# beast-dev/beast-mcmc

Hardware: AMD Instinct MI355X
Metric: full-tree lnL evals/sec (GTR+G4, 1e5 patterns) (higher is better)
Workload: dtype f64

## Files before the change

### beast-mcmc_amd/beagle.py

```python
import ctypes as C
import os

import numpy as np

_HERE = os.path.dirname(os.path.abspath(__file__))
ENGINE_LIB = os.path.join(_HERE, "lib", "libhmsbeagle-jni.so")
if os.environ.get("BEAGLE_MI355_ENGINE_LIB"):
    ENGINE_LIB = os.environ["BEAGLE_MI355_ENGINE_LIB"]
HOST_LIB = os.path.join(_HERE, "lib", "libbeast_host.so")

NONE = -1
FLAG_EIGEN_REAL, FLAG_EIGEN_COMPLEX, FLAG_PROCESSOR_GPU, FLAG_FRAMEWORK_CPU = 1 << 4, 1 << 5, 1 << 16, 1 << 27
OPERATION_TUPLE_SIZE = 7

ERROR_NAMES = {0: "NO_ERROR", -1: "GENERAL_ERROR", -2: "OUT_OF_MEMORY_ERROR", -3: "UNIDENTIFIED_EXCEPTION_ERROR",
               -4: "UNINITIALIZED_INSTANCE_ERROR", -5: "OUT_OF_RANGE_ERROR", -6: "NO_RESOURCE_ERROR",
               -7: "NO_IMPLEMENTATION_ERROR", -8: "FLOATING_POINT_ERROR"}


class BeagleException(RuntimeError):

    def __init__(self, function_name, code):
        super().__init__("%s returned %d (%s)" % (function_name, code, ERROR_NAMES.get(code, "?")))
        self.function_name = function_name
# ... 56 lines not shown
    "ConvolveTransitionMatrices": ([C.c_int, _IP, _IP, _IP, C.c_int], C.c_int),
    "UpdateTransitionMatrices": ([C.c_int, C.c_int, _IP, _IP, _IP, _DP, C.c_int], C.c_int),
    "UpdateTransitionMatricesWithMultipleModels": ([C.c_int, _IP, _IP, _IP, _IP, _IP, _DP, C.c_int], C.c_int),
    "UpdatePartials": ([C.c_int, _IP, C.c_int, C.c_int], C.c_int),
    "UpdatePartialsByPartition": ([C.c_int, _IP, C.c_int], C.c_int),
    "WaitForPartials": ([C.c_int, _IP, C.c_int], C.c_int),
    "AccumulateScaleFactors": ([C.c_int, _IP, C.c_int, C.c_int], C.c_int),
    "AccumulateScaleFactorsByPartition": ([C.c_int, _IP, C.c_int, C.c_int, C.c_int], C.c_int),
    "RemoveScaleFactors": ([C.c_int, _IP, C.c_int, C.c_int], C.c_int),
    "RemoveScaleFactorsByPartition": ([C.c_int, _IP, C.c_int, C.c_int, C.c_int], C.c_int),
    "ResetScaleFactors": ([C.c_int, C.c_int], C.c_int),
    "ResetScaleFactorsByPartition": ([C.c_int, C.c_int, C.c_int], C.c_int),
    "CopyScaleFactors": ([C.c_int, C.c_int, C.c_int], C.c_int),
    "CalculateRootLogLikelihoods": ([C.c_int, _IP, _IP, _IP, _IP, C.c_int, _DP], C.c_int),
    "CalculateRootLogLikelihoodsByPartition": ([C.c_int, _IP, _IP, _IP, _IP, _IP, C.c_int, C.c_int, _DP, _DP], C.c_int),
    "GetSiteLogLikelihoods": ([C.c_int, _DP], C.c_int),
    "SetRootPrePartials": ([C.c_int, _IP, _IP, C.c_int], C.c_int),
    "SetDifferentialMatrix": ([C.c_int, C.c_int, _DP], C.c_int),
    "AddTransitionMatrices": ([C.c_int, _IP, _IP, _IP, C.c_int], C.c_int),
    "TransposeTransitionMatrices": ([C.c_int, _IP, _IP, C.c_int], C.c_int),
    "UpdatePrePartials": ([C.c_int, _IP, C.c_int, C.c_int], C.c_int),
    "UpdatePrePartialsByPartition": ([C.c_int, _IP, C.c_int], C.c_int),
    "CalculateEdgeDifferentials": ([C.c_int, _IP, _IP, _IP, _IP, C.c_int, _DP, _DP, _DP], C.c_int),
    "CalculateCrossProductDifferentials": ([C.c_int, _IP, _IP, _IP, _IP, _DP, C.c_int, _DP, _DP], C.c_int),
}

ABI_SYMBOLS = ["beagleGetVersion", "beagleGetCitation", "beagleGetResourceList", "beagleGetBenchmarkedResourceList", "beagleGetApiTable",
               "beagleGetPartitionApiTable"] + \
              ["beagle" + k for k in _PROTOS] + \
              ["beagleMi355SetStream", "beagleMi355CalculateRootLogLikelihoodsDevice", "beagleMi355Synchronize",
               "beagleMi355KernelTimer", "beagleMi355DeviceBytes", "beagleMi355WalkStats", "beagleMi355GradientStats", "beagleMi355GetPartialsBatch", "beagleMi355SampleAncestralStates", "beagleMi355SampleMarkovJumps", "beagleMi355SampleMarkovJumpsUniformized",
               "beagleMi355SimulateSequences", "beagleMi355SimulateCompleteHistories", "beagleMi355RobustCounts", "beagleMi355SimulateUnconditionedCounts", "beagleMi355NodeHeightDerivatives", "beagleMi355UpdateDifferentialMatrices", "beagleMi355SetReversibleModels", "beagleMi355GetEigenDecomposition", "beagleMi355EigenStats", "beagleMi355UpdateTransitionMatricesFromGenerators", "beagleMi355GeneratorStats", "beagleMi355UpdateTransitionMatricesWithEpochs", "beagleMi355EpochStats", "beagleMi355NodePatternLikelihoods", "beagleMi355NodePatternStats", "beagleMi355NodePosteriors", "beagleMi355NodePosteriorStats", "beagleMi355PlacementScores", "beagleMi355PlacementStats", "beagleMi355SetTipEmission", "beagleMi355TipEmissionStats",
               "beagleMi355GetPartialsPinned", "beagleMi355GetSiteLogLikelihoodsPinned",
               "beagleMi355KernelTimerCalls", "beagleMi355WalkHealth", "beagleMi355RepeatStats", "beagleMi355RepeatSubRunStats", "beagleMi355TableOperandStats", "beagleMi355WalkLaunchInfo", "beagleMi355RootFusedCount", "beagleMi355SitePrefetchCount", "beagleMi355KernelTimerRestart", "beagleMi355GetDimensions", "beagleMi355GetCommUniqueId", "beagleMi355CommInit", "beagleMi355CommInfo", "beagleMi355CalculateRootLogLikelihoodsAllReduce"] + \
              ["beagleBasta" + k for k in ("AllocateCoalescentBuffers", "UpdatePartials", "AccumulatePartials", "GetBuffer", "GetBufferLength", "Stats", "SampleStates", "StatesStats",
                                           "Gradient", "GradientStats", "UpdatePartialsGrad", "UpdateTransitionMatricesGrad", "AccumulatePartialsGrad")]
BASTA_OPERATION_SIZE = 8


class EngineLibrary:

    def __init__(self, path=ENGINE_LIB, prefix=""):
        if not os.path.exists(path):
            raise OSError("engine library %s is missing: run `python -c 'import __graft_entry__ as g; g.build()'` "
                          "(there is no CPU fallback)" % path)
        self.path = path
        self.prefix = prefix
        self.lib = C.CDLL(path, mode=C.RTLD_LOCAL)
        self.fn = {}
        for name, (argtypes, restype) in _PROTOS.items():
            f = getattr(self.lib, prefix + "beagle" + name, None)
            if f is None:
                continue
            f.argtypes = argtypes
            f.restype = restype
            self.fn[name] = f
        gv = getattr(self.lib, prefix + "beagleGetVersion")
        gv.restype = C.c_char_p
        self.version = gv().decode()
        tab = getattr(self.lib, prefix + "beagleGetApiTable")
        tab.restype = C.c_void_p
        self.api_table = tab()
        ptab = getattr(self.lib, prefix + "beagleGetPartitionApiTable", None)
        self.partition_api_table = None
        if ptab is not None:
            ptab.restype = C.c_void_p
            self.partition_api_table = ptab()
# ... 858 lines not shown

    def bastaGradientStats(self):
        out = (C.c_long * 4)()
        self._check("bastaGradientStats", self._ext("beagleBastaGradientStats", [C.c_int, C.POINTER(C.c_long)])(self.instance, out))
        return tuple(out)

    def walkStats(self):
        out = (C.c_long * 8)()
        self._check("walkStats", self._ext("beagleMi355WalkStats", [C.c_int, C.POINTER(C.c_long)])(self.instance, out))
        keys = ("micro_ops", "stored", "mem_reads", "tip_reads", "scale_reads", "walks", "scale_writes", "fast_walks")
        stats = {k: int(out[i]) for i, k in enumerate(keys)}
        rep = self.repeatStats()
        stats.update({k: rep[k] for k in ("table_rows", "table_reads", "repeat_clades")})
        return stats

    def repeatStats(self):
        out = (C.c_long * 10)()
        self._check("repeatStats", self._ext("beagleMi355RepeatStats", [C.c_int, C.POINTER(C.c_long)])(self.instance, out))
        keys = ("table_rows", "table_reads", "repeat_clades", "table_bytes", "clades_indexed", "index_host_us", "two_table_nodes",
                "tables_under_definitions", "index_host_bytes", "index_resets")
        return {k: int(out[i]) for i, k in enumerate(keys)}

    def repeatSubRunStats(self):
        out = (C.c_long * 2)()
        self._check("repeatSubRunStats", self._ext("beagleMi355RepeatSubRunStats", [C.c_int, C.POINTER(C.c_long)])(self.instance, out))
        return {"sub_runs": int(out[0]), "sub_run_micro_ops": int(out[1])}

    def tableOperandStats(self):
        out = (C.c_long * 4)()
        self._check("tableOperandStats", self._ext("beagleMi355TableOperandStats", [C.c_int, C.POINTER(C.c_long)])(self.instance, out))
        return {"table_first_children": int(out[0]), "behind_memory_first_child": int(out[1]), "behind_fused_cherry": int(out[2]),
                "max_classes": int(out[3])}

    def walkHealth(self):
        out = (C.c_long * 4)()
        self._check("walkHealth", self._ext("beagleMi355WalkHealth", [C.c_int, C.POINTER(C.c_long)])(self.instance, out))
        return {"self_served": int(out[0]), "spin_limit_us": int(out[1]), "folded_vectors": int(out[2]), "fold_builds": int(out[3])}

    def walkLaunchInfo(self):
        out = (C.c_long * 8)()
        self._check("walkLaunchInfo", self._ext("beagleMi355WalkLaunchInfo", [C.c_int, C.POINTER(C.c_long)])(self.instance, out))
        return {"ticket_walks": int(out[0]), "flag_walks": int(out[1]), "rows": int(out[2]), "slices": int(out[3]),
                "fused_cherries": int(out[4]), "micro_ops": int(out[5]), "slice_accumulations": int(out[6]), "partition_roots_in_walk": int(out[7])}

    def gradientStats(self):
        out = (C.c_long * 4)()
        self._check("gradientStats", self._ext("beagleMi355GradientStats", [C.c_int, C.POINTER(C.c_long)])(self.instance, out))
        return {"fused": int(out[0]), "by_operation": int(out[1]), "walked": int(out[2]), "late": int(out[3])}

    def deviceBytes(self):
        return self._ext("beagleMi355DeviceBytes", [C.c_int], C.c_long)(self.instance)
```

### beast-mcmc_amd/csrc/engine_abi.cpp

```cpp
#include "engine_internal.h"

using mi355::OpDesc;
using mi355::shardedStates;
using mi355::shardedCategories;
using namespace mi355::eng;

namespace {

int accumulate(Instance* in, const int* idx, int count, int cum, double sign, int part) {
    if (badIndex(cum, in->scaleCount) || (part >= 0 && badIndex(part, in->partitionCount))) return BEAGLE_ERROR_OUT_OF_RANGE;
    const int pStart = part < 0 ? 0 : in->partStart[part], pEnd = part < 0 ? in->P : in->partEnd[part];
    int rc = materializeScaleUsers(in, cum); if (rc) return rc;
    rc = ensureScale(in, cum); if (rc) return rc;
    if (in->scaleIsRaw[cum]) return BEAGLE_ERROR_OUT_OF_RANGE;
    if (in->walk && in->sliceSums && in->partitionCount == 1 && in->lastSums.valid && in->lastSums.epoch == in->scaleWriteEpoch &&
        count > 0 && count == in->lastSums.nWritten) {
        const long stamp = ++in->seenCounter;
        bool same = true;
        for (int k = 0; k < count && same; k++) {
            if (badIndex(idx[k], in->scaleCount)) return BEAGLE_ERROR_OUT_OF_RANGE;
            same = in->scaleGen[(size_t)idx[k]] == in->lastSums.gen && in->scaleSeen[(size_t)idx[k]] != stamp;
            in->scaleSeen[(size_t)idx[k]] = stamp;
        }
        if (same) {
// ... 11 lines not shown
    for (int k = 0; k < count; k++) {
        if (badIndex(idx[k], in->scaleCount)) return BEAGLE_ERROR_OUT_OF_RANGE;
        rc = ensureScale(in, idx[k]); if (rc) return rc;
        srcs[k] = in->scale[idx[k]]; raw[k] = in->scaleIsRaw[idx[k]];
    }
    const int chunk = 4096;
    for (int b = 0; b < count; b += chunk) {
        const int n = std::min(chunk, count - b);
        void *dSrc = nullptr, *dRaw = nullptr;
        rc = uploadTransient(in, &srcs[b], (size_t)n * sizeof(double*), &dSrc); if (rc) return rc;
        rc = uploadTransient(in, &raw[b], (size_t)n * sizeof(int), &dRaw); if (rc) return rc;
        mi355::launchAccumulateScale(live(in), in->scale[cum], (const double* const*)dSrc, (const int*)dRaw, n, sign, pStart, pEnd);
    }
    HIP_TRY(hipGetLastError());
    return 0;
}

int runTriples(Instance* in, const int* first, const int* second, const int* result, int count, decltype(&mi355::launchConvolveMatrices) launch) {
    int b = 0;
    while (b < count) {
        int e = b + 1;
        for (; e < count; e++) {
            bool dep = false;
            for (int k = b; k < e && !dep; k++)
                dep = result[k] == first[e] || result[k] == second[e] || result[k] == result[e] ||
                      first[k] == result[e] || second[k] == result[e];
            if (dep) break;
        }
        const int n = e - b;
        void *dF, *dS, *dR;
        int rc = uploadTransient(in, first + b, n * sizeof(int), &dF); if (rc) return rc;
        rc = uploadTransient(in, second + b, n * sizeof(int), &dS); if (rc) return rc;
        rc = uploadTransient(in, result + b, n * sizeof(int), &dR); if (rc) return rc;
        launch(live(in), in->matrices, (const int*)dF, (const int*)dS, (const int*)dR, n, in->S, in->C);
        b = e;
    }
    HIP_TRY(hipGetLastError());
    return BEAGLE_SUCCESS;
}

void toTiled(const Instance* in, const double* api, double* tiled, int categories) {
    const size_t S = in->S, P = in->P, nt = in->ntile;
    std::fill(tiled, tiled + (size_t)categories * nt * S * 32, 0.0);
    for (int c = 0; c < categories; c++)
        for (size_t p = 0; p < P; p++) {
            const double* src = api + ((size_t)c * P + p) * S;
            double* dst = tiled + ((size_t)c * nt + p / 32) * S * 32 + p % 32;
            for (size_t j = 0; j < S; j++) dst[j * 32] = src[j];
        }
}

}

extern "C" {

const char* beagleGetVersion(void) { return "4.0.0-mi355"; }

const char* beagleGetCitation(void) {
    return "MI355X-native tree-likelihood engine behind the beagle.Beagle surface (gfx950 HIP kernels).\n"
           "API after: Ayres et al. (2019) BEAGLE 3, Systematic Biology 68:1052-1061.";
}

BeagleResourceList* beagleGetResourceList(void) { return &resources()->rl; }

int beagleFinalizeInstance(int instance) {
    if (mi355::isShardedHandle(instance)) { return mi355::shardedFinalize(instance); }
    Instance* in = nullptr;
// ... 16 lines not shown
int beagleSetPatternWeights(int instance, const double* w) {
    if (mi355::isShardedHandle(instance)) {
        return mi355::shardedSetPerPatternDoubles(instance, w, 1, 1, [&](int h, const double* v) { return beagleSetPatternWeights(h, v); });
    }
    GET_INSTANCE(instance);
    return upload(in, in->patternWeights, w, (size_t)in->P * sizeof(double));
}

int beagleSetPatternPartitions(int instance, int partitionCount, const int* partitions) {
    if (mi355::isShardedHandle(instance)) {
        return mi355::shardedSetPerPatternInts(instance, partitions,
                                               [&](int h, const int* v) { return beagleSetPatternPartitions(h, partitionCount, v); });
    }
    GET_INSTANCE(instance);
    if (partitionCount < 1) return BEAGLE_ERROR_OUT_OF_RANGE;
    for (int x = 0; x < in->partialsCount; x++) { int rcv = materializeVirtual(in, x); if (rcv) return rcv; }
    std::vector<int> s(partitionCount, -1), e(partitionCount, -1);
    for (int p = 0; p < in->P; p++) {
        const int k = partitions[p];
        if (badIndex(k, partitionCount)) return BEAGLE_ERROR_OUT_OF_RANGE;
        if (s[k] < 0) s[k] = p;
        else if (e[k] != p) return BEAGLE_ERROR_NO_IMPLEMENTATION;
        e[k] = p + 1;
    }
    for (int k = 0; k < partitionCount; k++) if (s[k] < 0) { s[k] = 0; e[k] = 0; }
    in->partitionCount = partitionCount; in->partStart = s; in->partEnd = e; in->resolveEpoch++;
    if (in->walk || in->walkT || in->virt) in->planner.setPartitionCount(partitionCount);
    if (in->virt) {
        const size_t per = (size_t)in->C * in->S * in->S, slots = matrixSlotLayout(in);
        double* grown = nullptr;
        int rcm = devAlloc(in, (void**)&grown, slots * per * sizeof(double)); if (rcm) return rcm;
        HIP_TRY(hipMemsetAsync(grown, 0, slots * per * sizeof(double), live(in)));
        HIP_TRY(hipMemcpyAsync(grown, in->matrices, (size_t)std::max(1, in->matrixCount) * per * sizeof(double), hipMemcpyDeviceToDevice, live(in)));
        in->matrices = grown;
        if (in->tiled) { int rci = uploadIdentityMatrix(in); if (rci) return rci; }
    }
    if (in->walk) {
        forgetFolds(in);
        setPairLayout(in);
        in->sliceRows = 0; in->lastSums.valid = false;
        if (!in->dPairPos) { int rc = devAlloc(in, (void**)&in->dPairPos, (size_t)in->P * sizeof(unsigned)); if (rc) return rc; }
        HIP_TRY(hipStreamSynchronize(live(in)));
        HIP_TRY(hipMemcpy(in->dPairPos, in->pairPos.data(), (size_t)in->P * sizeof(unsigned), hipMemcpyHostToDevice));
        in->stateSlabLeft = 0; in->scaleSlabLeft = 0;
        std::vector<mi355::RelayoutJob> jobs;
        for (int t = 0; t < in->partialsCount; t++) {
            uint8_t* old = in->tipStates[t];
            if (!old) continue;
            in->tipStates[t] = nullptr;
            int rc = ensureStates(in, t); if (rc) return rc;
            jobs.push_back({old, in->tipStates[t], in->tipStates[t] + in->statePairOff});
        }
        for (size_t b = 0; b < jobs.size(); b += 16384) {
            const size_t e = std::min(jobs.size(), b + 16384);
            void* dJobs = nullptr;
            int rc = uploadTransient(in, jobs.data() + b, (e - b) * sizeof(mi355::RelayoutJob), &dJobs); if (rc) return rc;
            mi355::launchRelayoutStatesBatch(live(in), (const mi355::RelayoutJob*)dJobs, (int)(e - b), in->dPairPos, in->P, (int)in->pairLen, in->S);
        }
        for (int k = 0; k < (int)in->scale.size(); k++) {
            double* old = in->scale[k];
            if (!old) continue;
            const char raw = in->scaleIsRaw[k];
            in->scale[k] = nullptr;
            int rc = ensureScale(in, k); if (rc) return rc;
            in->scaleIsRaw[k] = raw;
            HIP_TRY(hipMemcpyAsync(in->scale[k], old, (size_t)in->P * sizeof(double), hipMemcpyDeviceToDevice, live(in)));
            if (raw) mi355::launchRecipFromFactors(live(in), in->scale[k], in->scale[k] + in->scaleStride, in->dPairPos, in->P);
// ... 200 lines not shown

int beagleConvolveTransitionMatrices(int instance, const int* first, const int* second, const int* result, int count) {
    if (mi355::isShardedHandle(instance)) {
        return mi355::shardedBroadcast(instance, [&](int h) { return beagleConvolveTransitionMatrices(h, first, second, result, count); });
    }
    GET_INSTANCE(instance);
    if (count <= 0) return BEAGLE_SUCCESS;
    for (int k = 0; k < count; k++) {
        if (badIndex(first[k], in->matrixCount) || badIndex(second[k], in->matrixCount) || badIndex(result[k], in->matrixCount) ||
            result[k] == first[k] || result[k] == second[k]) return BEAGLE_ERROR_OUT_OF_RANGE;
    }
    return runTriples(in, first, second, result, count, mi355::launchConvolveMatrices);
}

static void noteScaleOfOp(Instance* in, const int* op, int tuple) {
    if (badIndex(op[0], in->partialsCount)) return;
    const int sIdx = op[1] != BEAGLE_OP_NONE ? op[1] : op[2];
    if (op[1] != BEAGLE_OP_NONE && !badIndex(op[1], in->scaleCount)) in->scaleVersion[op[1]]++;
    const bool unknown = tuple == BEAGLE_PARTITION_OP_COUNT && in->partitionCount > 1;
    in->scaleOfPartial[op[0]] = unknown ? -2 : (sIdx != BEAGLE_OP_NONE && !badIndex(sIdx, in->scaleCount)) ? sIdx : -1;
    in->scaleVersionAtWrite[op[0]] = in->scaleOfPartial[op[0]] >= 0 ? in->scaleVersion[sIdx] : 0u;
}

static int transitionMatrices(Instance* in, const int* eigenIdx, int eigenScalar, const int* rateIdx,
                              const int* probIdx, const double* lens, int count) {
    if (count <= 0) return BEAGLE_SUCCESS;
    auto outOfRange = [count](const int* v, int limit) {
        int lo = v[0], hi = v[0];
        for (int k = 1; k < count; k++) { lo = v[k] < lo ? v[k] : lo; hi = v[k] > hi ? v[k] : hi; }
        return lo < 0 || hi >= limit;
    };
    if (outOfRange(probIdx, in->matrixCount) || (eigenIdx ? outOfRange(eigenIdx, in->eigenCount) : badIndex(eigenScalar, in->eigenCount)) ||
        (rateIdx && outOfRange(rateIdx, in->eigenCount))) return BEAGLE_ERROR_OUT_OF_RANGE;
    bool fusable = in->S == 4 && in->kernelUploads && in->fuseLaunches && !eigenIdx && !rateIdx && (size_t)count * 12 <= RING_BYTES / 4 &&
                   (int)in->pendingCopies.size() <= mi355::HOST_COPY_MAX;
    if (fusable) {
        const char* m0 = (const char*)in->matrices;
        const char* m1 = m0 + (size_t)std::max(1, in->matrixCount) * in->C * in->S * in->S * sizeof(double);
        const std::vector<Instance::PendingCopy>& pc = in->pendingCopies;
        for (size_t a = 0; a < pc.size() && fusable; a++) {
            const char* d0 = (const char*)pc[a].dst; const char* d1 = d0 + pc[a].bytes;
            if (d0 < m1 && m0 < d1) fusable = false;
            for (size_t b = a + 1; b < pc.size() && fusable; b++) {
                const char* e0 = (const char*)pc[b].dst; const char* e1 = e0 + pc[b].bytes;
                if (d0 < e1 && e0 < d1 && !(e0 <= d0 && d1 <= e1)) fusable = false;
            }
        }
    }
    if (fusable) {
        const size_t lenBytes = (size_t)count * sizeof(double), idxBytes = (size_t)count * sizeof(int);
        const long off = stage(in, lens, lenBytes, lenBytes + idxBytes);
        if (off < 0) return BEAGLE_ERROR_GENERAL;
        memcpy(in->hRing + off + lenBytes, probIdx, idxBytes);
        const size_t eigStride = in->eigenComplex ? 40 : 36;
        const double* const eigDst = in->eigen + eigStride * eigenScalar;
        const double* eigSrc = eigDst;
        const double* ratesSrc = in->rates;
        mi355::HostCopyList L;
        L.n = 0;
        unsigned blocks = 0;
        for (const Instance::PendingCopy& pc : in->pendingCopies) {
            mi355::HostCopyList::Entry& e = L.e[L.n++];
            e.dst = pc.dst; e.src = in->hRingDev + pc.ringOff; e.bytes = (unsigned)pc.bytes; e.firstBlock = blocks;
            blocks += (unsigned)((pc.bytes + 4095) / 4096);
            if (pc.dst == (void*)eigDst && pc.bytes == eigStride * sizeof(double)) eigSrc = (const double*)(in->hRingDev + pc.ringOff);
            if (pc.dst == (void*)in->rates && pc.bytes >= (size_t)in->C * sizeof(double)) ratesSrc = (const double*)(in->hRingDev + pc.ringOff);
        }
        for (int a = 0; a < L.n; a++)
            for (int b = a + 1; b < L.n; b++)
                if ((const char*)L.e[b].dst <= (const char*)L.e[a].dst &&
                    (const char*)L.e[a].dst + L.e[a].bytes <= (const char*)L.e[b].dst + L.e[b].bytes) L.e[a].bytes = 0;
        in->pendingCopies.clear();
        mi355::launchTransitionMatrices4Fused(in->stream, in->matrices, eigSrc, ratesSrc, (const int*)(in->hRingDev + off + lenBytes),
                                              (const double*)(in->hRingDev + off), count, in->C, in->eigenComplex, L, (int)blocks);
        HIP_TRY(hipGetLastError());
        return BEAGLE_SUCCESS;
    }
    if (in->S == 4 && in->kernelUploads && in->fuseLaunches && (size_t)count * 20 <= RING_BYTES / 4) {
        const size_t lenBytes = (size_t)count * sizeof(double), idxBytes = (size_t)count * sizeof(int);
        const long off = stage(in, lens, lenBytes, lenBytes + 3 * idxBytes);
        if (off < 0) return BEAGLE_ERROR_GENERAL;
        memcpy(in->hRing + off + lenBytes, probIdx, idxBytes);
        int* rEig = (int*)(in->hRing + off + lenBytes + idxBytes);
        int* rRate = rEig + count;
        if (eigenIdx) memcpy(rEig, eigenIdx, idxBytes); else std::fill(rEig, rEig + count, eigenScalar);
        if (rateIdx) memcpy(rRate, rateIdx, idxBytes); else std::fill(rRate, rRate + count, 0);
        const int* rIdx = (const int*)(in->hRingDev + off + lenBytes);
        mi355::launchTransitionMatrices(live(in), in->matrices, in->eigen, in->rates, rIdx, (const double*)(in->hRingDev + off),
                                        rIdx + count, rIdx + 2 * (size_t)count, count, in->S, in->C, in->eigenComplex);
        HIP_TRY(hipGetLastError());
        return BEAGLE_SUCCESS;
    }
    std::vector<char> pack((size_t)count * (sizeof(double) + 3 * sizeof(int)));
    double* pLen = (double*)pack.data();
    int* pIdx = (int*)(pack.data() + (size_t)count * sizeof(double));
    memcpy(pLen, lens, (size_t)count * sizeof(double));
    memcpy(pIdx, probIdx, (size_t)count * sizeof(int));
    if (eigenIdx) memcpy(pIdx + count, eigenIdx, (size_t)count * sizeof(int)); else std::fill(pIdx + count, pIdx + 2 * (size_t)count, eigenScalar);
    if (rateIdx) memcpy(pIdx + 2 * (size_t)count, rateIdx, (size_t)count * sizeof(int)); else std::fill(pIdx + 2 * (size_t)count, pIdx + 3 * (size_t)count, 0);
    void* dPack;
    int rc = uploadTransient(in, pack.data(), pack.size(), &dPack); if (rc) return rc;
    const double* dLen = (const double*)dPack;
    const int* dIdx = (const int*)((const char*)dPack + (size_t)count * sizeof(double));
    mi355::launchTransitionMatrices(live(in), in->matrices, in->eigen, in->rates, dIdx, dLen,
                                    dIdx + count, dIdx + 2 * (size_t)count, count, in->S, in->C, in->eigenComplex);
    HIP_TRY(hipGetLastError());
    return BEAGLE_SUCCESS;
}

int beagleUpdateTransitionMatrices(int instance, int eigenIndex, const int* probabilityIndices,
                                   const int* firstDerivativeIndices, const int* secondDerivativeIndices,
                                   const double* edgeLengths, int count) {
    if (mi355::isShardedHandle(instance)) {
        if (firstDerivativeIndices || secondDerivativeIndices) return BEAGLE_ERROR_NO_IMPLEMENTATION;
        if (count <= 0) return BEAGLE_SUCCESS;
        std::vector<int> p(probabilityIndices, probabilityIndices + count); std::vector<double> t(edgeLengths, edgeLengths + count);
        return mi355::shardedPost(instance, [=](int h) { return beagleUpdateTransitionMatrices(h, eigenIndex, p.data(), nullptr, nullptr, t.data(), count); });
    }
    GET_INSTANCE_KEEP_PENDING(instance);
    if (firstDerivativeIndices || secondDerivativeIndices) return BEAGLE_ERROR_NO_IMPLEMENTATION;
    if (in->heldPre.held && probabilityIndices)
        for (int k = 0; k < count; k++) if (heldReadsMatrix(in, probabilityIndices[k])) { int rcp = executeHeldPre(in); if (rcp) return rcp; break; }
    return transitionMatrices(in, nullptr, eigenIndex, nullptr, probabilityIndices, edgeLengths, count);
}

int beagleUpdateTransitionMatricesWithMultipleModels(int instance, const int* eigenIndices, const int* categoryRateIndices,
                                   const int* probabilityIndices, const int* firstDerivativeIndices,
                                   const int* secondDerivativeIndices, const double* edgeLengths, int count) {
    if (mi355::isShardedHandle(instance)) {
        if (firstDerivativeIndices || secondDerivativeIndices) return BEAGLE_ERROR_NO_IMPLEMENTATION;
        if (!eigenIndices || !categoryRateIndices) return BEAGLE_ERROR_OUT_OF_RANGE;
        if (count <= 0) return BEAGLE_SUCCESS;
        std::vector<int> e(eigenIndices, eigenIndices + count), r(categoryRateIndices, categoryRateIndices + count), p(probabilityIndices, probabilityIndices + count);
        std::vector<double> t(edgeLengths, edgeLengths + count);
        return mi355::shardedPost(instance, [=](int h) { return beagleUpdateTransitionMatricesWithMultipleModels(h, e.data(), r.data(), p.data(), nullptr, nullptr, t.data(), count); });
    }
    GET_INSTANCE(instance);
    if (firstDerivativeIndices || secondDerivativeIndices) return BEAGLE_ERROR_NO_IMPLEMENTATION;
// ... 131 lines not shown
}

int beagleSetDifferentialMatrix(int instance, int matrixIndex, const double* inMatrix) {
    return beagleSetTransitionMatrix(instance, matrixIndex, inMatrix, 0.0);
}

int beagleAddTransitionMatrices(int instance, const int* first, const int* second, const int* result, int count) {
    if (mi355::isShardedHandle(instance)) {
        return mi355::shardedBroadcast(instance, [&](int h) { return beagleAddTransitionMatrices(h, first, second, result, count); });
    }
    GET_INSTANCE(instance);
    if (count <= 0) return BEAGLE_SUCCESS;
    if (!first || !second || !result) return BEAGLE_ERROR_OUT_OF_RANGE;
    for (int k = 0; k < count; k++)
        if (badIndex(first[k], in->matrixCount) || badIndex(second[k], in->matrixCount) || badIndex(result[k], in->matrixCount)) return BEAGLE_ERROR_OUT_OF_RANGE;
    return runTriples(in, first, second, result, count, mi355::launchAddMatrices);
}

int beagleTransposeTransitionMatrices(int instance, const int* inputIndices, const int* resultIndices, int matrixCount) {
    if (mi355::isShardedHandle(instance)) {
        return mi355::shardedBroadcast(instance,
                                       [&](int h) { return beagleTransposeTransitionMatrices(h, inputIndices, resultIndices, matrixCount); });
    }
    GET_INSTANCE(instance);
    if (matrixCount <= 0) return BEAGLE_SUCCESS;
    std::vector<int> pairs((size_t)matrixCount * 2);
    for (int k = 0; k < matrixCount; k++) {
        if (badIndex(inputIndices[k], in->matrixCount) || badIndex(resultIndices[k], in->matrixCount) || inputIndices[k] == resultIndices[k])
            return BEAGLE_ERROR_OUT_OF_RANGE;
        pairs[2 * k] = inputIndices[k]; pairs[2 * k + 1] = resultIndices[k];
    }
    void* dPairs = nullptr;
    int rc = uploadTransient(in, pairs.data(), pairs.size() * sizeof(int), &dPairs); if (rc) return rc;
    mi355::launchTransposeMatrices(live(in), in->matrices, (const int*)dPairs, matrixCount, in->S, in->C);
    HIP_TRY(hipGetLastError());
    return BEAGLE_SUCCESS;
}

int beagleUpdatePrePartials(int instance, const int* operations, int operationCount, int cumulativeScaleIndex) {
    if (mi355::isShardedHandle(instance)) {
        return mi355::shardedBroadcast(instance, [&](int h) { return beagleUpdatePrePartials(h, operations, operationCount, cumulativeScaleIndex); });
    }
    GET_INSTANCE_KEEP_PENDING(instance);
    DEMOTE_FOLDED_TIPS(in);
    return runPreOperations(in, operations, operationCount, cumulativeScaleIndex, true);
}

int beagleCalculateCrossProductDifferentials(int instance, const int* postBufferIndices, const int* preBufferIndices,
                                             const int* categoryRateIndices, const int* categoryWeightsIndices,
                                             const double* edgeLengths, int count,
                                             double* outSumDerivatives, double* outSumSquaredDerivatives) {
    if (mi355::isShardedHandle(instance)) {
        if (!outSumDerivatives) return BEAGLE_ERROR_OUT_OF_RANGE;
        const int len = shardedStates(instance) * shardedStates(instance);
        std::vector<double> tot(len, 0.0);
        const int rc = mi355::shardedSumDoubles(instance, len, [&](int h, double* out) { return beagleCalculateCrossProductDifferentials(h, postBufferIndices,
                              preBufferIndices, categoryRateIndices, categoryWeightsIndices, edgeLengths, count, out, outSumSquaredDerivatives); }, tot.data());
        for (int k = 0; k < len && !rc; k++) outSumDerivatives[k] += tot[k];
        return rc;
    }
    GET_INSTANCE(instance);
    DEMOTE_FOLDED_TIPS(in);
    if (outSumSquaredDerivatives) return BEAGLE_ERROR_NO_IMPLEMENTATION;
    if (!postBufferIndices || !preBufferIndices || !categoryRateIndices || !categoryWeightsIndices || !edgeLengths || !outSumDerivatives)
        return BEAGLE_ERROR_OUT_OF_RANGE;
    if (badIndex(categoryRateIndices[0], in->eigenCount) || badIndex(categoryWeightsIndices[0], in->eigenCount)) return BEAGLE_ERROR_OUT_OF_RANGE;
    return crossProducts(in, postBufferIndices, preBufferIndices, categoryRateIndices[0], categoryWeightsIndices[0], edgeLengths, count,
// ... 84 lines not shown
```

### beast-mcmc_amd/csrc/engine_create.cpp

```cpp
#include "engine_internal.h"

using mi355::labEnv;
using namespace mi355::eng;

static bool switchOn(const char* name) {
    const char* v = getenv(name);
    return v && atoi(v) != 0;
}

namespace mi355 {
namespace eng {

size_t matrixSlotLayout(Instance* in) {
    size_t slots = std::max<size_t>(std::max<size_t>(1, in->matrixCount), (size_t)in->planner.matrixSlots());
    if (in->tiled) { in->preIdentity = (int)slots; in->preTransposed = (int)slots + 1; slots += 1 + PRE_SCRATCH; }
    if (in->emis) { in->emis->shadowBase = (int)slots; slots += (size_t)std::max(1, in->matrixCount); }
    return slots;
}
int uploadIdentityMatrix(Instance* in) {
    const size_t S = in->S, C = in->C;
    std::vector<double> eye(C * S * S, 0.0);
    for (size_t c = 0; c < C; c++) for (size_t i = 0; i < S; i++) eye[c * S * S + i * S + i] = 1.0;
    return upload(in, in->matrices + (size_t)in->preIdentity * C * S * S, eye.data(), eye.size() * sizeof(double));
}
// ... 147 lines not shown
                     !switchOn("BEAGLE_MI355_NO_T32_WRITE_WALK");
    in->planner.init(partialsBufferCount, tipCount, matrixBufferCount, scaleBufferCount, maxVirtSteps, virtualOn, in->holdSlots);
    {
        int memSteps = maxVirtSteps == 24 ? MEM_DEF_STEPS : 0, seenSteps = maxVirtSteps == 24 ? MEM_DEF_SEEN_STEPS : 0;
        if (getenv("BEAGLE_MI355_MEM_DEF_STEPS")) { memSteps = std::max(0, std::min(maxVirtSteps, atoi(getenv("BEAGLE_MI355_MEM_DEF_STEPS")))); seenSteps = 0; }
        if (getenv("BEAGLE_MI355_MEM_DEF_SEEN_STEPS")) seenSteps = std::max(0, std::min(maxVirtSteps, atoi(getenv("BEAGLE_MI355_MEM_DEF_SEEN_STEPS"))));
        if (switchOn("BEAGLE_MI355_NO_MEM_DEFS") || !in->walk || in->walkT || !virtualOn || in->holdSlots < 2) memSteps = seenSteps = 0;
        in->planner.memStepCap = memSteps;
        in->planner.memStepCapSeen = seenSteps;
        if (getenv("BEAGLE_MI355_MEM_DEF_INLINE_STEPS")) in->memDefInlineSteps = std::max(0, atoi(getenv("BEAGLE_MI355_MEM_DEF_INLINE_STEPS")));
    }
    {
        double frac = 1.0 / 8.0;
        if (const char* f = getenv("BEAGLE_MI355_REPEAT_MAX_FRAC")) {
            const char* slash = strchr(f, '/');
            const double num = atof(f), den = slash ? atof(slash + 1) : 1.0;
            if (num > 0.0 && den > 0.0) frac = num > 1.0 && !slash ? 1.0 / num : num / den;
        }
        frac = std::min(frac, 0.5);
        in->repeatsOn = in->walk && !in->walkT && virtualOn && stateCount == 4 && in->holdSlots >= 2 && !switchOn("BEAGLE_MI355_NO_REPEATS") &&
                        (bufferBytes >= ((size_t)2 << 20) || switchOn("BEAGLE_MI355_REPEATS_ANY_SIZE"));
        in->repeatMaxClasses = std::max(1, (int)((double)patternCount * frac));
        if (in->repeatsOn) { in->repeatIndex.init(tipCount, patternCount, in->repeatMaxClasses); in->hostTips.assign((size_t)tipCount, std::vector<uint8_t>()); }
        if (in->repeatsOn && getenv("BEAGLE_MI355_REPEAT_CAPACITY")) in->repeatIndex.setCapacity((size_t)std::max(1, atoi(getenv("BEAGLE_MI355_REPEAT_CAPACITY"))));
    }
    in->planner.memDefTables = !switchOn("BEAGLE_MI355_NO_MEMDEF_TABLES");
    in->planner.cacheEnabled = !switchOn("BEAGLE_MI355_NO_PLAN_CACHE");
    in->fastWalk = !switchOn("BEAGLE_MI355_NO_FAST_WALK");
    in->strictWaits = !(getenv("BEAGLE_MI355_STRICT_WAITS") && atoi(getenv("BEAGLE_MI355_STRICT_WAITS")) == 0);
    in->fuseGradient = !switchOn("BEAGLE_MI355_NO_FUSED_GRADIENT");
    in->preWalk = !switchOn("BEAGLE_MI355_NO_PRE_WALK");
    in->fuseLaunches = !switchOn("BEAGLE_MI355_NO_LAUNCH_FUSION");
    in->deferWalk = !switchOn("BEAGLE_MI355_NO_ROOT_FUSION");
    in->foldScales = !switchOn("BEAGLE_MI355_NO_SCALE_FOLD");
    {
        const int gv = getenv("BEAGLE_MI355_GRADIENT_VIRTUAL") ? atoi(getenv("BEAGLE_MI355_GRADIENT_VIRTUAL")) : GRADIENT_VIRT_DEFAULT;
        in->gradientVirtual = in->walk && virtualOn && in->preWalk && in->fuseGradient && gv > 0;
        in->gradientVirtualSteps = std::max(1, std::min(GRADIENT_VIRT_STEPS, gv));
    }
    const size_t matrixSlots = matrixSlotLayout(in);
    const size_t patternSlots = in->tiled ? (size_t)in->ntile * 32 : (size_t)patternCount;
    in->partialsBytes = (((size_t)categoryCount * patternSlots * stateCount * sizeof(double)) + 255 + (in->walk ? 256 : 0)) & ~(size_t)255;
    in->partials.assign(partialsBufferCount, nullptr);
    in->scaleOfPartial.assign(partialsBufferCount, -2); in->scaleVersionAtWrite.assign(partialsBufferCount, 0u);
    in->scaleVersion.assign(std::max(1, scaleBufferCount), 0u);
    in->tipStates.assign(partialsBufferCount, nullptr);
    in->scale.assign(std::max(1, scaleBufferCount), nullptr);
    in->scaleIsRaw.assign(std::max(1, scaleBufferCount), 0);
    in->partStart.assign(1, 0); in->partEnd.assign(1, patternCount);
    setPairLayout(in);
    in->wStamp.assign(partialsBufferCount, 0); in->wLevel.assign(partialsBufferCount, 0); in->wOp.assign(partialsBufferCount, 0);
    in->rStamp.assign(partialsBufferCount, 0); in->rLevel.assign(partialsBufferCount, 0);
    in->resourceName = res->names[device + 1];

    bool ok = hipStreamCreateWithFlags(&in->ownStream, hipStreamNonBlocking) == hipSuccess;
    in->stream = in->ownStream;
    ok = ok && hipHostMalloc((void**)&in->hRing, RING_BYTES, hipHostMallocMapped | hipHostMallocCoherent) == hipSuccess;
    ok = ok && hipHostGetDevicePointer((void**)&in->hRingDev, in->hRing, 0) == hipSuccess;
    in->kernelUploads = !switchOn("BEAGLE_MI355_COPY_ENGINE_UPLOADS");
    in->sitePrefetch = !switchOn("BEAGLE_MI355_NO_SITE_PREFETCH");
    in->fuseWaves = !switchOn("BEAGLE_MI355_NO_WALK_FUSION");
    in->useTickets = !switchOn("BEAGLE_MI355_NO_WALK_TICKETS");
    in->xcdAware = !switchOn("BEAGLE_MI355_NO_XCD_MAP");
    in->fuseCherries = !switchOn("BEAGLE_MI355_NO_CHERRY_FUSION");
    in->skipTipLoads = !switchOn("BEAGLE_MI355_NO_LOAD_SKIP");
    in->sliceSums = !switchOn("BEAGLE_MI355_NO_SLICE_SUMS");
// ... 62 lines not shown
```

### beast-mcmc_amd/csrc/engine_differential.cpp

```cpp
#include "engine_internal.h"

using namespace mi355::eng;

static int differentialMatrices(Instance* in, const int* eigenIdx, const int* rateIdx, const double* inDifferentials, int differentialCount,
                                const int* diffIdx, const int* slots, const double* lens, int count, int mode) {
    if (in->S > 64 || in->basta) return BEAGLE_ERROR_NO_IMPLEMENTATION;
    if (count <= 0) return BEAGLE_SUCCESS;
    if (mode != BEAGLE_MI355_DIFFERENTIAL_EXACT && mode != BEAGLE_MI355_DIFFERENTIAL_FIRST_ORDER) return BEAGLE_ERROR_OUT_OF_RANGE;
    if (!inDifferentials || !slots || !lens || differentialCount < 1) return BEAGLE_ERROR_OUT_OF_RANGE;
    std::vector<char> named((size_t)in->matrixCount, 0);
    for (int k = 0; k < count; k++) {
        if (badIndex(slots[k], in->matrixCount) || named[(size_t)slots[k]]) return BEAGLE_ERROR_OUT_OF_RANGE;
        named[(size_t)slots[k]] = 1;
        if ((eigenIdx && badIndex(eigenIdx[k], in->eigenCount)) || (rateIdx && badIndex(rateIdx[k], in->eigenCount)) ||
            (diffIdx && badIndex(diffIdx[k], differentialCount))) return BEAGLE_ERROR_OUT_OF_RANGE;
    }
    if (in->eigenCount < 1) return BEAGLE_ERROR_OUT_OF_RANGE;
    const bool exact = mode == BEAGLE_MI355_DIFFERENTIAL_EXACT;
    std::vector<int> pairs, pairOf((size_t)count);
    if (exact) {
        std::unordered_map<long long, int> seen;
        for (int k = 0; k < count; k++) {
            const int e = eigenIdx ? eigenIdx[k] : 0, d = diffIdx ? diffIdx[k] : 0;
            const auto at = seen.emplace((long long)e * differentialCount + d, (int)(pairs.size() / 2));
            if (at.second) { pairs.push_back(e); pairs.push_back(d); }
            pairOf[(size_t)k] = at.first->second;
        }
    } else for (int k = 0; k < count; k++) pairOf[(size_t)k] = diffIdx ? diffIdx[k] : 0;
    const size_t per = (size_t)in->S * in->S, nPairs = pairs.size() / 2;
    const size_t qBytes = (size_t)differentialCount * per * sizeof(double), lenBytes = (size_t)count * sizeof(double),
                 idxBytes = (size_t)count * sizeof(int), bytes = qBytes + lenBytes + 4 * idxBytes + pairs.size() * sizeof(int);
    if (bytes > RING_BYTES / 2) return BEAGLE_ERROR_OUT_OF_RANGE;
    for (int k = 0; k < count; k++)
        if (heldReadsMatrix(in, slots[k])) { const int rcp = executeHeldPre(in); if (rcp) return rcp; break; }
    std::vector<char> pack(bytes);
    memcpy(pack.data(), inDifferentials, qBytes);
    memcpy(pack.data() + qBytes, lens, lenBytes);
    int* pIdx = (int*)(pack.data() + qBytes + lenBytes);
    memcpy(pIdx, slots, idxBytes);
    if (eigenIdx) memcpy(pIdx + count, eigenIdx, idxBytes); else std::fill(pIdx + count, pIdx + 2 * (size_t)count, 0);
    if (rateIdx) memcpy(pIdx + 2 * (size_t)count, rateIdx, idxBytes); else std::fill(pIdx + 2 * (size_t)count, pIdx + 3 * (size_t)count, 0);
    memcpy(pIdx + 3 * (size_t)count, pairOf.data(), idxBytes);
    if (!pairs.empty()) memcpy(pIdx + 4 * (size_t)count, pairs.data(), pairs.size() * sizeof(int));
    if (exact) {
        const size_t need = nPairs * per * sizeof(double);
        const int rcg = growDevice(in, in->differentialDev, need, (need + 4095) & ~(size_t)4095, Grow::SyncIfHeld); if (rcg) return rcg;
    }
    void* dPack = nullptr;
    const int rc = uploadTransient(in, pack.data(), bytes, &dPack); if (rc) return rc;
    const double* dQ = (const double*)dPack;
    const double* dLen = (const double*)((const char*)dPack + qBytes);
    const int* dIdx = (const int*)((const char*)dPack + qBytes + lenBytes);
    const int *dEig = dIdx + count, *dRate = dIdx + 2 * (size_t)count, *dPair = dIdx + 3 * (size_t)count, *dPairs = dIdx + 4 * (size_t)count;
    if (exact) {
        double* V = in->differentialDev.as<double>();
        mi355::launchDifferentialRotate(live(in), V, in->eigen, dQ, dPairs, (int)nPairs, in->S, in->eigenComplex);
        mi355::launchDifferentialExact(live(in), in->matrices, in->eigen, in->rates, V, dIdx, dLen, dEig, dRate, dPair, count, in->S, in->C,
                                       in->eigenComplex);
    } else {
        mi355::launchDifferentialFirstOrder(live(in), in->matrices, in->rates, dQ, dIdx, dLen, dRate, dPair, count, in->S, in->C);
    }
    HIP_TRY(hipGetLastError());
    return BEAGLE_SUCCESS;
}

extern "C" {

int beagleMi355UpdateDifferentialMatrices(int instance, const int* eigenIndices, const int* categoryRatesIndices,
                                          const double* inDifferentials, int differentialCount, const int* differentialIndices,
                                          const int* matrixIndices, const double* edgeLengths, int count, int mode) {
    if (mi355::isShardedHandle(instance)) {
        return mi355::shardedBroadcast(instance, [&](int h) {
            return beagleMi355UpdateDifferentialMatrices(h, eigenIndices, categoryRatesIndices, inDifferentials, differentialCount,
                                                         differentialIndices, matrixIndices, edgeLengths, count, mode); });
    }
    GET_INSTANCE_KEEP_PENDING(instance);
    return differentialMatrices(in, eigenIndices, categoryRatesIndices, inDifferentials, differentialCount, differentialIndices,
                                matrixIndices, edgeLengths, count, mode);
}

}
```

### beast-mcmc_amd/csrc/engine_epoch.cpp

```cpp
#include "engine_internal.h"

using namespace mi355::eng;

constexpr size_t EPOCH_LAUNCH_BYTES = RING_BYTES / 4;

static size_t epochChunk() {
    if (const char* e = getenv("BEAGLE_MI355_EPOCH_CHUNK")) { const long v = atol(e); if (v > 0) return (size_t)v; }
    return SIZE_MAX;
}

static int checkEpochList(int S, const int* off, const int* segEig, const double* segLen, const int* slots, int count, int flags) {
    if (S > 64) return BEAGLE_ERROR_NO_IMPLEMENTATION;
    if (count < 0 || flags != 0) return BEAGLE_ERROR_OUT_OF_RANGE;
    if (count == 0) return BEAGLE_SUCCESS;
    if (!off || !segEig || !segLen || !slots) return BEAGLE_ERROR_OUT_OF_RANGE;
    if (off[0] != 0) return BEAGLE_ERROR_OUT_OF_RANGE;
    for (int k = 0; k < count; k++) if (off[k + 1] <= off[k]) return BEAGLE_ERROR_OUT_OF_RANGE;
    for (int j = 0; j < off[count]; j++) if (!(std::isfinite(segLen[j]) && segLen[j] >= 0.0)) return BEAGLE_ERROR_OUT_OF_RANGE;
    return BEAGLE_SUCCESS;
}

static int epochMatrices(Instance* in, const int* off, const int* segEig, const double* segLen, const int* rateIdx, const int* slots,
                         int count, int flags) {
    const int rcc = checkEpochList(in->S, off, segEig, segLen, slots, count, flags); if (rcc) return rcc;
// ... 9 lines not shown
    for (int j = 0; j < off[count]; j++) if (badIndex(segEig[j], in->eigenCount)) return BEAGLE_ERROR_OUT_OF_RANGE;
    if (in->eigenCount < 1) return BEAGLE_ERROR_OUT_OF_RANGE;
    for (int k = 0; k < count; k++)
        if (heldReadsMatrix(in, slots[k])) { const int rcp = executeHeldPre(in); if (rcp) return rcp; break; }
    const size_t chunk = epochChunk();
    std::vector<char> pack;
    for (int first = 0; first < count;) {
        const size_t perEntry = 3 * sizeof(int), perSeg = sizeof(double) + sizeof(int);
        int last = first + 1;
        size_t bytes = sizeof(int) + perEntry + (size_t)(off[last] - off[first]) * perSeg;
        while (last < count && (size_t)(last - first) < chunk) {
            const size_t more = perEntry + (size_t)(off[last + 1] - off[last]) * perSeg;
            if (bytes + more > EPOCH_LAUNCH_BYTES) break;
            bytes += more; last++;
        }
        const size_t m = (size_t)(last - first), s0 = (size_t)off[first], nSeg = (size_t)off[last] - s0;
        pack.resize(nSeg * sizeof(double) + (m + 1 + nSeg + 2 * m) * sizeof(int));
        double* pLen = (double*)pack.data();
        int* pOff = (int*)(pack.data() + nSeg * sizeof(double));
        int* pEig = pOff + m + 1;
        int* pSlot = pEig + nSeg;
        int* pRate = pSlot + m;
        memcpy(pLen, segLen + s0, nSeg * sizeof(double));
        memcpy(pEig, segEig + s0, nSeg * sizeof(int));
        for (size_t k = 0; k <= m; k++) pOff[k] = off[(size_t)first + k] - (int)s0;
        for (size_t k = 0; k < m; k++) { pSlot[k] = slots[(size_t)first + k]; pRate[k] = rateIdx ? rateIdx[(size_t)first + k] : 0; }
        void* dPack = nullptr;
        const int rc = uploadTransient(in, pack.data(), pack.size(), &dPack); if (rc) return rc;
        const double* dLen = (const double*)dPack;
        const int* dOff = (const int*)((const char*)dPack + nSeg * sizeof(double));
        const int* dEig = dOff + m + 1;
        const int* dSlot = dEig + nSeg;
        const int* dRate = dSlot + m;
        if (!mi355::launchEpochMatrices(live(in), in->matrices, in->eigen, in->rates, dSlot, dRate, dOff, dEig, dLen, (int)m, in->S, in->C,
                                        in->eigenComplex)) return BEAGLE_ERROR_GENERAL;
        HIP_TRY(hipGetLastError());
        first = last;
    }
    in->statEpochCalls++; in->statEpochMatrices += (long)count * in->C; in->statEpochSegments += off[count]; in->statEpochLongest = longest;
    return BEAGLE_SUCCESS;
}

extern "C" {

int beagleMi355UpdateTransitionMatricesWithEpochs(int instance, const int* segmentOffsets, const int* segmentEigenIndices,
                                                  const double* segmentLengths, const int* categoryRateIndices,
                                                  const int* probabilityIndices, int count, int flags) {
    if (mi355::isShardedHandle(instance)) {
        const int rcc = checkEpochList(mi355::shardedStates(instance), segmentOffsets, segmentEigenIndices, segmentLengths,
                                       probabilityIndices, count, flags); if (rcc) return rcc;
        if (count == 0) return BEAGLE_SUCCESS;
        const int nSeg = segmentOffsets[count];
        std::vector<int> o(segmentOffsets, segmentOffsets + count + 1), e(segmentEigenIndices, segmentEigenIndices + nSeg),
                         p(probabilityIndices, probabilityIndices + count), r;
        std::vector<double> t(segmentLengths, segmentLengths + nSeg);
        if (categoryRateIndices) r.assign(categoryRateIndices, categoryRateIndices + count);
        const bool hasR = categoryRateIndices != nullptr;
        return mi355::shardedPost(instance, [=](int h) {
            return beagleMi355UpdateTransitionMatricesWithEpochs(h, o.data(), e.data(), t.data(), hasR ? r.data() : nullptr, p.data(), count, 0); });
    }
    GET_INSTANCE_KEEP_PENDING(instance);
    return epochMatrices(in, segmentOffsets, segmentEigenIndices, segmentLengths, categoryRateIndices, probabilityIndices, count, flags);
}

int beagleMi355EpochStats(int instance, long* out4) {
    if (mi355::isShardedHandle(instance)) { return mi355::shardedFirst(instance, [&](int h) { return beagleMi355EpochStats(h, out4); }); }
    GET_INSTANCE_KEEP_PENDING(instance);
// ... 7 lines not shown
```

### beast-mcmc_amd/csrc/engine_generator.cpp

```cpp
#include "engine_internal.h"
#include <cfloat>

using namespace mi355::eng;

constexpr size_t GENERATOR_TABLE_BUDGET = (size_t)128 << 20;

static size_t generatorChunk(size_t n) {
    n = std::max<size_t>(1, n);
    if (const char* e = getenv("BEAGLE_MI355_GENERATOR_CHUNK")) { const long v = atol(e); if (v > 0) n = std::min(n, (size_t)v); }
    return n;
}

static int checkGenerators(int S, const double* Q, int G, const double* lens, int count, std::vector<double>& mu) {
    if (S > 64) return BEAGLE_ERROR_NO_IMPLEMENTATION;
    if (count < 0 || G < 1 || !Q) return BEAGLE_ERROR_OUT_OF_RANGE;
    if (count > 0 && !lens) return BEAGLE_ERROR_OUT_OF_RANGE;
    mu.resize((size_t)G);
    for (int g = 0; g < G; g++) {
        const double* q = Q + (size_t)g * S * S;
        for (int i = 0; i < S; i++)
            for (int j = 0; j < S; j++) {
                const double x = q[(size_t)i * S + j];
                if (!std::isfinite(x) || (i == j ? x > 0.0 : x < 0.0)) return BEAGLE_ERROR_OUT_OF_RANGE;
            }
// ... 37 lines not shown
        if (heldReadsMatrix(in, slots[k])) { const int rcp = executeHeldPre(in); if (rcp) return rcp; break; }
    int rc = growScratch(in, in->generatorDev, std::min((size_t)G, genChunk) * tableBytes); if (rc) return rc;
    bool fresh = false;
    rc = growDevice(in, in->generatorStatsDev, 2 * sizeof(unsigned), 256, Grow::SyncIfHeld, &fresh); if (rc) return rc;
    if (fresh) HIP_TRY(hipMemsetAsync(in->generatorStatsDev.p, 0, 256, live(in)));
    std::vector<char> pack;
    for (size_t p = 0; p < nParts; p++) {
        const size_t g0 = p * genChunk, nGen = std::min(genChunk, (size_t)G - g0);
        bool tablesDone = false;
        for (size_t first = (size_t)partStart[p]; first < (size_t)partStart[p + 1]; first += entChunk) {
            const size_t m = std::min(entChunk, (size_t)partStart[p + 1] - first);
            const size_t qBytes = tablesDone ? 0 : nGen * SS * sizeof(double), muBytes = nGen * sizeof(double),
                         lenBytes = m * sizeof(double), idxBytes = m * sizeof(int), bytes = qBytes + muBytes + lenBytes + 3 * idxBytes;
            pack.resize(bytes);
            if (qBytes) memcpy(pack.data(), Q + g0 * SS, qBytes);
            memcpy(pack.data() + qBytes, mu.data() + g0, muBytes);
            double* pLen = (double*)(pack.data() + qBytes + muBytes);
            int* pIdx = (int*)(pack.data() + qBytes + muBytes + lenBytes);
            for (size_t k = 0; k < m; k++) {
                const int e = order[first + k];
                pLen[k] = lens[e];
                pIdx[k] = slots[e];
                pIdx[m + k] = (genIdx ? genIdx[e] : 0) - (int)g0;
                pIdx[2 * m + k] = rateIdx ? rateIdx[e] : 0;
            }
            void* dPack = nullptr;
            rc = uploadTransient(in, pack.data(), bytes, &dPack); if (rc) return rc;
            const double* dMu = (const double*)((const char*)dPack + qBytes);
            const double* dLen = (const double*)((const char*)dPack + qBytes + muBytes);
            const int* dIdx = (const int*)((const char*)dPack + qBytes + muBytes + lenBytes);
            double* tables = in->generatorDev.as<double>();
            if (!tablesDone && !mi355::launchGeneratorPowers(live(in), tables, (const double*)dPack, dMu, (int)nGen, in->S)) return BEAGLE_ERROR_GENERAL;
            tablesDone = true;
            if (!mi355::launchGeneratorMatrices(live(in), in->matrices, in->rates, tables, dMu, dIdx, dLen, dIdx + m, dIdx + 2 * m,
                                                in->generatorStatsDev.as<unsigned>(), (int)m, in->S, in->C)) return BEAGLE_ERROR_GENERAL;
            HIP_TRY(hipGetLastError());
        }
    }
    in->statGeneratorCalls++; in->statGeneratorMatrices += (long)count * in->C;
    return BEAGLE_SUCCESS;
}

extern "C" {

int beagleMi355UpdateTransitionMatricesFromGenerators(int instance, const double* generators, int generatorCount,
                                                      const int* generatorIndices, const int* categoryRateIndices,
                                                      const int* probabilityIndices, const double* edgeLengths, int count) {
    if (mi355::isShardedHandle(instance)) {
        const int S = mi355::shardedStates(instance);
        std::vector<double> mu;
        const int rcc = checkGenerators(S, generators, generatorCount, edgeLengths, count, mu); if (rcc) return rcc;
        if (count == 0) return BEAGLE_SUCCESS;
        if (!probabilityIndices) return BEAGLE_ERROR_OUT_OF_RANGE;
        std::vector<double> q(generators, generators + (size_t)generatorCount * S * S), t(edgeLengths, edgeLengths + count);
        std::vector<int> p(probabilityIndices, probabilityIndices + count), g, r;
        if (generatorIndices) g.assign(generatorIndices, generatorIndices + count);
        if (categoryRateIndices) r.assign(categoryRateIndices, categoryRateIndices + count);
        const bool hasG = generatorIndices != nullptr, hasR = categoryRateIndices != nullptr;
        return mi355::shardedPost(instance, [=](int h) {
            return beagleMi355UpdateTransitionMatricesFromGenerators(h, q.data(), generatorCount, hasG ? g.data() : nullptr,
                                                                     hasR ? r.data() : nullptr, p.data(), t.data(), count); });
    }
    GET_INSTANCE_KEEP_PENDING(instance);
    return generatorMatrices(in, generators, generatorCount, generatorIndices, categoryRateIndices, probabilityIndices, edgeLengths, count);
}

int beagleMi355GeneratorStats(int instance, long* out4) {
// ... 14 lines not shown
```

### beast-mcmc_amd/csrc/engine_instance.cpp

```cpp
#include "engine_internal.h"

using mi355::OpDesc;

namespace mi355 {
namespace eng {

std::mutex g_mutex;
std::vector<Instance*> g_instances;

Instance* lookup(int h) {
    std::lock_guard<std::mutex> lock(g_mutex);
    if (h < 0 || h >= (int)g_instances.size()) return nullptr;
    return g_instances[h];
}

int devAlloc(Instance* in, void** p, size_t bytes, bool counted) {
    HIP_TRY(hipMalloc(p, bytes));
    in->allocations.push_back({*p, bytes, counted});
    if (counted) in->deviceBytes += bytes;
    return 0;
}

void devFree(Instance* in, void* p) {
    if (!p) return;
// ... 5 lines not shown

int growDevice(Instance* in, DevBuf& b, size_t need, size_t want, Grow how, bool* grew) {
    if (grew) *grew = false;
    if (b.bytes >= need) return 0;
    if (how == Grow::SyncAndFree || (how == Grow::SyncIfHeld && b.p)) HIP_TRY(hipStreamSynchronize(live(in)));
    if (how != Grow::KeepOld) devFree(in, b.p);
    b.p = nullptr; b.bytes = 0;
    int rc = devAlloc(in, (void**)&b.p, want, b.counted); if (rc) { b.p = nullptr; return rc; }
    b.bytes = want;
    if (grew) *grew = true;
    return 0;
}

int ScopedDevice::alloc(size_t bytes) {
    reset();
    if (hipMalloc(&p, bytes) != hipSuccess) { p = nullptr; return BEAGLE_ERROR_OUT_OF_MEMORY; }
    return 0;
}
void ScopedDevice::reset() { if (p) { hipStreamSynchronize(live(in)); hipFree(p); p = nullptr; } }

long stage(Instance* in, const void* src, size_t bytes, size_t reserve) {
    const size_t need = (std::max(bytes, reserve) + 255) & ~(size_t)255;
    if (need > RING_BYTES) return -1;
    if (in->ringHead + need > RING_BYTES) {
        if (hipStreamSynchronize(live(in)) != hipSuccess) return -1;
        in->ringHead = 0;
    }
    const size_t off = in->ringHead;
    memcpy(in->hRing + off, src, bytes);
    in->ringHead += need;
    return (long)off;
}

int upload(Instance* in, void* dst, const void* src, size_t bytes) {
    if (bytes == 0) return 0;
    if (bytes <= RING_BYTES / 4) {
        long off = stage(in, src, bytes);
        if (off < 0) return BEAGLE_ERROR_GENERAL;
        return queueCopy(in, dst, (size_t)off, bytes);
    }
    HIP_TRY(hipMemcpyAsync(dst, src, bytes, hipMemcpyHostToDevice, live(in)));
    HIP_TRY(hipStreamSynchronize(live(in)));
    return 0;
}

int uploadTransient(Instance* in, const void* src, size_t bytes, void** dptr) {
    long off = stage(in, src, bytes);
    if (off < 0) return BEAGLE_ERROR_GENERAL;
    *dptr = in->dRing + off;
    return queueCopy(in, in->dRing + off, (size_t)off, bytes);
}

int queueCopy(Instance* in, void* dst, size_t off, size_t bytes) {
    if (bytes == 0) return 0;
    if (in->pendingWalk.valid && !in->copyKeepsWalk) { const int rcw = flushWalk(in); if (rcw) return rcw; }
    if (!in->kernelUploads) {
        HIP_TRY(hipMemcpyAsync(dst, in->hRing + off, bytes, hipMemcpyHostToDevice, in->stream));
        return 0;
    }
    Instance::PendingCopy pc; pc.dst = dst; pc.ringOff = off; pc.bytes = bytes;
    in->pendingCopies.push_back(pc);
    return 0;
}

int flushUploads(Instance* in) {
    std::vector<Instance::PendingCopy>& pc = in->pendingCopies;
    int rc = 0;
    for (size_t i = 0; i < pc.size();) {
        mi355::HostCopyList L;
        L.n = 0;
        unsigned blocks = 0;
        for (; i < pc.size() && L.n < mi355::HOST_COPY_MAX; i++) {
            const char* d0 = (const char*)pc[i].dst; const char* d1 = d0 + pc[i].bytes;
            bool partial = false;
            for (int a = 0; a < L.n; a++) {
                const char* e0 = (const char*)L.e[a].dst; const char* e1 = e0 + L.e[a].bytes;
                if (L.e[a].bytes == 0 || !(d0 < e1 && e0 < d1)) continue;
                if (d0 <= e0 && e1 <= d1) L.e[a].bytes = 0; else partial = true;
            }
            if (partial) break;
            mi355::HostCopyList::Entry& e = L.e[L.n++];
            e.dst = pc[i].dst; e.src = in->hRingDev + pc[i].ringOff; e.bytes = (unsigned)pc[i].bytes; e.firstBlock = blocks;
            blocks += (unsigned)((pc[i].bytes + 4095) / 4096);
        }
        mi355::launchHostCopies(in->stream, L, (int)blocks);
    }
    pc.clear();
    if (hipGetLastError() != hipSuccess) rc = BEAGLE_ERROR_GENERAL;
// ... 170 lines not shown
```

### beast-mcmc_amd/csrc/engine_internal.h

```cpp
#pragma once
#include <hip/hip_runtime.h>
#include <rccl/rccl.h>
#include <algorithm>
#include <climits>
#include <cmath>
#include <cstdio>
#include <cstdlib>
#include <cstring>
#include <mutex>
#include <string>
#include <thread>
#include <vector>
#include <chrono>
#include <atomic>
#include <unordered_map>
#include "../../include/beagle_mi355.h"
#include "kernels.h"
#include "planner.h"
#include "scratch_layout.h"
#include "sharded.h"

namespace mi355 {
namespace eng {


#define HIP_TRY(expr)                                                                         \
    do {                                                                                      \
        hipError_t e__ = (expr);                                                              \
        if (e__ != hipSuccess) {                                                              \
            if (getenv("BEAGLE_MI355_DEBUG"))                                                 \
                fprintf(stderr, "[beagle-mi355] %s failed: %s (%s:%d)\n", #expr, hipGetErrorString(e__), __FILE__, __LINE__); \
            return e__ == hipErrorOutOfMemory ? BEAGLE_ERROR_OUT_OF_MEMORY : BEAGLE_ERROR_GENERAL; \
        }                                                                                     \
    } while (0)

constexpr size_t RING_BYTES = 16u << 20;
constexpr int SLAB_BUFFERS = 32;
constexpr int PRE_SCRATCH = 32;
constexpr int GRADIENT_VIRT_STEPS = 2;
constexpr int MEM_DEF_STEPS = 8;
constexpr int MEM_DEF_SEEN_STEPS = 24;
constexpr int MEM_DEF_INLINE_STEPS = 8;
constexpr int GRADIENT_VIRT_DEFAULT = 1;

struct Basta;
struct TipEmissions;

struct DevBuf {
    char* p = nullptr; size_t bytes = 0;
    bool counted = true;
    template <class T> T* as() const { return reinterpret_cast<T*>(p); }
};
// ... 10 lines not shown
    mi355::WalkPlanner planner;
    mi355::Plan plan;
    size_t scaleStride = 0;
    size_t statePairOff = 0;
    std::vector<unsigned> pairPos; size_t pairLen = 0; std::vector<int> padStart; unsigned* dPairPos = nullptr;
    DevBufUncounted matStream;
    uint8_t* dummyTips = nullptr; double* onesScale = nullptr;
    long statFastWalks = 0;
    struct WalkTraffic {
        long memReads = 0, tipReads = 0, scaleReads = 0, scaleWrites = 0, stored = 0, fused = 0;
        long microOps = 0;
        long tableRows = 0, tableReads = 0, repeatClades = 0, twoTables = 0, unstoredConsumers = 0;
        long subRuns = 0, subRunOps = 0;
        long tabFirst = 0, tabFirstBehindMem = 0, tabFirstBehindCherry = 0, tabMaxClasses = 0;
    };
    struct Resolved {
        bool kept = false;
        long tag = 0, epoch = -1;
        std::vector<mi355::WalkOp> w; std::vector<mi355::WalkSeg> segs; std::vector<int> deps;
        bool oneLaunch = false;
        std::vector<int> order;
        int leaves = 0;
        int maxRange = 0, sinks = 0;
        std::vector<int> finalStore, finalPart, sinkRows;
        std::vector<int> sumRows, wroteScale;
        std::vector<const double*> cm;
        WalkTraffic traffic;
        DevBufUncounted dProg; bool dProgValid = false;
        std::vector<int> folds;
        long foldEpoch = -1;
        long noFoldTag = 0;
        bool compressed = false; mi355::RepeatPlan repeats; int lowerRange = 0;
        bool repeatsMissing = false;
    } resolved[8], scratch;
    struct FoldVec { std::vector<int> members; double* recip = nullptr; long builtEpoch = -1; bool bad = false; };
    std::vector<FoldVec> folds;
    std::vector<std::pair<size_t, int>> foldIndex;
    std::vector<double*> foldFree;
    long scaleWriteEpoch = 0;
    bool foldScales = true;
    DevBuf foldWorst;
    long resolveEpoch = 0;
    bool repeatsOn = false; int repeatMaxClasses = 0;
    bool repeatSlicing = false, repeatSlicingOff = false;
    int memDefInlineSteps = MEM_DEF_INLINE_STEPS;
    int closedListRun = 0;
    mi355::RepeatIndex repeatIndex;
    std::vector<std::vector<uint8_t>> hostTips;
    long tipDataEpoch = 0, repeatEpoch = -1, repeatCompactEpoch = -1;
    struct RepeatTable { int D = 0, arena = 0, row = 0; char* dev = nullptr; size_t bytes = 0, tipStride = 0; std::vector<int> tips; };
    std::unordered_map<int, RepeatTable> repeatTables;
    struct RepeatBlock { char* dev = nullptr; size_t size = 0, used = 0; };
    std::vector<RepeatBlock> repeatPool;
    char* repeatStage = nullptr; size_t repeatStageSize = 0, repeatStageUsed = 0;
    double* repeatArena = nullptr; int repeatArenas = 0; mi355::RepeatRows repeatRows;
    std::vector<int> repeatQueue;
    long statTableRows = 0, statTableReads = 0, statRepeatClades = 0, statTwoTables = 0, statUnstoredConsumers = 0;
    long statSubRuns = 0, statSubRunOps = 0;
    long statTabFirst = 0, statTabFirstBehindMem = 0, statTabFirstBehindCherry = 0, statTabMaxClasses = 0;
    size_t repeatTableCap = 0;
    bool lastPlanCached = false;
    long statRepeatResets = 0;
    long statRepeatBuildUs = 0;
    bool lowerLaunched = false;
    bool fastWalk = true;
    struct HeldPreNode { int par, preA, preB, postA, postB, matA, matB, level, jobA, jobB, size; };
    struct HeldPreList {
// ... 2 lines not shown
        std::vector<HeldPreNode> nodes;
        std::vector<int> order;
        std::vector<unsigned> walkFlags;
        std::vector<int> segStart, segRoot;
        int maxLevel = 0, holdSlots = 0, rootBuf = -1;
        std::vector<char> readsMatrix, readsBuf, writesBuf;
    } heldPre;
    double* preRootCopy = nullptr;
    uint8_t* preDummyStates = nullptr;
    DevBuf dPreProg;
    std::vector<int> scaleOfPartial; std::vector<unsigned> scaleVersionAtWrite, scaleVersion;
    bool trackScales = false;
    long statFusedGradients = 0, statPreLists = 0, statWalkedGradients = 0, statLateLists = 0;
    int storeAllEvaluations = 0;
    bool gradientVirtual = false; int gradientVirtualSteps = GRADIENT_VIRT_STEPS;
    DevBuf edgeScratch;
    bool preWalk = true;
    bool fuseGradient = true;
    bool walkT = false;
    bool walkTWrite = false;
    bool fuseRootParts = true;
    long statRootPartsFused = 0;
    static constexpr int ROOT_PARTS_TABLES = 4;
    mi355::RootFusedParts* rootPartsDev = nullptr;
    std::vector<char> rootPartsShadow[ROOT_PARTS_TABLES];
    int rootPartsNext = 0;
    bool fuseLaunches = true;
    struct PendingWalk {
        bool valid = false;
        const mi355::WalkOp* prog = nullptr; const mi355::WalkSeg* segs = nullptr; const int* deps = nullptr;
        int nSegs = 0, range = 0, flagStride = 0; unsigned epoch = 0;
        int leaves = 0;
        unsigned cherryOff = 0;
        std::vector<int> finalStore;
        std::vector<int> finalPart;
        std::vector<int> sinkRows;
    } pendingWalk;
    std::vector<int> snapSourceOf;
    bool deferWalk = true;
    bool copyKeepsWalk = false;
    long statRootFused = 0;
    long statFoldedVectors = 0, statFoldBuilds = 0;
    unsigned* rootCounter = nullptr;
    DevBuf cherryTables;
    int holdSlots = 3;
    bool eigenComplex = false;
    bool strictWaits = true;
    bool virt = false;
    bool cherry = false;
    long statCherries = 0;
    double hostPlanUs = 0, hostRunUs = 0, hostPrepUs = 0, hostPlanHitUs = 0, hostRunHitUs = 0; long hostCalls = 0, hostHits = 0; bool hostTrace = false, lastResolveMiss = false;
    DevBufUncounted bigStage;
    DevBufUncounted exportDev[2]; double* exportHost[2] = {nullptr, nullptr}; size_t exportBytes = 0;
    hipEvent_t exportEvent[2] = {nullptr, nullptr};
    DevBuf ancestralDev;
    DevBuf jumpDev;
    DevBuf uniformDev;
    DevBuf eventDev;
    DevBuf simulateDev;
    DevBuf robustDev;
    DevBuf historyDev;
    DevBuf differentialDev;
    DevBuf eigenSweepsDev;
    long statEigenCalls = 0, statEigenModels = 0; int eigenLastCount = 0;
    Basta* basta = nullptr;
    TipEmissions* emis = nullptr;
// ... 69 lines not shown
int devAlloc(Instance* in, void** p, size_t bytes, bool counted = true);
void devFree(Instance* in, void* p);
int growDevice(Instance* in, DevBuf& b, size_t need, size_t want, Grow how, bool* grew = nullptr);
void releaseDevice(Instance* in, DevBuf& b);
inline int growScratch(Instance* in, DevBuf& b, size_t need) { return growDevice(in, b, need, need, Grow::SyncIfHeld); }
static_assert(mi355::scratch::FLAG_SLOTS == mi355::MAX_JUMP_REGISTERS, "scratch_layout.h keeps one flag word per possible register");
long stage(Instance* in, const void* src, size_t bytes, size_t reserve = 0);
int upload(Instance* in, void* dst, const void* src, size_t bytes);
int uploadTransient(Instance* in, const void* src, size_t bytes, void** dptr);
int download(Instance* in, void* dst, const void* src, size_t bytes);
int ensurePartials(Instance* in, int idx);
int ensureScale(Instance* in, int idx);
int ensureStates(Instance* in, int idx);
void destroy(Instance* in);
struct Resources {
    std::vector<std::string> names, descs;
    std::vector<BeagleResource> list;
    BeagleResourceList rl;
    int gpuCount = 0;
};
extern const long GPU_FLAGS;
Resources* resources();
void setPairLayout(Instance* in);
int holdPreList(Instance* in, const int* ops, int count);
bool supersedesHeld(Instance* in, const int* ops, int count);
int ensureWalkDummies(Instance* in);
int flushUploads(Instance* in);
int flushWalk(Instance* in, const mi355::RootFused* root = nullptr);
inline hipStream_t live(Instance* in) {
    if (!in->pendingCopies.empty()) flushUploads(in);
    if (in->pendingWalk.valid) flushWalk(in);
    return in->stream;
}
int queueCopy(Instance* in, void* dst, size_t off, size_t bytes);
inline void ringIdle(Instance* in) { if (in->pendingCopies.empty() && !in->pendingWalk.valid) in->ringHead = 0; }
struct KeepWalkHeld {
    Instance* in;
    explicit KeepWalkHeld(Instance* i) : in(i) { in->copyKeepsWalk = true; }
    ~KeepWalkHeld() { in->copyKeepsWalk = false; }
};

#define GET_INSTANCE_KEEP_PENDING(h)                             \
    Instance* in = lookup(h);                                    \
    if (!in) return BEAGLE_ERROR_UNINITIALIZED_INSTANCE;         \
    if (hipSetDevice(in->device) != hipSuccess) return BEAGLE_ERROR_GENERAL;
#define GET_INSTANCE(h)                                          \
    GET_INSTANCE_KEEP_PENDING(h)                                 \
    if (in->heldPre.held) { const int rcPending__ = executeHeldPre(in); if (rcPending__) return rcPending__; }

struct ScopedDevice {
    Instance* in; void* p = nullptr;
    explicit ScopedDevice(Instance* i) : in(i) {}
    ScopedDevice(const ScopedDevice&) = delete; ScopedDevice& operator=(const ScopedDevice&) = delete;
    int alloc(size_t bytes);
    template <class T> T* as() const { return static_cast<T*>(p); }
    void reset();
    ~ScopedDevice() { reset(); }
};

inline bool badIndex(int i, int n) { return i < 0 || i >= n; }

struct TipEmission {
    int K = 0;
    bool folded = false;
    std::vector<uint8_t> codes;
    std::vector<double> table;
// ... 189 lines not shown
```

### beast-mcmc_amd/csrc/engine_preorder.cpp

```cpp
#include "engine_internal.h"

using mi355::OpDesc;

namespace mi355 {
namespace eng {

int ensurePreScratch(Instance* in) {
    if (!in->preScratch.empty()) return 0;
    void* slab = nullptr;
    int rc = devAlloc(in, &slab, in->partialsBytes * PRE_SCRATCH); if (rc) return rc;
    void* miss = nullptr;
    rc = devAlloc(in, &miss, ((size_t)in->P + 255) & ~(size_t)255); if (rc) return rc;
    in->preMissing = (uint8_t*)miss;
    HIP_TRY(hipMemsetAsync(in->preMissing, in->S, (size_t)in->P, live(in)));
    in->preScratch.assign(PRE_SCRATCH, nullptr);
    for (int j = 0; j < PRE_SCRATCH; j++) in->preScratch[j] = (double*)((char*)slab + in->partialsBytes * j);
    return 0;
}

int ensureEdgeScratch(Instance* in, size_t bytes) {
    return growDevice(in, in->edgeScratch, bytes, (bytes * 5 / 4 + 4095) & ~(size_t)4095, Grow::SyncAndFree);
}

int preLevelTwoPass(Instance* in, const OpDesc* ops, int nOps) {
    { int rc0 = ensurePreScratch(in); if (rc0) return rc0; }
    std::vector<OpDesc> pass(2 * PRE_SCRATCH);
    std::vector<int> pairs(2 * PRE_SCRATCH);
    for (int b = 0; b < nOps; b += PRE_SCRATCH) {
        const int n = std::min(PRE_SCRATCH, nOps - b);
        bool anyWrite = false;
        for (int j = 0; j < n; j++) {
            const OpDesc& o = ops[b + j];
            pairs[2 * j] = o.mat1; pairs[2 * j + 1] = in->preTransposed + j;
            OpDesc& a = pass[j];
            memset(&a, 0, sizeof(a));
            a.dest = in->preScratch[j];
            a.child1 = o.child1; a.mat1 = in->preIdentity;
            a.child2 = o.child2; a.mat2 = o.mat2; a.kind = o.kind & mi355::KIND_STATES2;
            a.pStart = 0; a.pEnd = in->P;
            OpDesc& c = pass[n + j];
            memset(&c, 0, sizeof(c));
            c.dest = o.dest;
            c.child1 = in->preScratch[j]; c.mat1 = in->preTransposed + j;
            c.child2 = in->preMissing; c.mat2 = in->preIdentity; c.kind = mi355::KIND_STATES2;
            c.scaleWrite = o.scaleWrite; c.scaleRead = o.scaleRead;
            c.pStart = 0; c.pEnd = in->P;
            anyWrite = anyWrite || o.scaleWrite != nullptr;
        }
        void *dPairs = nullptr, *dPass = nullptr;
        int rc = uploadTransient(in, pairs.data(), (size_t)2 * n * sizeof(int), &dPairs); if (rc) return rc;
        rc = uploadTransient(in, pass.data(), (size_t)2 * n * sizeof(OpDesc), &dPass); if (rc) return rc;
        mi355::launchTransposeMatrices(live(in), in->matrices, (const int*)dPairs, n, in->S, in->C);
        mi355::launchPruneLevelTiled(live(in), (const OpDesc*)dPass, n, in->matrices, in->P, in->S, in->C, false);
        mi355::launchPruneLevelTiled(live(in), (const OpDesc*)dPass + n, n, in->matrices, in->P, in->S, in->C, anyWrite);
    }
    return 0;
}

static bool walkableDefinition(const Instance* in, int buf) {
    if (!in->gradientVirtual || in->partitionCount != 1 || !isVirt(in, buf)) return false;
    const mi355::VirtDef& d = in->planner.definition(in->planner.key(buf, 0));
    if (!d.on || d.nSteps < 1 || d.nSteps > 2) return false;
    const mi355::VirtStep& s0 = d.steps[0];
    if (s0.type != mi355::VT_CHERRY || s0.memA || s0.memB || !in->tipStates[s0.tipA] || !in->tipStates[s0.tipB]) return false;
    if (d.nSteps == 2) {
        const mi355::VirtStep& s1 = d.steps[1];
        if (s1.type != mi355::VT_EXTEND || s1.subA != 0 || s1.memB || !in->tipStates[s1.tipB]) return false;
    }
    return true;
}
static int materializeHeldOperands(Instance* in) {
    ReadSet reads(in);
    for (const Instance::HeldPreNode& nd : in->heldPre.nodes) { reads.note(nd.postA); reads.note(nd.postB); }
    return reads.materialize();
}

int runPreOperations(Instance* in, const int* ops, int count, int globalCum, bool mayHold, int tuple) {
    if (count <= 0) return 0;
    if (in->partitionCount != 1 || tuple != BEAGLE_OP_COUNT) mayHold = false;
    const int n = in->partialsCount;
    {
        std::vector<char> written(n, 0), scaleWritten(std::max(1, in->scaleCount), 0);
        for (int k = 0; k < count; k++) {
            const int* op = ops + (size_t)k * tuple;
            const int dest = op[0], wS = op[1], rS = op[2], par = op[3], mc = op[4], sib = op[5], ms = op[6];
// ... 664 lines not shown
```

### beast-mcmc_amd/csrc/engine_stats.cpp

```cpp
#include "engine_internal.h"

using mi355::shardedStates;
using mi355::shardedCategories;
using namespace mi355::eng;

static void resetWalkCounters(Instance* in) {
    in->statMicroOps = in->statStored = in->statMemReads = in->statTipReads = in->statScaleReads = in->statWalks = in->statScaleWrites = 0;
    in->statFastWalks = in->statFused = 0;
    in->statTableRows = in->statTableReads = in->statRepeatClades = in->statTwoTables = in->statUnstoredConsumers = 0;
    in->statSubRuns = in->statSubRunOps = 0;
    in->statTabFirst = in->statTabFirstBehindMem = in->statTabFirstBehindCherry = in->statTabMaxClasses = 0;
}

extern "C" {

int beagleMi355SetStream(int instance, void* hipStream) {
    if (mi355::isShardedHandle(instance)) { return BEAGLE_ERROR_NO_IMPLEMENTATION; }
    GET_INSTANCE(instance);
    HIP_TRY(hipStreamSynchronize(live(in)));
    ringIdle(in);
    in->stream = hipStream ? (hipStream_t)hipStream : in->ownStream;
    return BEAGLE_SUCCESS;
}

// ... 121 lines not shown
        return mi355::shardedFirst(instance, [&](int h) { return beagleMi355RepeatStats(h, out10); });
    }
    Instance* in = lookup(instance);
    if (!in || !out6) return BEAGLE_ERROR_UNINITIALIZED_INSTANCE;
    out10[6] = in->statTwoTables; out10[7] = in->statUnstoredConsumers;
    out10[8] = (long)in->repeatIndex.bytes(); out10[9] = in->statRepeatResets;
    size_t bytes = in->repeatArena ? (size_t)in->repeatArenas * in->C * in->P * 32 : 0;
    for (const auto& b : in->repeatPool) bytes += b.size;
    out6[0] = in->statTableRows; out6[1] = in->statTableReads; out6[2] = in->statRepeatClades;
    out6[3] = (long)bytes; out6[4] = in->repeatIndex.builds; out6[5] = in->statRepeatBuildUs;
    return BEAGLE_SUCCESS;
}

int beagleMi355RepeatSubRunStats(int instance, long* out2) {
    if (mi355::isShardedHandle(instance)) {
        return mi355::shardedFirst(instance, [&](int h) { return beagleMi355RepeatSubRunStats(h, out2); });
    }
    Instance* in = lookup(instance);
    if (!in || !out2) return BEAGLE_ERROR_UNINITIALIZED_INSTANCE;
    out2[0] = in->statSubRuns; out2[1] = in->statSubRunOps;
    return BEAGLE_SUCCESS;
}

int beagleMi355TableOperandStats(int instance, long* out4) {
    if (mi355::isShardedHandle(instance)) {
        return mi355::shardedFirst(instance, [&](int h) { return beagleMi355TableOperandStats(h, out4); });
    }
    Instance* in = lookup(instance);
    if (!in || !out4) return BEAGLE_ERROR_UNINITIALIZED_INSTANCE;
    out4[0] = in->statTabFirst; out4[1] = in->statTabFirstBehindMem; out4[2] = in->statTabFirstBehindCherry; out4[3] = in->statTabMaxClasses;
    return BEAGLE_SUCCESS;
}

int beagleMi355WalkLaunchInfo(int instance, long* out8) {
    if (mi355::isShardedHandle(instance)) {
        return mi355::shardedFirst(instance, [&](int h) { return beagleMi355WalkLaunchInfo(h, out8); });
    }
    Instance* in = lookup(instance);
    if (!in || !out8) return BEAGLE_ERROR_UNINITIALIZED_INSTANCE;
    out8[0] = in->statTicketWalks; out8[1] = in->statFlagWalks; out8[2] = in->lastLaunchRows; out8[3] = in->lastLaunchSlices;
    out8[4] = in->statFused; out8[5] = in->statMicroOps; out8[6] = in->statSliceAccum; out8[7] = in->statRootPartsFused;
    return BEAGLE_SUCCESS;
}

int beagleMi355GradientStats(int instance, long* out4) {
    if (mi355::isShardedHandle(instance)) {
        return mi355::shardedFirst(instance, [&](int h) { return beagleMi355GradientStats(h, out4); });
    }
    Instance* in = lookup(instance);
    if (!in || !out4) return BEAGLE_ERROR_UNINITIALIZED_INSTANCE;
    out4[0] = in->statFusedGradients; out4[1] = in->statPreLists; out4[2] = in->statWalkedGradients; out4[3] = in->statLateLists;
    return BEAGLE_SUCCESS;
}

long beagleMi355DeviceBytes(int instance) {
    if (mi355::isShardedHandle(instance)) {
        std::mutex mu; long total = 0;
        mi355::shardedBroadcast(instance, [&](int h) { const long b = beagleMi355DeviceBytes(h); std::lock_guard<std::mutex> l(mu); total += b; return 0; });
        return total;
    }
    Instance* in = lookup(instance);
    return in ? (long)in->deviceBytes : -1;
}

}
```

### beast-mcmc_amd/csrc/engine_tipemission.cpp

```cpp
#include "engine_internal.h"

using namespace mi355::eng;

namespace mi355 {
namespace eng {

static int enableEmissions(Instance* in) {
    const size_t per = (size_t)in->C * in->S * in->S, oldSlots = matrixSlotLayout(in);
    in->emis = new TipEmissions();
    in->emis->tips.resize((size_t)in->tipCount);
    in->emis->useOf.assign((size_t)std::max(1, in->matrixCount), -1);
    in->emis->useStamp.assign((size_t)std::max(1, in->matrixCount), 0);
    const size_t slots = matrixSlotLayout(in);
    double* grown = nullptr;
    int rc = devAlloc(in, (void**)&grown, slots * per * sizeof(double));
    if (rc) { delete in->emis; in->emis = nullptr; matrixSlotLayout(in); return rc; }
    HIP_TRY(hipMemsetAsync(grown + oldSlots * per, 0, (slots - oldSlots) * per * sizeof(double), live(in)));
    HIP_TRY(hipMemcpyAsync(grown, in->matrices, oldSlots * per * sizeof(double), hipMemcpyDeviceToDevice, live(in)));
    in->matrices = grown;
    in->resolveEpoch++;
    return 0;
}

void freeTipEmissions(Instance* in) { delete in->emis; in->emis = nullptr; }

void dropTipEmission(Instance* in, int tip) {
    if (!in->emis || badIndex(tip, in->tipCount)) return;
    TipEmission& t = in->emis->tips[(size_t)tip];
    if (t.K == 0) return;
    if (t.folded) in->emis->foldedCount--; else in->emis->expandedCount--;
    t.K = 0; t.folded = false;
    t.codes.clear(); t.codes.shrink_to_fit(); t.table.clear();
}

static int uploadTable(Instance* in, TipEmission& t) {
    const size_t n = (size_t)t.K * in->S;
    int rc = growDevice(in, t.dTable, n * sizeof(double), n * sizeof(double), Grow::KeepOld); if (rc) return rc;
    return upload(in, t.dTable.p, t.table.data(), n * sizeof(double));
}

static int expandTip(Instance* in, int tip) {
    TipEmission& t = in->emis->tips[(size_t)tip];
    in->scaleOfPartial[tip] = -1;
    int rc = materializeTipUsers(in, tip); if (rc) return rc;
    clearVirtual(in, tip);
    rc = ensurePartials(in, tip); if (rc) return rc;
    if (!t.dCodes) { rc = devAlloc(in, (void**)&t.dCodes, ((size_t)in->P + 255) & ~(size_t)255); if (rc) return rc; }
    if (!t.codesOnDevice) { rc = upload(in, t.dCodes, t.codes.data(), (size_t)in->P); if (rc) return rc; t.codesOnDevice = true; }
    mi355::launchExpandTipEmission(live(in), in->partials[tip], t.dCodes, t.dTable.as<double>(), t.K, in->P, in->S, in->C, in->tiled);
    HIP_TRY(hipGetLastError());
    in->tipStates[tip] = nullptr;
    setCompact(in, tip, false);
// ... 34 lines not shown
            for (int w = 0; w < 2; w++) {
                const int c = op[3 + 2 * w], m = op[4 + 2 * w];
                if (badIndex(m, in->matrixCount)) continue;
                const int user = foldedTip(in, c) ? c : OTHER;
                any = any || user != OTHER;
                if (E.useStamp[(size_t)m] != stamp) {
                    E.useStamp[(size_t)m] = stamp; E.useOf[(size_t)m] = user;
                    if (user != OTHER) {
                        const TipEmission& t = E.tips[(size_t)c];
                        E.jobs.push_back(mi355::TipFoldJob{m, E.shadowBase + m, t.K, 0, t.dTable.as<double>()});
                    }
                } else if (E.useOf[(size_t)m] != user) { E.useOf[(size_t)m] = -3; conflict = true; }
            }
        }
        if (!any) return 0;
        if (!conflict) break;
        for (int k = 0; k < count; k++) {
            const int* op = ops + (size_t)k * tuple;
            for (int w = 0; w < 2; w++) {
                const int c = op[3 + 2 * w], m = op[4 + 2 * w];
                if (badIndex(m, in->matrixCount) || E.useOf[(size_t)m] != -3 || !foldedTip(in, c)) continue;
                const int rc = demoteFoldedTip(in, c); if (rc) return rc;
            }
        }
    }
    E.ops.assign(ops, ops + (size_t)count * tuple);
    for (int k = 0; k < count; k++) {
        int* op = E.ops.data() + (size_t)k * tuple;
        if (foldedTip(in, op[3]) && !badIndex(op[4], in->matrixCount)) op[4] += E.shadowBase;
        if (foldedTip(in, op[5]) && !badIndex(op[6], in->matrixCount)) op[6] += E.shadowBase;
    }
    void* dJobs = nullptr;
    int rc = uploadTransient(in, E.jobs.data(), E.jobs.size() * sizeof(mi355::TipFoldJob), &dJobs); if (rc) return rc;
    mi355::launchFoldTipEmission(live(in), in->matrices, (const mi355::TipFoldJob*)dJobs, (int)E.jobs.size(), in->S, in->C);
    HIP_TRY(hipGetLastError());
    E.foldLaunches++;
    *opsInOut = E.ops.data();
    return 0;
}

}
}

extern "C" {

int beagleMi355SetTipEmission(int instance, int tipIndex, const int* codes, int codeCount, const double* emission) {
    if (mi355::isShardedHandle(instance)) {
        if (codeCount < 1 || codeCount > 255 || !emission) return BEAGLE_ERROR_OUT_OF_RANGE;
        if (codes) return mi355::shardedSetPerPatternInts(instance, codes, [&](int h, const int* v) { return beagleMi355SetTipEmission(h, tipIndex, v, codeCount, emission); });
        return mi355::shardedBroadcast(instance, [&](int h) { return beagleMi355SetTipEmission(h, tipIndex, nullptr, codeCount, emission); });
    }
    GET_INSTANCE(instance);
    if (in->basta) return BEAGLE_ERROR_NO_IMPLEMENTATION;
    if (codeCount < 1 || codeCount > 255 || !emission || badIndex(tipIndex, in->tipCount) || badIndex(tipIndex, in->partialsCount) ||
        tipIndex >= in->compactCount) return BEAGLE_ERROR_OUT_OF_RANGE;
    if (!codes && (!in->emis || in->emis->tips[(size_t)tipIndex].K == 0)) return BEAGLE_ERROR_OUT_OF_RANGE;
    if (!in->emis) { const int rce = enableEmissions(in); if (rce) return rce; }
    TipEmissions& E = *in->emis;
    TipEmission& t = E.tips[(size_t)tipIndex];
    const int S = in->S;
    if (!codes) {
        if (codeCount != t.K) return BEAGLE_ERROR_OUT_OF_RANGE;
        t.table.assign(emission, emission + (size_t)codeCount * S);
        int rc = uploadTable(in, t); if (rc) return rc;
        return t.folded ? 0 : expandTip(in, tipIndex);
    }
    std::vector<uint8_t> c8((size_t)in->P);
// ... 25 lines not shown
```

### beast-mcmc_amd/csrc/engine_walk.cpp

```cpp
#include "engine_internal.h"
#include <atomic>
#include <unordered_map>

using mi355::OpDesc;

namespace mi355 {
namespace eng {

constexpr int FOLD_MAX_MEMBERS = 32;
constexpr double FOLD_SAFE_MAX = 1e100;

static inline void invalidate(Instance::Resolved& r) { r.tag = 0; r.dProgValid = false; r.folds.clear(); r.foldEpoch = -1; }

static void dropFolds(Instance* in, bool keepVectors) {
    for (Instance::FoldVec& f : in->folds) if (keepVectors && f.recip) in->foldFree.push_back(f.recip);
    if (!keepVectors) in->foldFree.clear();
    in->folds.clear(); in->foldIndex.clear();
    for (Instance::Resolved& r : in->resolved) invalidate(r);
}
void forgetFolds(Instance* in) { dropFolds(in, false); scalesWritten(in); }

static int foldFor(Instance* in, const std::vector<int>& members) {
    size_t h = 1469598103934665603ull;
    for (int m : members) { h ^= (size_t)(unsigned)m; h *= 1099511628211ull; }
// ... 453 lines not shown
    if (s.low) { sg.pStart = s.tab->row; sg.pEnd = s.tab->row + s.tab->D; sg.tStart = 0; sg.next = -1; return; }
    const mi355::PlanSeg& ps = *s.ps;
    sg.pStart = in->partStart[ps.partition]; sg.pEnd = in->partEnd[ps.partition]; sg.tStart = in->padStart[ps.partition];
    r.maxRange = std::max(r.maxRange, sg.pEnd - sg.pStart);
    if (r.oneLaunch) {
        if (ps.progCount > 0) r.finalStore[s.si] = use->prog[(size_t)ps.progStart + ps.progCount - 1].storeBuf;
        r.finalPart[s.si] = ps.partition;
    }
}

void ProgramResolver::finish() {
    for (size_t oi = 0; oi < nUp; oi++) {
        const mi355::PlanSeg& ps = use->segs[r.oneLaunch ? (size_t)r.order[oi] : oi];
        r.segs[oi].next = ticket && ps.next >= 0 ? posOf[(size_t)ps.next] : -1;
    }
    r.sinks = 0; r.sinkRows.clear();
    if (r.oneLaunch) {
        std::vector<char> feeds(r.segs.size(), 0);
        for (int d : r.deps) feeds[(size_t)d] = 1;
        for (size_t i = 0; i < nUp; i++) if (!feeds[i] && r.segs[i].progCount > 0) r.sinkRows.push_back((int)i);
        r.sinks = (int)r.sinkRows.size();
    }
    r.cm.clear();
    if (!fusedAt.empty()) {
        r.cm.assign(2 * r.w.size(), nullptr);
        for (const FusedAt& f : fusedAt) { r.cm[2 * f.at] = in->matrices + (size_t)f.matA * matStride; r.cm[2 * f.at + 1] = in->matrices + (size_t)f.matB * matStride; }
    }
    r.traffic.fused = (long)fusedAt.size();
    for (const mi355::PlanSeg& sg : use->segs) r.traffic.microOps += sg.progCount;
    if (r.kept) r.tag = planTag;
    r.epoch = in->resolveEpoch;
}

static int resolveProgram(Instance* in, const mi355::Plan& plan, long planTag, Instance::Resolved& r) {
    ProgramResolver pr{in, plan, r, planTag};
    return pr.run();
}

static void accountTraffic(Instance* in, const Instance::Resolved& r) {
    const Instance::WalkTraffic& t = r.traffic;
    in->statMemReads += t.memReads; in->statTipReads += t.tipReads; in->statScaleReads += t.scaleReads;
    in->statScaleWrites += t.scaleWrites; in->statStored += t.stored; in->statFused += t.fused; in->statMicroOps += t.microOps;
    in->statTableRows += t.tableRows; in->statTableReads += t.tableReads; in->statRepeatClades += t.repeatClades;
    in->statTwoTables += t.twoTables; in->statUnstoredConsumers += t.unstoredConsumers;
    in->statSubRuns += t.subRuns; in->statSubRunOps += t.subRunOps;
    in->statTabFirst += t.tabFirst; in->statTabFirstBehindMem += t.tabFirstBehindMem; in->statTabFirstBehindCherry += t.tabFirstBehindCherry;
    in->statTabMaxClasses = std::max(in->statTabMaxClasses, t.tabMaxClasses);
}

static void recordSliceSums(Instance* in, const Instance::Resolved& r) {
    if (r.sumRows.empty()) return;
    if (in->scaleGen.size() < (size_t)in->scaleCount) { in->scaleGen.assign((size_t)in->scaleCount, 0); in->scaleSeen.assign((size_t)in->scaleCount, 0); }
    const long gen = ++in->sliceGen;
    for (int idx : r.wroteScale) in->scaleGen[(size_t)idx] = gen;
    in->lastSums.valid = true; in->lastSums.epoch = in->scaleWriteEpoch; in->lastSums.gen = gen; in->lastSums.rows = r.sumRows; in->lastSums.nWritten = (int)r.wroteScale.size();
}

static int refreshProgramFolds(Instance* in, Instance::Resolved& r, bool* bad) {
    *bad = false;
    if (r.folds.empty()) return 0;
    if (r.foldEpoch != in->scaleWriteEpoch) {
        int rc = refreshFolds(in, r.folds, bad); if (rc) return rc;
        r.foldEpoch = in->scaleWriteEpoch;
        if (*bad) return 0;
    }
    in->statFoldedVectors = (long)r.folds.size();
    return 0;
// ... 22 lines not shown
};
static inline unsigned cherryRegionOff(const Instance* in, const Instance::Resolved& r) {
    return r.cm.empty() ? 0u : (unsigned)(r.w.size() * (size_t)in->C * 40 * sizeof(double));
}
static inline size_t matStreamBytes(const Instance* in, const Instance::Resolved& r) {
    if (in->walkT) return mi355::walkT32StreamBytes((int)r.w.size(), in->C, in->S) + 8192;
    return r.w.size() * (size_t)in->C * 40 * sizeof(double) * (r.cm.empty() ? 1 : 2) + 1024;
}

static int stageProgram(Instance* in, Instance::Resolved& r, PackedProgram& pp) {
    if (r.kept && r.dProgValid) { pp.dev = r.dProg.p; return 0; }
    if (pp.total > RING_BYTES / 4) {
        HIP_TRY(hipStreamSynchronize(live(in)));
        { int rc = growDevice(in, in->bigStage, pp.total, pp.total, Grow::SyncIfHeld); if (rc) return rc; }
        for (const PackedProgram::Part& q : pp.part) if (q.bytes) HIP_TRY(hipMemcpy(in->bigStage.p + q.off, q.src, q.bytes, hipMemcpyHostToDevice));
        pp.dev = in->bigStage.p;
        return 0;
    }
    const long off = stage(in, pp.part[0].src, pp.part[0].bytes, pp.total);
    if (off < 0) return BEAGLE_ERROR_GENERAL;
    for (int k = 1; k < 5; k++) if (pp.part[k].bytes) memcpy(in->hRing + off + pp.part[k].off, pp.part[k].src, pp.part[k].bytes);
    { int rc = queueCopy(in, in->dRing + off, (size_t)off, pp.total); if (rc) return rc; }
    pp.dev = in->dRing + off;
    if (in->kernelUploads) pp.staged = (const char*)in->hRingDev + off;
    if (r.kept) {
        { int rc = growDevice(in, r.dProg, pp.total, pp.total + pp.total / 4, Grow::SyncIfHeld); if (rc) return rc; }
        if (in->kernelUploads) { int rc = queueCopy(in, r.dProg.p, (size_t)off, pp.total); if (rc) return rc; }
        else HIP_TRY(hipMemcpyAsync(r.dProg.p, in->dRing + off, pp.total, hipMemcpyDeviceToDevice, live(in)));
        r.dProgValid = true;
    }
    return 0;
}

static bool uploadsCanRide(const Instance* in, const PackedProgram& pp) {
    if (in->walkT || !in->fuseLaunches || !pp.staged || in->pendingCopies.empty() || (int)in->pendingCopies.size() > mi355::HOST_COPY_MAX) return false;
    const char* m0 = (const char*)in->matrices;
    const char* m1 = m0 + (size_t)std::max(1, in->planner.matrixSlots()) * in->C * in->S * in->S * sizeof(double);
    const char* t0 = in->matStream.p; const char* t1 = t0 + in->matStream.bytes;
    const std::vector<Instance::PendingCopy>& pc = in->pendingCopies;
    for (size_t a = 0; a < pc.size(); a++) {
        const char* d0 = (const char*)pc[a].dst; const char* d1 = d0 + pc[a].bytes;
        if ((d0 < m1 && m0 < d1) || (d0 < t1 && t0 < d1)) return false;
        for (size_t b = a + 1; b < pc.size(); b++) {
            const char* e0 = (const char*)pc[b].dst; const char* e1 = e0 + pc[b].bytes;
            if (d0 < e1 && e0 < d1 && !(e0 <= d0 && d1 <= e1)) return false;
        }
    }
    return true;
}
static unsigned takeQueuedCopies(Instance* in, mi355::HostCopyList& L) {
    L.n = 0;
    unsigned blocks = 0;
    for (const Instance::PendingCopy& pc : in->pendingCopies) {
        mi355::HostCopyList::Entry& e = L.e[L.n++];
        e.dst = pc.dst; e.src = in->hRingDev + pc.ringOff; e.bytes = (unsigned)pc.bytes; e.firstBlock = blocks;
        blocks += (unsigned)((pc.bytes + 4095) / 4096);
    }
    for (int a = 0; a < L.n; a++)
        for (int b = a + 1; b < L.n; b++)
            if ((const char*)L.e[b].dst <= (const char*)L.e[a].dst && (const char*)L.e[a].dst + L.e[a].bytes <= (const char*)L.e[b].dst + L.e[b].bytes) L.e[a].bytes = 0;
    in->pendingCopies.clear();
    return blocks;
}

static int gatherMatrices(Instance* in, const Instance::Resolved& r, const PackedProgram& pp, bool* rode) {
    const int elems = in->C * in->S * in->S;
    const bool fusedSnapshot = pp.nPairs && !in->walkT && in->fuseLaunches;
    if (pp.nPairs && !fusedSnapshot) mi355::launchSnapshotMatrices(live(in), in->matrices, pp.pairs(pp.dev), pp.nPairs, elems);
    const size_t streamBytes = matStreamBytes(in, r);
    { int rc = growDevice(in, in->matStream, streamBytes, std::max(streamBytes + streamBytes / 4, (size_t)1 << 20), Grow::SyncAndFree); if (rc) return rc; }
    *rode = uploadsCanRide(in, pp);
    if (*rode) {
        if (in->pendingWalk.valid) { int rc = flushWalk(in); if (rc) return rc; }
        mi355::HostCopyList L;
        const unsigned blocks = takeQueuedCopies(in, L);
        mi355::launchGatherAndSnapshot(in->stream, pp.ops(pp.staged), pp.nOps, in->C, in->matStream.p, in->matrices, pp.pairs(pp.staged), pp.nPairs, elems,
                                       &L, (int)blocks, pp.cherryMats(pp.staged));
    }
    else if (in->walkT) mi355::launchGatherFragments(live(in), pp.ops(pp.dev), pp.nOps, in->C, in->S, in->matStream.p);
    else if (fusedSnapshot) mi355::launchGatherAndSnapshot(live(in), pp.ops(pp.dev), pp.nOps, in->C, in->matStream.p, in->matrices, pp.pairs(pp.dev), pp.nPairs, elems,
                                                           nullptr, 0, pp.cherryMats(pp.dev));
    else mi355::launchGatherMatrices(live(in), pp.ops(pp.dev), pp.nOps, in->C, in->matStream.p, pp.cherryMats(pp.dev));
    return 0;
}

static void dumpPlan(const Instance::Resolved& r, const mi355::Plan& plan) {
    if (!labEnv("BEAGLE_MI355_DUMP_PLAN")) return;
    const mi355::Plan& UP = planInUse(r, plan);
    const size_t lowN = lowerSlices(r), upN = r.segs.size() - lowN;
    fprintf(stderr, "[mi355] plan: %zu micro-ops in %zu slices (+ %zu class-table programs):", plan.prog.size(), upN, lowN);
    for (size_t i = 0; i < upN; i++) {
        const mi355::PlanSeg& ps = UP.segs[r.oneLaunch ? (size_t)r.order[i] : i];
        fprintf(stderr, " w%d:%d", ps.wave, r.segs[i].progCount);
        if (r.oneLaunch) fprintf(stderr, "(t%d d%d)", ps.tail, ps.depCount);
    }
    fprintf(stderr, "\n");
    if (atoi(labEnv("BEAGLE_MI355_DUMP_PLAN")) > 1)
        for (size_t i = 0; i < r.w.size(); i++)
            fprintf(stderr, "[mi355]   %3zu: k1 %u k2 %u hold %u scale %u store %d\n", i, (r.w[i].flags >> 5) & 7, (r.w[i].flags >> 8) & 7, (r.w[i].flags >> 11) & 3,
                    (r.w[i].flags >> 13) & 3, (r.w[i].flags & mi355::WF_STORE) ? 1 : 0);
}

static void launchClassTables(Instance* in, const Instance::Resolved& r, const PackedProgram& pp) {
    const size_t lowN = lowerSlices(r);
    in->lowerLaunched = lowN > 0;
    if (!lowN) return;
    const mi355::WalkSeg* dLow = pp.segs(pp.dev) + (r.segs.size() - lowN);
    if (in->fastWalk)
        mi355::launchWalk4Fast(live(in), pp.ops(pp.dev), dLow, (int)lowN, r.lowerRange, in->matStream.p, in->P, in->C, (long)in->scaleStride,
                               nullptr, nullptr, 0, 0, nullptr, 0, nullptr, nullptr, 0, false, cherryRegionOff(in, r));
    else
        mi355::launchWalk4(live(in), pp.ops(pp.dev), dLow, (int)lowN, r.lowerRange, in->matStream.p, in->P, in->C, (long)in->scaleStride);
}

static int launchWalk(Instance* in, const Instance::Resolved& r, const PackedProgram& pp, bool timed) {
    const size_t upN = r.segs.size() - lowerSlices(r);
    const int flagStride = (in->P + 127) / 128 + 1;
    const size_t flagBytes = r.segs.size() * (size_t)flagStride * sizeof(unsigned);
    const size_t want = (std::max(flagBytes + flagBytes / 2, (size_t)1 << 16) + 255) & ~(size_t)255;
    bool grew = false;
    in->walkTickets = nullptr;
    { int rc = growDevice(in, in->walkFlags, 2 * flagBytes, 2 * want, Grow::SyncAndFree, &grew); if (rc) return rc; }
    if (grew) HIP_TRY(hipMemsetAsync(in->walkFlags.p, 0, in->walkFlags.bytes, live(in)));
    in->walkTickets = (unsigned*)(in->walkFlags.p + in->walkFlags.bytes / 2);
    if (++in->walkEpoch == 0u) in->walkEpoch = 1u;
    Instance::PendingWalk& pw = in->pendingWalk;
    if (pw.valid) { int rc = flushWalk(in); if (rc) return rc; }
    pw.prog = pp.ops(pp.dev); pw.segs = pp.segs(pp.dev); pw.deps = pp.deps(pp.dev);
    pw.nSegs = (int)upN; pw.range = r.maxRange; pw.flagStride = flagStride; pw.epoch = in->walkEpoch;
    pw.leaves = r.leaves;
    pw.cherryOff = cherryRegionOff(in, r);
    in->statFastWalks++; in->statWalks++;
    const bool holdParts = in->partitionCount > 1 && r.sinks >= 1 && r.sinks <= mi355::ROOT_MAX_PARTS && in->fuseRootParts;
    const bool hold = in->deferWalk && in->fuseLaunches && !timed && ((in->partitionCount == 1 && pw.range == in->P && r.sinks == 1) || holdParts);
    if (hold) {
        pw.finalStore = r.finalStore; pw.finalPart = r.finalPart; pw.sinkRows = r.sinkRows;
        (void)live(in);
        pw.valid = true;
        return 0;
    }
    pw.valid = true;
    return flushWalk(in);
}

static int launchWaves(Instance* in, const Instance::Resolved& r, const mi355::Plan& UP, const PackedProgram& pp) {
    const size_t lowN = lowerSlices(r), upN = r.segs.size() - lowN;
    for (size_t b = 0; b < upN;) {
        size_t e = b + 1;
        while (e < upN && UP.segs[e].wave == UP.segs[b].wave) e++;
        int range = 0;
        for (size_t i = b; i < e; i++) range = std::max(range, r.segs[i].pEnd - r.segs[i].pStart);
        if (in->walkT) {
            if (!mi355::launchWalkT32(live(in), pp.ops(pp.dev), pp.segs(pp.dev) + b, (int)(e - b), range,
                                      in->matStream.p, in->P, in->S, in->C, in->holdSlots, r.traffic.scaleWrites > 0)) return BEAGLE_ERROR_GENERAL;
        } else if (in->fastWalk) {
            mi355::launchWalk4Fast(live(in), pp.ops(pp.dev), pp.segs(pp.dev) + b, (int)(e - b), range,
                                   in->matStream.p, in->P, in->C, (long)in->scaleStride, nullptr, nullptr, 0, 0, nullptr, 0, nullptr, nullptr, 0, false,
                                   cherryRegionOff(in, r));
            in->statFastWalks++;
        } else
            mi355::launchWalk4(live(in), pp.ops(pp.dev), pp.segs(pp.dev) + b, (int)(e - b), range,
                               in->matStream.p, in->P, in->C, (long)in->scaleStride, lowN > 0);
        in->statWalks++;
        b = e;
    }
    HIP_TRY(hipGetLastError());
    return 0;
}

static int snapshotsOnly(Instance* in, const mi355::Plan& plan) {
    if (plan.snapPairs.empty()) return 0;
    void* dPairs = nullptr;
    int rc = uploadTransient(in, plan.snapPairs.data(), plan.snapPairs.size() * sizeof(int), &dPairs); if (rc) return rc;
    mi355::launchSnapshotMatrices(live(in), in->matrices, (const int*)dPairs, (int)(plan.snapPairs.size() / 2), in->C * in->S * in->S);
    HIP_TRY(hipGetLastError());
    return 0;
}

int runPlan(Instance* in, const mi355::Plan& plan, long planTag, hipEvent_t recordBeforeWalk) {
    typedef std::chrono::steady_clock PhaseClock;
    const PhaseClock::time_point ph0 = PhaseClock::now();
    if (plan.prog.empty()) return snapshotsOnly(in, plan);
    Instance::Resolved& r = planTag && !ablateMode() ? in->resolved[planTag & 7] : in->scratch;
    r.kept = &r != &in->scratch;
    bool reuse = r.kept && r.tag == planTag && r.epoch == in->resolveEpoch;
    in->lastResolveMiss = !reuse;
    in->lastPlanCached = planTag != 0;
    if (!reuse) { int rc = resolveProgram(in, plan, planTag, r); if (rc) return rc; }
    if (r.traffic.scaleWrites > 0) scalesWritten(in);
    bool badFolds = false;
    { int rc = refreshProgramFolds(in, r, &badFolds); if (rc) return rc; }
    if (badFolds) {
        r.noFoldTag = planTag; reuse = false; in->lastResolveMiss = true;
        int rc = resolveProgram(in, plan, planTag, r); if (rc) return rc;
    }
    accountTraffic(in, r);
    recordSliceSums(in, r);
    const PhaseClock::time_point ph1 = PhaseClock::now();
    PackedProgram pp(r, plan);
    { int rc = stageProgram(in, r, pp); if (rc) return rc; }
    const PhaseClock::time_point ph2 = PhaseClock::now();
    bool rode = false;
    { int rc = gatherMatrices(in, r, pp, &rode); if (rc) return rc; }
    dumpPlan(r, plan);
    const PhaseClock::time_point ph3 = PhaseClock::now();
    if (in->hostTrace) {
        static std::atomic<int> left{6};
        if (left.fetch_sub(1) > 0)
            fprintf(stderr, "[mi355] gather launch: %zu micro-operations x %d categories%s, %zu matrix snapshots, program %s (%zu bytes), %zu queued uploads ride along\n",
                    r.w.size(), in->C, r.cm.empty() ? "" : " + cherry region", (size_t)pp.nPairs, pp.staged ? "staged by this call" : "on the device",
                    pp.total, rode ? (size_t)1 : (size_t)0);
    }
    if (in->hostTrace && !reuse && plan.prog.size() >= 64) {
        auto us = [](PhaseClock::time_point a, PhaseClock::time_point b) { return std::chrono::duration<double, std::micro>(b - a).count(); };
        fprintf(stderr, "[mi355] program of %zu micro-operations resolved: descriptors and waits %.1f us, upload %.1f us, stream + gather launch %.1f us\n", plan.prog.size(), us(ph0, ph1), us(ph1, ph2), us(ph2, ph3));
    }
    if (recordBeforeWalk) HIP_TRY(hipEventRecord(recordBeforeWalk, live(in)));
    launchClassTables(in, r, pp);
    if (r.oneLaunch) return launchWalk(in, r, pp, recordBeforeWalk != nullptr);
    return launchWaves(in, r, planInUse(r, plan), pp);
}

int flushWalk(Instance* in, const mi355::RootFused* root) {
    Instance::PendingWalk& pw = in->pendingWalk;
    if (!pw.valid) return 0;
    pw.valid = false;
    if (!in->pendingCopies.empty()) { int rc = flushUploads(in); if (rc) return rc; }
#ifdef BEAGLE_MI355_LAB
    static const int traceAt = labEnv("BEAGLE_MI355_WALK_TRACE") ? atoi(labEnv("BEAGLE_MI355_WALK_TRACE")) : 0;
    static int traceSeen = 0;
    unsigned long long* dTrace = nullptr;
    const int groupsX = (pw.range + 127) / 128;
    if (traceAt > 0 && pw.nSegs > 1 && ++traceSeen == traceAt) {
        HIP_TRY(hipMalloc((void**)&dTrace, (size_t)pw.nSegs * groupsX * 3 * sizeof(unsigned long long)));
        HIP_TRY(hipMemsetAsync(dTrace, 0, (size_t)pw.nSegs * groupsX * 3 * sizeof(unsigned long long), in->stream));
        mi355::setWalkTrace(dTrace);
    }
#endif
    mi355::launchWalk4Fast(in->stream, pw.prog, pw.segs, pw.nSegs, pw.range, in->matStream.p, in->P, in->C, (long)in->scaleStride,
                           pw.deps, in->walkFlags.as<unsigned>(), pw.epoch, pw.flagStride, root, in->walkSpinLimit, in->walkSelfServed,
                           pw.leaves > 0 ? in->walkTickets : nullptr, pw.leaves, in->xcdAware, pw.cherryOff);
#ifdef BEAGLE_MI355_LAB
    if (dTrace) {
        HIP_TRY(hipStreamSynchronize(in->stream));
        std::vector<unsigned long long> t((size_t)pw.nSegs * groupsX * 3);
        HIP_TRY(hipMemcpy(t.data(), dTrace, t.size() * sizeof(unsigned long long), hipMemcpyDeviceToHost));
        mi355::setWalkTrace(nullptr);
        hipFree(dTrace);
        unsigned long long t0 = ~0ull;
        for (size_t i = 0; i < t.size(); i += 3) if (t[i] && t[i] < t0) t0 = t[i];
        fprintf(stderr, "[mi355] walk trace, %d slices x %d groups (us from the first workgroup's entry: entry min..max | wait over min..max | end min..max):\n", pw.nSegs, groupsX);
        for (int s = 0; s < pw.nSegs; s++) {
            double lo[3] = {1e30, 1e30, 1e30}, hi[3] = {0, 0, 0};
            for (int g = 0; g < groupsX; g++)
                for (int k = 0; k < 3; k++) {
                    const unsigned long long v = t[((size_t)s * groupsX + g) * 3 + k];
                    if (!v) continue;
                    const double us = (double)(v - t0) / 100.0;
                    lo[k] = std::min(lo[k], us); hi[k] = std::max(hi[k], us);
                }
            fprintf(stderr, "[mi355]   slice %2d: %6.1f..%6.1f | %6.1f..%6.1f | %6.1f..%6.1f\n", s, lo[0], hi[0], lo[1], hi[1], lo[2], hi[2]);
        }
    }
#endif
    if (root) in->statRootFused++;
    if (pw.leaves > 0) in->statTicketWalks++; else in->statFlagWalks++;
    in->lastLaunchRows = pw.leaves > 0 ? pw.leaves : pw.nSegs; in->lastLaunchSlices = pw.nSegs;
    HIP_TRY(hipGetLastError());
    return 0;
}

int materializeList(Instance* in, const std::vector<int>& xs) {
    if (!in->virt || xs.empty()) return 0;
    if (!in->walk && !in->walkT) return materializeCherries(in, xs);
    mi355::Plan mp;
    in->planner.planMaterialize(xs, mp);
    return runPlan(in, mp);
}
int materializeVirtual(Instance* in, int X) {
    ReadSet reads(in);
    return reads.note(X) ? reads.materialize() : 0;
}
int materializeScaleUsers(Instance* in, int scaleIdx) {
    if (!in->virt || in->planner.scaleUsers(scaleIdx).empty()) return 0;
    return materializeList(in, std::vector<int>(in->planner.scaleUsers(scaleIdx)));
}
int materializeTipUsers(Instance* in, int tip) {
    if (!in->virt || in->planner.tipUsers(tip).empty()) return 0;
    return materializeList(in, std::vector<int>(in->planner.tipUsers(tip)));
}


int walkChunkOps(const Instance* in, int opCount) {
    static const int forced = labEnv("BEAGLE_MI355_CHUNK") ? atoi(labEnv("BEAGLE_MI355_CHUNK")) : -1;
    if (forced >= 0) return forced;
    if (opCount < (in->fuseWaves && in->fastWalk && !in->walkT && in->useTickets ? 32 : 64)) return 0;
    const long groups = (in->P + 127) / 128;
// ... 103 lines not shown
```

### beast-mcmc_amd/csrc/kernels.h

```cpp
#pragma once
#include <hip/hip_runtime.h>
#include <stdint.h>
#include <stdlib.h>

namespace mi355 {

#ifdef BEAGLE_MI355_LAB
inline const char* labEnv(const char* name) { return getenv(name); }
#else
inline const char* labEnv(const char*) { return nullptr; }
#endif

#if defined(__HIPCC__)
#define MI355_GLOBAL __attribute__((address_space(1)))
template <class T> __device__ __forceinline__ T MI355_GLOBAL* gptr(T* p) { return (T MI355_GLOBAL*)p; }
#endif

struct OpDesc {
    double*        dest;
    const void*    child1;
    const void*    child2;
    double*        scaleWrite;
    const double*  scaleRead;
    int            mat1, mat2;
// ... 89 lines not shown
        }
        w[i].flags |= walkWaitCode(nWait);
    }
}
struct WalkSeg { int progStart, progCount, pStart, pEnd, tStart, depStart, depCount, next; };
void launchWalk4(hipStream_t stream, const WalkOp* dProg, const WalkSeg* dSegs, int nSegs, int maxRange, const void* dStream,
                 int P, int C, long recipOff, bool tables = false);
void launchGatherMatrices(hipStream_t stream, const WalkOp* dProg, int nOps, int C, void* dStream, const double* const* cherryMats = nullptr);
struct HostCopyList;
void launchGatherAndSnapshot(hipStream_t stream, const WalkOp* dProg, int nOps, int C, void* dStream, double* matrices, const int* dSrcDst, int nPairs, int elems,
                             const HostCopyList* copies = nullptr, int copyBlocks = 0, const double* const* cherryMats = nullptr);
struct RootFusedParts;
struct RootFused {
    const double* catWeights; const double* freqs; const double* cum; const double* patternWeights;
    double* siteLogL; double* blockSums; unsigned* counter; double* out; unsigned long long* flag; unsigned long long seq;
    int cumIsRaw; int rootSeg; int groups; int pad;
    const RootFusedParts* parts;
};
struct RootFusedPart { const double* catWeights; const double* freqs; const double* cum; int cumIsRaw, rootSeg, blockOff, groups; };
struct RootFusedParts { RootFusedPart p[8]; int n, totalGroups; };
void launchWalk4Fast(hipStream_t stream, const WalkOp* dProg, const WalkSeg* dSegs, int nSegs, int maxRange, const void* dStream, int P, int C,
                     long recipOff, const int* dDeps = nullptr, unsigned* flags = nullptr, unsigned epoch = 0, int flagStride = 0,
                     const RootFused* root = nullptr, unsigned long long spinLimit = 0, unsigned* selfServed = nullptr,
                     unsigned* tickets = nullptr, int nLeaves = 0, bool xcdAware = false, unsigned cherryOff = 0);
#ifdef BEAGLE_MI355_LAB
void setWalkTrace(unsigned long long* devicePointer);
#endif
void launchRootLogLikelihood4W(hipStream_t stream, const double* root, const double* catWeights, const double* freqs,
                               const double* cum, int cumIsRaw, const double* patternWeights, double* siteLogL,
                               double* blockSums, double* out, int P, int C, int pStart, int pEnd,
                               unsigned long long* flag, unsigned long long seq, unsigned* counter);

void launchSnapshotMatrices(hipStream_t stream, double* matrices, const int* dSrcDst, int n, int elems);


constexpr int HOST_COPY_MAX = 12;
struct HostCopyList { struct Entry { void* dst; const void* src; unsigned bytes, firstBlock; } e[HOST_COPY_MAX]; int n; };
void launchHostCopies(hipStream_t stream, const HostCopyList& list, int blocks);
#ifdef __HIPCC__
__device__ __forceinline__ void hostCopyBlock(const HostCopyList& L, unsigned block) {
    int k = 0;
    while (k + 1 < L.n && block >= L.e[k + 1].firstBlock) k++;
    const size_t base = (size_t)(block - L.e[k].firstBlock) * 4096;
    if (base >= L.e[k].bytes) return;
    const char* s = (const char*)L.e[k].src + base;
    char* d = (char*)L.e[k].dst + base;
    const unsigned left = L.e[k].bytes - (unsigned)base, n = left < 4096u ? left : 4096u;
    const unsigned t = threadIdx.x;
    if ((((size_t)s | (size_t)d) & 15) == 0) {
        if (t * 16 + 16 <= n) *reinterpret_cast<uint4*>(d + t * 16) = *reinterpret_cast<const uint4*>(s + t * 16);
        for (unsigned i = (n & ~15u) + t; i < n; i += 256) d[i] = s[i];
    } else if ((((size_t)s | (size_t)d) & 3) == 0) {
        for (unsigned i = t * 4; i + 4 <= n; i += 1024) *reinterpret_cast<unsigned*>(d + i) = *reinterpret_cast<const unsigned*>(s + i);
        for (unsigned i = (n & ~3u) + t; i < n; i += 256) d[i] = s[i];
    } else
        for (unsigned i = t; i < n; i += 256) d[i] = s[i];
}
#endif
void launchPublish(hipStream_t stream, const double* src, int n, double* dst, unsigned long long* flag, unsigned long long seq);

void launchTransitionMatrices(hipStream_t stream, double* matrices, const double* eigen, const double* rates,
                              const int* dIdx, const double* dLen, const int* dEig, const int* dRate,
                              int count, int S, int C, bool complexEigen = false);

void launchTransitionMatrices4Fused(hipStream_t stream, double* matrices, const double* eigSrc, const double* ratesSrc, const int* idx,
                                    const double* len, int count, int C, bool complexEigen, const HostCopyList& pending, int copyBlocks);

void launchConvolveMatrices(hipStream_t stream, double* matrices, const int* dFirst, const int* dSecond,
                            const int* dResult, int count, int S, int C);
void launchAddMatrices(hipStream_t stream, double* matrices, const int* dFirst, const int* dSecond, const int* dResult, int count, int S, int C);

void launchDifferentialRotate(hipStream_t stream, double* V, const double* eigen, const double* dQ, const int* dPairs, int pairCount,
                              int S, bool complexEigen);
void launchDifferentialExact(hipStream_t stream, double* matrices, const double* eigen, const double* rates, const double* V,
                             const int* dIdx, const double* dLen, const int* dEig, const int* dRate, const int* dPair,
                             int count, int S, int C, bool complexEigen);
void launchDifferentialFirstOrder(hipStream_t stream, double* matrices, const double* rates, const double* dQ, const int* dIdx,
                                  const double* dLen, const int* dRate, const int* dDiff, int count, int S, int C);

constexpr int EIGEN_SWEEP_CAP = 30;
bool launchEigenReversible(hipStream_t stream, double* eigen, const double* models, const int* slots, int* sweeps, int count, int S,
                           bool complexEigen);

constexpr int GENERATOR_TERMS = 21;
constexpr int GENERATOR_MAX_SQUARINGS = 40;
bool launchGeneratorPowers(hipStream_t stream, double* tables, const double* Q, const double* mu, int count, int S);
bool launchGeneratorMatrices(hipStream_t stream, double* matrices, const double* rates, const double* tables, const double* mu,
                             const int* dIdx, const double* dLen, const int* dGen, const int* dRate, unsigned* stats, int count, int S, int C);

bool launchEpochMatrices(hipStream_t stream, double* matrices, const double* eigen, const double* rates, const int* dSlot, const int* dRate,
                         const int* dOff, const int* dSegEig, const double* dSegLen, int count, int S, int C, bool complexEigen);

void launchPruneLevel(hipStream_t stream, const OpDesc* dOps, int nOps, const double* matrices,
                      int P, int S, int C, int maxRange);

constexpr int ROOT_MAX_PARTS = 8;
struct RootPart { const double* root; const double* catWeights; const double* freqs; const double* cum; int cumIsRaw, pStart, pEnd, blockOff; };
struct RootParts { RootPart p[ROOT_MAX_PARTS]; int n; };
void launchRootLogLikelihoodParts(hipStream_t stream, const RootParts& parts, const double* patternWeights, double* siteLogL, double* blockSums,
// ... 371 lines not shown
```

### beast-mcmc_amd/csrc/kernels.hip

```cpp
#include "kernels.h"
#include "root_site4.h"
#include "transition_body.h"
#include <stdlib.h>
#include <algorithm>
#include <map>
#include <mutex>
#include <utility>

namespace mi355 {

bool grantDynamicLds(const void* kernel, size_t bytes) {
    static std::mutex mu;
    static std::map<std::pair<const void*, int>, size_t> granted;
    int dev = 0;
    if (hipGetDevice(&dev) != hipSuccess) return false;
    std::lock_guard<std::mutex> lock(mu);
    size_t& g = granted[std::make_pair(kernel, dev)];
    if (bytes <= g) return true;
    if (hipFuncSetAttribute(kernel, hipFuncAttributeMaxDynamicSharedMemorySize, (int)bytes) != hipSuccess) return false;
    g = bytes;
    return true;
}

__global__ __launch_bounds__(256) void k_hostCopies(const HostCopyList L) { hostCopyBlock(L, blockIdx.x); }
// ... 33 lines not shown
    extern __shared__ double sh[];
    double* ec = sh; double* es = sh + S; double* role = sh + 2 * S;
    const int u = blockIdx.x, c = blockIdx.y;
    const size_t eigStride = (size_t)2 * S * S + (complexEigen ? 2 : 1) * S;
    const double* U = eigen + eigStride * dEig[u];
    const double* Ui = U + (size_t)S * S;
    const double* lam = Ui + (size_t)S * S;
    const double dist = dLen[u] * rates[(size_t)dRate[u] * C + c];
    for (int k = threadIdx.x; k < S; k += blockDim.x) {
        const double im = complexEigen ? lam[S + k] : 0.0;
        if (im == 0.0) { ec[k] = exp(dist * lam[k]); es[k] = 0.0; role[k] = 0.0; continue; }
        int run = 0;
        for (int q = k - 1; q >= 0 && lam[S + q] != 0.0; q--) run++;
        const int first = (run & 1) ? k - 1 : k;
        const double b = lam[S + first], expat = exp(dist * lam[first]);
        ec[k] = expat * cos(dist * b); es[k] = expat * sin(dist * b); role[k] = first == k ? 1.0 : 2.0;
    }
    __syncthreads();
    double* M = matrices + ((size_t)dIdx[u] * C + c) * S * S;
    for (int e = threadIdx.x; e < S * S; e += blockDim.x) {
        const int i = e / S, j = e - i * S;
        double s = 0.0;
        for (int k = 0; k < S; k++) {
            const double r = role[k];
            const double ie = r == 0.0 ? Ui[k * S + j] * ec[k]
                            : r == 1.0 ? ec[k] * Ui[k * S + j] + es[k] * Ui[(k + 1) * S + j]
                                       : ec[k] * Ui[k * S + j] - es[k] * Ui[(k - 1) * S + j];
            s += U[i * S + k] * ie;
        }
        M[e] = s > 0.0 ? s : 0.0;
    }
}

__global__ __launch_bounds__(256) void k_transition4(double* __restrict__ matrices, const double* __restrict__ eigen,
                                                     const double* __restrict__ rates, const int* __restrict__ dIdx,
                                                     const double* __restrict__ dLen, const int* __restrict__ dEig,
                                                     const int* __restrict__ dRate, int count, int C, int complexEigen) {
    const int t = blockIdx.x * 256 + threadIdx.x;
    if (t >= count * C) return;
    const int u = t / C, c = t - u * C;
    const double* U = eigen + (size_t)(complexEigen ? 40 : 36) * dEig[u];
    const double dist = dLen[u] * rates[(size_t)dRate[u] * C + c];
    double m[16];
    transitionMatrixThread<4>(m, U, dist, complexEigen);
    double* M = matrices + ((size_t)dIdx[u] * C + c) * 16;
    for (int e = 0; e < 16; e++) M[e] = m[e];
}


__global__ __launch_bounds__(256) void k_transition4Fused(double* __restrict__ matrices, const double* __restrict__ eigSrc,
                                                          const double* __restrict__ ratesSrc, const int* __restrict__ idx,
                                                          const double* __restrict__ len, int count, int C, int complexEigen,
                                                          const HostCopyList L, int transitionBlocks) {
    if ((int)blockIdx.x >= transitionBlocks) { hostCopyBlock(L, blockIdx.x - (unsigned)transitionBlocks); return; }
    __shared__ double sEig[40], sRate[16];
    const int nEig = complexEigen ? 40 : 36;
    const int t = blockIdx.x * 256 + threadIdx.x;
    const bool live = t < count * C;
    const int u = live ? t / C : 0, c = live ? t - u * C : 0;
    const double myLen = len[u];
    const int myIdx = idx[u];
    if ((int)threadIdx.x < nEig) sEig[threadIdx.x] = eigSrc[threadIdx.x];
    else if ((int)threadIdx.x >= 64 && (int)threadIdx.x < 64 + C && C <= 16) sRate[threadIdx.x - 64] = ratesSrc[threadIdx.x - 64];
    __syncthreads();
    if (!live) return;
    const double* U = sEig;
    const double dist = myLen * (C <= 16 ? sRate[c] : ratesSrc[c]);
    double m[16];
    transitionMatrixThread<4>(m, U, dist, complexEigen);
    double* M = matrices + ((size_t)myIdx * C + c) * 16;
    for (int e = 0; e < 16; e++) M[e] = m[e];
}

void launchTransitionMatrices4Fused(hipStream_t stream, double* matrices, const double* eigSrc, const double* ratesSrc, const int* idx,
                                    const double* len, int count, int C, bool complexEigen, const HostCopyList& pending, int copyBlocks) {
    if (count <= 0) return;
    const int tb = (int)(((size_t)count * C + 255) / 256);
    hipLaunchKernelGGL(k_transition4Fused, dim3((unsigned)(tb + copyBlocks)), dim3(256), 0, stream, matrices, eigSrc, ratesSrc, idx, len,
                       count, C, complexEigen ? 1 : 0, pending, tb);
}

void launchTransitionMatrices(hipStream_t stream, double* matrices, const double* eigen, const double* rates,
                              const int* dIdx, const double* dLen, const int* dEig, const int* dRate,
                              int count, int S, int C, bool complexEigen) {
    if (count <= 0) return;
    if (S == 4) {
        hipLaunchKernelGGL(k_transition4, dim3((unsigned)(((size_t)count * C + 255) / 256)), dim3(256), 0, stream,
                           matrices, eigen, rates, dIdx, dLen, dEig, dRate, count, C, complexEigen ? 1 : 0);
        return;
    }
    const int threads = S * S >= 256 ? 256 : 64;
    if (((size_t)S * S + S) * sizeof(double) > 64 * 1024) {
        hipLaunchKernelGGL(k_transitionBig, dim3(count, C), dim3(256), (size_t)3 * S * sizeof(double), stream,
                           matrices, eigen, rates, dIdx, dLen, dEig, dRate, S, C, complexEigen ? 1 : 0);
        return;
    }
    hipLaunchKernelGGL(k_transition, dim3(count, C), dim3(threads), ((size_t)S * S + S) * sizeof(double), stream,
                       matrices, eigen, rates, dIdx, dLen, dEig, dRate, S, C, complexEigen ? 1 : 0);
}

__global__ __launch_bounds__(256) void k_addMatrices(double* __restrict__ matrices, const int* __restrict__ dFirst, const int* __restrict__ dSecond,
                                                     const int* __restrict__ dResult, int elems) {
    const double* a = matrices + (size_t)dFirst[blockIdx.x] * elems;
    const double* b = matrices + (size_t)dSecond[blockIdx.x] * elems;
    double* r = matrices + (size_t)dResult[blockIdx.x] * elems;
    for (int e = threadIdx.x; e < elems; e += 256) r[e] = a[e] + b[e];
}
void launchAddMatrices(hipStream_t stream, double* matrices, const int* dFirst, const int* dSecond, const int* dResult, int count, int S, int C) {
    if (count > 0) hipLaunchKernelGGL(k_addMatrices, dim3(count), dim3(256), 0, stream, matrices, dFirst, dSecond, dResult, C * S * S);
}

__global__ __launch_bounds__(256) void k_convolve(double* __restrict__ matrices, const int* __restrict__ dFirst,
                                                  const int* __restrict__ dSecond, const int* __restrict__ dResult,
                                                  int S, int C) {
    const int u = blockIdx.x, c = blockIdx.y;
    const double* A = matrices + ((size_t)dFirst[u] * C + c) * S * S;
    const double* B = matrices + ((size_t)dSecond[u] * C + c) * S * S;
    double* R = matrices + ((size_t)dResult[u] * C + c) * S * S;
    for (int e = threadIdx.x; e < S * S; e += blockDim.x) {
        const int i = e / S, j = e - i * S;
        double s = 0.0;
// ... 608 lines not shown
```

### beast-mcmc_amd/csrc/kernels_walk4.hip

```cpp
#include "kernels.h"
#include "root_site4.h"
#include <stdlib.h>
#include <string.h>
#include <algorithm>

namespace mi355 {

typedef double v4d __attribute__((ext_vector_type(4)));
typedef double v2d __attribute__((ext_vector_type(2)));
typedef unsigned int u32x8 __attribute__((ext_vector_type(8)));
typedef unsigned int u32x4 __attribute__((ext_vector_type(4)));
typedef unsigned long long u64;
#define MI355_CONST __attribute__((address_space(4)))

struct Fetched {
    v2d xa0, xa1, xb0, xb1;
    unsigned s1a, s1b, s2a, s2b;
    double inva, invb;
};

struct Desc {
    u64 src1, src2, store, scale, scaleW;
    unsigned flags;
    int tab2;
// ... 292 lines not shown
}

__global__ __launch_bounds__(256) void k_gatherAndSnapshot(const WalkOp* __restrict__ prog, int n, int C, double* __restrict__ stream, int gatherBlocks,
                                    double* __restrict__ matrices, const int* __restrict__ srcDst, int elems, int nPairs, const HostCopyList L,
                                    const double* const* __restrict__ cherryMats) {
    const int unitsPerPair = elems >> 1, snapBlocks = (int)(((size_t)nPairs * unitsPerPair + 255) / 256);
    if ((int)blockIdx.x >= gatherBlocks + snapBlocks) { hostCopyBlock(L, blockIdx.x - (unsigned)(gatherBlocks + snapBlocks)); return; }
    if ((int)blockIdx.x >= gatherBlocks) {
        const unsigned u = ((unsigned)blockIdx.x - (unsigned)gatherBlocks) * 256u + threadIdx.x, k = u / (unsigned)unitsPerPair, e = u - k * (unsigned)unitsPerPair;
        if ((int)k >= nPairs) return;
        const double2* s = reinterpret_cast<const double2*>(matrices + (size_t)srcDst[2 * k] * elems);
        double2* d = reinterpret_cast<double2*>(matrices + (size_t)srcDst[2 * k + 1] * elems);
        d[e] = s[e];
        return;
    }
    const size_t t = (size_t)blockIdx.x * blockDim.x + threadIdx.x;
    if (t >= (size_t)n * C * (cherryMats ? 20 : 10)) return;
    gatherOne(prog, stream, t, n, C, cherryMats);
}
void launchGatherAndSnapshot(hipStream_t stream, const WalkOp* dProg, int nOps, int C, void* dStream, double* matrices, const int* dSrcDst, int nPairs, int elems,
                             const HostCopyList* copies, int copyBlocks, const double* const* cherryMats) {
    HostCopyList none;
    none.n = 0;
    if (nPairs < 0) nPairs = 0;
    if (!copies || copyBlocks <= 0) { copies = &none; copyBlocks = 0; }
    if (nOps <= 0) { if (copyBlocks) launchHostCopies(stream, *copies, copyBlocks); launchSnapshotMatrices(stream, matrices, dSrcDst, nPairs, elems); return; }
    const size_t total = (size_t)nOps * C * (cherryMats ? 20 : 10);
    const int gatherBlocks = (int)((total + 255) / 256);
    const int snapBlocks = (int)(((size_t)nPairs * (elems >> 1) + 255) / 256);
    hipLaunchKernelGGL(k_gatherAndSnapshot, dim3((unsigned)(gatherBlocks + snapBlocks + copyBlocks)), dim3(256), 0, stream, dProg, nOps, C, (double*)dStream,
                       gatherBlocks, matrices, dSrcDst, elems, nPairs, *copies, cherryMats);
}

void launchGatherMatrices(hipStream_t stream, const WalkOp* dProg, int nOps, int C, void* dStream, const double* const* cherryMats) {
    if (nOps <= 0) return;
    const size_t total = (size_t)nOps * C * (cherryMats ? 20 : 10);
    hipLaunchKernelGGL(k_gatherMatrices, dim3((unsigned)((total + 255) / 256)), dim3(256), 0, stream, dProg, nOps, C, (double*)dStream, cherryMats);
}

#include "walk4_fast_loop.inc"
__device__ __forceinline__ int walkLane() {
    int l;
    asm volatile("v_mbcnt_lo_u32_b32 %0, -1, 0\n\tv_mbcnt_hi_u32_b32 %0, -1, %0" : "=v"(l));
    return l;
}
#ifdef BEAGLE_MI355_LAB
__device__ unsigned long long* g_walkTrace = nullptr;
void setWalkTrace(unsigned long long* p) { (void)hipMemcpyToSymbol(HIP_SYMBOL(g_walkTrace), &p, sizeof(p)); }
#endif
template <int MAXC>
__global__ __launch_bounds__(MAXC * 64, 4) void k_walk4_fast(const unsigned MI355_CONST* __restrict__ prog, const WalkSeg MI355_CONST* __restrict__ segs,
                                                             const v2d MI355_CONST* __restrict__ matStream, int P, int C, unsigned recipOffBytes,
                                                             const int MI355_CONST* __restrict__ deps, unsigned* __restrict__ flags, unsigned epoch, int flagStride,
                                                             unsigned long long spinLimit, unsigned* __restrict__ selfServed, const RootFused rootArgs,
                                                             unsigned* __restrict__ tickets, int xcdGroups, int nRows, unsigned cherryOff) {
    extern __shared__ v2d lds[];
    int y, bx;
    if (xcdGroups > 0) {
        const unsigned per = 8u * (unsigned)xcdGroups, batch = blockIdx.x / per, r = blockIdx.x % per;
        y = (int)(batch * 8u + (r & 7u)); bx = (int)(r >> 3);
        if (y >= nRows) return;
    } else { y = (int)blockIdx.y; bx = (int)blockIdx.x; }
#ifdef BEAGLE_MI355_LAB
    const int gridX = xcdGroups > 0 ? xcdGroups : (int)gridDim.x;
#endif
    const WalkSeg MI355_CONST& sg = segs[y];
// ... 201 lines not shown
```

### include/beagle_mi355.h

```cpp
#ifndef BEAGLE_MI355_H
#define BEAGLE_MI355_H

#ifdef __cplusplus
extern "C" {
#endif
#if defined(__GNUC__)
#pragma GCC visibility push(default)
#endif

#define BEAGLE_SUCCESS                      0
#define BEAGLE_ERROR_GENERAL               -1
#define BEAGLE_ERROR_OUT_OF_MEMORY         -2
#define BEAGLE_ERROR_UNIDENTIFIED_EXCEPTION -3
#define BEAGLE_ERROR_UNINITIALIZED_INSTANCE -4
#define BEAGLE_ERROR_OUT_OF_RANGE          -5
#define BEAGLE_ERROR_NO_RESOURCE           -6
#define BEAGLE_ERROR_NO_IMPLEMENTATION     -7
#define BEAGLE_ERROR_FLOATING_POINT        -8

#define BEAGLE_OP_NONE                     -1
#define BEAGLE_OP_COUNT                     7
#define BEAGLE_PARTITION_OP_COUNT           9

#define BEAGLE_FLAG_PRECISION_SINGLE    (1L << 0)
// ... 217 lines not shown
int beagleMi355RobustCounts(const int* instances, const int* nodes, int nodeCount, const int* categoryWeightsIndices,
                            const int* stateFrequenciesIndices, const unsigned long long* seeds, int flags, const double* branchLengths,
                            const double* eigenVectors, const double* inverseEigenVectors, const double* eigenValues,
                            const double* infinitesimalMatrix, const double* registers, int registerCount,
                            const unsigned char* includeRows, unsigned char* outStates, double* outCounts, double* outSiteTotals,
                            double* outBranchTotals, double* outTables);
int beagleMi355SimulateUnconditionedCounts(int instance, int stateCount, const double* infinitesimalMatrix,
                                           const double* startFrequencies, const double* lengths, int lengthCount, int siteCount,
                                           const double* registers, int registerCount, unsigned long long seed, double* outCounts,
                                           double* outTotals);
int beagleMi355SimulateCompleteHistories(int instance, const int* nodes, int nodeCount, int siteCount, const double* branchLengths,
                                         const double* nodeHeights, const double* infinitesimalMatrices, int qCount,
                                         int categoryRatesIndex, int categoryWeightsIndex, int stateFrequenciesIndex,
                                         const double* registers, const int* registerFlags, int registerCount, unsigned long long seed,
                                         int flags, const unsigned char* inRootStates, const int* inRateCategories,
                                         unsigned char* outStates, int* outRateCategories, double* outValues, double* outRowTotals,
                                         double* outSiteTotals, int* outEventCounts, long long eventCapacity, double* outEventHeights,
                                         unsigned char* outEventStates, long long* outEventTotal);
int beagleMi355SetTipEmission(int instance, int tipIndex, const int* codes, int codeCount, const double* emission);
int beagleMi355TipEmissionStats(int instance, long* out4);
int beagleMi355GetPartialsPinned(int instance, int bufferIndex, int scaleIndex, const double** outPinned, long* outCount);
int beagleMi355GetSiteLogLikelihoodsPinned(int instance, const double** outPinned, long* outCount);
int beagleMi355Synchronize(int instance);
int beagleMi355KernelTimer(int instance, int enable, double* outMillis, long* outLaunches);
int beagleMi355KernelTimerCalls(int instance, long* outCalls);
int beagleMi355RootFusedCount(int instance, long* outCount);
int beagleMi355SitePrefetchCount(int instance, long* outCount);
int beagleMi355KernelTimerRestart(int instance);
int beagleMi355WalkStats(int instance, long* out8);
int beagleMi355WalkHealth(int instance, long* out4);
int beagleMi355RepeatStats(int instance, long* out10);
int beagleMi355RepeatSubRunStats(int instance, long* out2);
int beagleMi355TableOperandStats(int instance, long* out4);
int beagleMi355WalkLaunchInfo(int instance, long* out8);
int beagleMi355GradientStats(int instance, long* out4);
int beagleMi355GetDimensions(int instance, int* out8);
long beagleMi355DeviceBytes(int instance);

int beagleBastaAllocateCoalescentBuffers(int instance, int coalescentBufferCount, int maxCoalescentIntervalCount,
                                         int partialsBufferCount, int initial, int threadCount);
int beagleBastaUpdatePartials(int instance, const int* operations, int operationCount, const int* intervals, int intervalCount,
                              int populationSizesIndex, int coalescentProbabilityIndex);
int beagleBastaAccumulatePartials(int instance, const int* operations, int operationCount, const int* intervals, int intervalCount,
                                  const double* intervalLengths, int populationSizesIndex, int coalescentProbabilityIndex,
                                  double* outLogLikelihood);
int beagleBastaGetBuffer(int instance, int index, double* out);
int beagleBastaGetBufferLength(int instance, int index);
int beagleBastaStats(int instance, long* out4);
#define BEAGLE_MI355_BASTA_STATES_AS_WRITTEN 2
int beagleBastaSampleStates(int instance, const int* operations, int operationCount, const int* intervals, int intervalCount,
                            int stateFrequenciesIndex, int replicateCount, unsigned long long seed, int flags,
                            unsigned char* outStates, double* outOccupancy, double* outChanges);
int beagleBastaStatesStats(int instance, long* out4);
int beagleBastaGradient(int instance, const int* operations, int operationCount, const int* intervals, int intervalCount,
                        const double* intervalLengths, const double* intervalDistances, int populationSizesIndex,
                        int coalescentProbabilityIndex, int flags, double* outPopulationSizes, double* outMigration, double* outAdjoints);
int beagleBastaGradientStats(int instance, long* out4);
int beagleBastaUpdatePartialsGrad(int instance, const int* operations, int operationCount, const int* intervals, int intervalCount,
                                  int populationSizesIndex, int coalescentProbabilityIndex);
int beagleBastaUpdateTransitionMatricesGrad(int instance, const int* transitionMatrixIndices, const double* branchLengths, int count);
int beagleBastaAccumulatePartialsGrad(int instance, const int* operations, int operationCount, const int* intervals, int intervalCount,
                                      const double* intervalLengths, int populationSizesIndex, int coalescentProbabilityIndex,
                                      double* outGradient);

typedef struct BeagleApi {
    const char* (*getVersion)(void);
// ... 46 lines not shown
```

Baseline: 3614.

## Scatter transition matrices directly into the walk stream from the matrix kernel

The transition-matrix kernels now also write each computed 4x4 matrix straight into the walk's packed matrix stream at precomputed columns, so the walk can skip its separate gather pass. A matrix epoch counter and a destination map track when the stream stays valid, and every other matrix writer marks it stale through matricesForWrite. This removes a gather kernel and its extra memory traffic per likelihood evaluation. In exchange it adds host-side bookkeeping, extra stores in the transition kernel, and cache-invalidation logic that has to stay correct.

```diff
diff --git a/beast-mcmc_amd/beagle.py b/beast-mcmc_amd/beagle.py
--- a/beast-mcmc_amd/beagle.py
+++ b/beast-mcmc_amd/beagle.py
@@ -112,7 +112,7 @@
                "beagleMi355KernelTimer", "beagleMi355DeviceBytes", "beagleMi355WalkStats", "beagleMi355GradientStats", "beagleMi355GetPartialsBatch", "beagleMi355SampleAncestralStates", "beagleMi355SampleMarkovJumps", "beagleMi355SampleMarkovJumpsUniformized",
                "beagleMi355SimulateSequences", "beagleMi355SimulateCompleteHistories", "beagleMi355RobustCounts", "beagleMi355SimulateUnconditionedCounts", "beagleMi355NodeHeightDerivatives", "beagleMi355UpdateDifferentialMatrices", "beagleMi355SetReversibleModels", "beagleMi355GetEigenDecomposition", "beagleMi355EigenStats", "beagleMi355UpdateTransitionMatricesFromGenerators", "beagleMi355GeneratorStats", "beagleMi355UpdateTransitionMatricesWithEpochs", "beagleMi355EpochStats", "beagleMi355NodePatternLikelihoods", "beagleMi355NodePatternStats", "beagleMi355NodePosteriors", "beagleMi355NodePosteriorStats", "beagleMi355PlacementScores", "beagleMi355PlacementStats", "beagleMi355SetTipEmission", "beagleMi355TipEmissionStats",
                "beagleMi355GetPartialsPinned", "beagleMi355GetSiteLogLikelihoodsPinned",
-               "beagleMi355KernelTimerCalls", "beagleMi355WalkHealth", "beagleMi355RepeatStats", "beagleMi355RepeatSubRunStats", "beagleMi355TableOperandStats", "beagleMi355WalkLaunchInfo", "beagleMi355RootFusedCount", "beagleMi355SitePrefetchCount", "beagleMi355KernelTimerRestart", "beagleMi355GetDimensions", "beagleMi355GetCommUniqueId", "beagleMi355CommInit", "beagleMi355CommInfo", "beagleMi355CalculateRootLogLikelihoodsAllReduce"] + \
+               "beagleMi355KernelTimerCalls", "beagleMi355WalkHealth", "beagleMi355RepeatStats", "beagleMi355RepeatSubRunStats", "beagleMi355TableOperandStats", "beagleMi355StreamScatterStats", "beagleMi355WalkLaunchInfo", "beagleMi355RootFusedCount", "beagleMi355SitePrefetchCount", "beagleMi355KernelTimerRestart", "beagleMi355GetDimensions", "beagleMi355GetCommUniqueId", "beagleMi355CommInit", "beagleMi355CommInfo", "beagleMi355CalculateRootLogLikelihoodsAllReduce"] + \
               ["beagleBasta" + k for k in ("AllocateCoalescentBuffers", "UpdatePartials", "AccumulatePartials", "GetBuffer", "GetBufferLength", "Stats", "SampleStates", "StatesStats",
                                            "Gradient", "GradientStats", "UpdatePartialsGrad", "UpdateTransitionMatricesGrad", "AccumulatePartialsGrad")]
 BASTA_OPERATION_SIZE = 8
@@ -1037,6 +1037,11 @@
         return {"table_first_children": int(out[0]), "behind_memory_first_child": int(out[1]), "behind_fused_cherry": int(out[2]),
                 "max_classes": int(out[3])}
 
+    def streamScatterStats(self):
+        out = (C.c_long * 4)()
+        self._check("streamScatterStats", self._ext("beagleMi355StreamScatterStats", [C.c_int, C.POINTER(C.c_long)])(self.instance, out))
+        return {"gathers_skipped": int(out[0]), "scattering_calls": int(out[1]), "registered": int(out[2]), "dropped": int(out[3])}
+
     def walkHealth(self):
         out = (C.c_long * 4)()
         self._check("walkHealth", self._ext("beagleMi355WalkHealth", [C.c_int, C.POINTER(C.c_long)])(self.instance, out))
diff --git a/beast-mcmc_amd/csrc/engine_abi.cpp b/beast-mcmc_amd/csrc/engine_abi.cpp
--- a/beast-mcmc_amd/csrc/engine_abi.cpp
+++ b/beast-mcmc_amd/csrc/engine_abi.cpp
@@ -67,7 +67,7 @@
         int rc = uploadTransient(in, first + b, n * sizeof(int), &dF); if (rc) return rc;
         rc = uploadTransient(in, second + b, n * sizeof(int), &dS); if (rc) return rc;
         rc = uploadTransient(in, result + b, n * sizeof(int), &dR); if (rc) return rc;
-        launch(live(in), in->matrices, (const int*)dF, (const int*)dS, (const int*)dR, n, in->S, in->C);
+        launch(live(in), matricesForWrite(in), (const int*)dF, (const int*)dS, (const int*)dR, n, in->S, in->C);
         b = e;
     }
     HIP_TRY(hipGetLastError());
@@ -150,7 +150,7 @@
         int rcm = devAlloc(in, (void**)&grown, slots * per * sizeof(double)); if (rcm) return rcm;
         HIP_TRY(hipMemsetAsync(grown, 0, slots * per * sizeof(double), live(in)));
         HIP_TRY(hipMemcpyAsync(grown, in->matrices, (size_t)std::max(1, in->matrixCount) * per * sizeof(double), hipMemcpyDeviceToDevice, live(in)));
-        in->matrices = grown;
+        in->matrices = grown; in->matrixEpoch++;
         if (in->tiled) { int rci = uploadIdentityMatrix(in); if (rci) return rci; }
     }
     if (in->walk) {
@@ -417,6 +417,11 @@
     };
     if (outOfRange(probIdx, in->matrixCount) || (eigenIdx ? outOfRange(eigenIdx, in->eigenCount) : badIndex(eigenScalar, in->eigenCount)) ||
         (rateIdx && outOfRange(rateIdx, in->eigenCount))) return BEAGLE_ERROR_OUT_OF_RANGE;
+    double* const block = matricesForWrite(in);
+    mi355::StreamScatter scatter;
+    bool scattering = false;
+    if (in->streamScatter) { int rcs = prepareScatter(in, probIdx, count, scatter, &scattering); if (rcs) return rcs; }
+    const mi355::StreamScatter* const sc = scattering ? &scatter : nullptr;
     bool fusable = in->S == 4 && in->kernelUploads && in->fuseLaunches && !eigenIdx && !rateIdx && (size_t)count * 12 <= RING_BYTES / 4 &&
                    (int)in->pendingCopies.size() <= mi355::HOST_COPY_MAX;
     if (fusable) {
@@ -456,8 +461,8 @@
                 if ((const char*)L.e[b].dst <= (const char*)L.e[a].dst &&
                     (const char*)L.e[a].dst + L.e[a].bytes <= (const char*)L.e[b].dst + L.e[b].bytes) L.e[a].bytes = 0;
         in->pendingCopies.clear();
-        mi355::launchTransitionMatrices4Fused(in->stream, in->matrices, eigSrc, ratesSrc, (const int*)(in->hRingDev + off + lenBytes),
-                                              (const double*)(in->hRingDev + off), count, in->C, in->eigenComplex, L, (int)blocks);
+        mi355::launchTransitionMatrices4Fused(in->stream, block, eigSrc, ratesSrc, (const int*)(in->hRingDev + off + lenBytes),
+                                              (const double*)(in->hRingDev + off), count, in->C, in->eigenComplex, L, (int)blocks, sc);
         HIP_TRY(hipGetLastError());
         return BEAGLE_SUCCESS;
     }
@@ -471,8 +476,8 @@
         if (eigenIdx) memcpy(rEig, eigenIdx, idxBytes); else std::fill(rEig, rEig + count, eigenScalar);
         if (rateIdx) memcpy(rRate, rateIdx, idxBytes); else std::fill(rRate, rRate + count, 0);
         const int* rIdx = (const int*)(in->hRingDev + off + lenBytes);
-        mi355::launchTransitionMatrices(live(in), in->matrices, in->eigen, in->rates, rIdx, (const double*)(in->hRingDev + off),
-                                        rIdx + count, rIdx + 2 * (size_t)count, count, in->S, in->C, in->eigenComplex);
+        mi355::launchTransitionMatrices(live(in), block, in->eigen, in->rates, rIdx, (const double*)(in->hRingDev + off),
+                                        rIdx + count, rIdx + 2 * (size_t)count, count, in->S, in->C, in->eigenComplex, sc);
         HIP_TRY(hipGetLastError());
         return BEAGLE_SUCCESS;
     }
@@ -487,8 +492,8 @@
     int rc = uploadTransient(in, pack.data(), pack.size(), &dPack); if (rc) return rc;
     const double* dLen = (const double*)dPack;
     const int* dIdx = (const int*)((const char*)dPack + (size_t)count * sizeof(double));
-    mi355::launchTransitionMatrices(live(in), in->matrices, in->eigen, in->rates, dIdx, dLen,
-                                    dIdx + count, dIdx + 2 * (size_t)count, count, in->S, in->C, in->eigenComplex);
+    mi355::launchTransitionMatrices(live(in), block, in->eigen, in->rates, dIdx, dLen,
+                                    dIdx + count, dIdx + 2 * (size_t)count, count, in->S, in->C, in->eigenComplex, sc);
     HIP_TRY(hipGetLastError());
     return BEAGLE_SUCCESS;
 }
@@ -686,7 +691,7 @@
     }
     void* dPairs = nullptr;
     int rc = uploadTransient(in, pairs.data(), pairs.size() * sizeof(int), &dPairs); if (rc) return rc;
-    mi355::launchTransposeMatrices(live(in), in->matrices, (const int*)dPairs, matrixCount, in->S, in->C);
+    mi355::launchTransposeMatrices(live(in), matricesForWrite(in), (const int*)dPairs, matrixCount, in->S, in->C);
     HIP_TRY(hipGetLastError());
     return BEAGLE_SUCCESS;
 }
diff --git a/beast-mcmc_amd/csrc/engine_create.cpp b/beast-mcmc_amd/csrc/engine_create.cpp
--- a/beast-mcmc_amd/csrc/engine_create.cpp
+++ b/beast-mcmc_amd/csrc/engine_create.cpp
@@ -203,6 +203,7 @@
     in->preWalk = !switchOn("BEAGLE_MI355_NO_PRE_WALK");
     in->fuseLaunches = !switchOn("BEAGLE_MI355_NO_LAUNCH_FUSION");
     in->deferWalk = !switchOn("BEAGLE_MI355_NO_ROOT_FUSION");
+    in->streamScatter = in->walk && !in->walkT && in->fuseLaunches && !switchOn("BEAGLE_MI355_NO_STREAM_SCATTER");
     in->foldScales = !switchOn("BEAGLE_MI355_NO_SCALE_FOLD");
     {
         const int gv = getenv("BEAGLE_MI355_GRADIENT_VIRTUAL") ? atoi(getenv("BEAGLE_MI355_GRADIENT_VIRTUAL")) : GRADIENT_VIRT_DEFAULT;
diff --git a/beast-mcmc_amd/csrc/engine_differential.cpp b/beast-mcmc_amd/csrc/engine_differential.cpp
--- a/beast-mcmc_amd/csrc/engine_differential.cpp
+++ b/beast-mcmc_amd/csrc/engine_differential.cpp
@@ -55,10 +55,10 @@
     if (exact) {
         double* V = in->differentialDev.as<double>();
         mi355::launchDifferentialRotate(live(in), V, in->eigen, dQ, dPairs, (int)nPairs, in->S, in->eigenComplex);
-        mi355::launchDifferentialExact(live(in), in->matrices, in->eigen, in->rates, V, dIdx, dLen, dEig, dRate, dPair, count, in->S, in->C,
+        mi355::launchDifferentialExact(live(in), matricesForWrite(in), in->eigen, in->rates, V, dIdx, dLen, dEig, dRate, dPair, count, in->S, in->C,
                                        in->eigenComplex);
     } else {
-        mi355::launchDifferentialFirstOrder(live(in), in->matrices, in->rates, dQ, dIdx, dLen, dRate, dPair, count, in->S, in->C);
+        mi355::launchDifferentialFirstOrder(live(in), matricesForWrite(in), in->rates, dQ, dIdx, dLen, dRate, dPair, count, in->S, in->C);
     }
     HIP_TRY(hipGetLastError());
     return BEAGLE_SUCCESS;
diff --git a/beast-mcmc_amd/csrc/engine_epoch.cpp b/beast-mcmc_amd/csrc/engine_epoch.cpp
--- a/beast-mcmc_amd/csrc/engine_epoch.cpp
+++ b/beast-mcmc_amd/csrc/engine_epoch.cpp
@@ -65,7 +65,7 @@
         const int* dEig = dOff + m + 1;
         const int* dSlot = dEig + nSeg;
         const int* dRate = dSlot + m;
-        if (!mi355::launchEpochMatrices(live(in), in->matrices, in->eigen, in->rates, dSlot, dRate, dOff, dEig, dLen, (int)m, in->S, in->C,
+        if (!mi355::launchEpochMatrices(live(in), matricesForWrite(in), in->eigen, in->rates, dSlot, dRate, dOff, dEig, dLen, (int)m, in->S, in->C,
                                         in->eigenComplex)) return BEAGLE_ERROR_GENERAL;
         HIP_TRY(hipGetLastError());
         first = last;
diff --git a/beast-mcmc_amd/csrc/engine_generator.cpp b/beast-mcmc_amd/csrc/engine_generator.cpp
--- a/beast-mcmc_amd/csrc/engine_generator.cpp
+++ b/beast-mcmc_amd/csrc/engine_generator.cpp
@@ -93,7 +93,7 @@
             double* tables = in->generatorDev.as<double>();
             if (!tablesDone && !mi355::launchGeneratorPowers(live(in), tables, (const double*)dPack, dMu, (int)nGen, in->S)) return BEAGLE_ERROR_GENERAL;
             tablesDone = true;
-            if (!mi355::launchGeneratorMatrices(live(in), in->matrices, in->rates, tables, dMu, dIdx, dLen, dIdx + m, dIdx + 2 * m,
+            if (!mi355::launchGeneratorMatrices(live(in), matricesForWrite(in), in->rates, tables, dMu, dIdx, dLen, dIdx + m, dIdx + 2 * m,
                                                 in->generatorStatsDev.as<unsigned>(), (int)m, in->S, in->C)) return BEAGLE_ERROR_GENERAL;
             HIP_TRY(hipGetLastError());
         }
diff --git a/beast-mcmc_amd/csrc/engine_instance.cpp b/beast-mcmc_amd/csrc/engine_instance.cpp
--- a/beast-mcmc_amd/csrc/engine_instance.cpp
+++ b/beast-mcmc_amd/csrc/engine_instance.cpp
@@ -61,8 +61,15 @@
     return (long)off;
 }
 
+static inline void noteMatrixUpload(Instance* in, const void* dst, size_t bytes) {
+    const char* m0 = (const char*)in->matrices;
+    const char* m1 = m0 + (size_t)std::max(1, in->matrixCount) * in->C * in->S * in->S * sizeof(double);
+    if (m0 && (const char*)dst < m1 && m0 < (const char*)dst + bytes) (void)matricesForWrite(in);
+}
+
 int upload(Instance* in, void* dst, const void* src, size_t bytes) {
     if (bytes == 0) return 0;
+    noteMatrixUpload(in, dst, bytes);
     if (bytes <= RING_BYTES / 4) {
         long off = stage(in, src, bytes);
         if (off < 0) return BEAGLE_ERROR_GENERAL;
@@ -83,6 +90,7 @@
 int queueCopy(Instance* in, void* dst, size_t off, size_t bytes) {
     if (bytes == 0) return 0;
     if (in->pendingWalk.valid && !in->copyKeepsWalk) { const int rcw = flushWalk(in); if (rcw) return rcw; }
+    noteMatrixUpload(in, dst, bytes);
     if (!in->kernelUploads) {
         HIP_TRY(hipMemcpyAsync(dst, in->hRing + off, bytes, hipMemcpyHostToDevice, in->stream));
         return 0;
diff --git a/beast-mcmc_amd/csrc/engine_internal.h b/beast-mcmc_amd/csrc/engine_internal.h
--- a/beast-mcmc_amd/csrc/engine_internal.h
+++ b/beast-mcmc_amd/csrc/engine_internal.h
@@ -18,6 +18,7 @@
 #include "kernels.h"
 #include "planner.h"
 #include "scratch_layout.h"
+#include "stream_dest.h"
 #include "sharded.h"
 
 namespace mi355 {
@@ -94,7 +95,20 @@
         long noFoldTag = 0;
         bool compressed = false; mi355::RepeatPlan repeats; int lowerRange = 0;
         bool repeatsMissing = false;
+        struct Scatter {
+            bool registered = false, filled = false;
+            long tag = 0, resolveEpoch = -1, stamp = -1, lastRun = 0;
+            const double* matBase = nullptr;
+            std::vector<int> list;
+            DevBufUncounted stream, dDest;
+            long triedTag = 0, triedSerial = -1;
+        } scat;
     } resolved[8], scratch;
+    bool streamScatter = false;
+    long matrixEpoch = 0, listSerial = 0, runSerial = 0;
+    std::vector<int> lastList;
+    long statGatherSkipped = 0, statScatterCalls = 0, statScatterRegistered = 0, statScatterDropped = 0;
+    struct DeferredSnap { const int* pairs = nullptr; int n = 0; } deferredSnap;
     struct FoldVec { std::vector<int> members; double* recip = nullptr; long builtEpoch = -1; bool bad = false; };
     std::vector<FoldVec> folds;
     std::vector<std::pair<size_t, int>> foldIndex;
@@ -163,6 +177,7 @@
         int nSegs = 0, range = 0, flagStride = 0; unsigned epoch = 0;
         int leaves = 0;
         unsigned cherryOff = 0;
+        const char* stream = nullptr;
         std::vector<int> finalStore;
         std::vector<int> finalPart;
         std::vector<int> sinkRows;
@@ -298,6 +313,12 @@
     if (in->pendingWalk.valid) flushWalk(in);
     return in->stream;
 }
+inline double* matricesForWrite(Instance* in) {
+    in->matrixEpoch++;
+    if (in->deferredSnap.n && in->pendingWalk.valid) flushWalk(in);
+    return in->matrices;
+}
+int prepareScatter(Instance* in, const int* probIdx, int count, mi355::StreamScatter& out, bool* any);
 int queueCopy(Instance* in, void* dst, size_t off, size_t bytes);
 inline void ringIdle(Instance* in) { if (in->pendingCopies.empty() && !in->pendingWalk.valid) in->ringHead = 0; }
 struct KeepWalkHeld {
diff --git a/beast-mcmc_amd/csrc/engine_preorder.cpp b/beast-mcmc_amd/csrc/engine_preorder.cpp
--- a/beast-mcmc_amd/csrc/engine_preorder.cpp
+++ b/beast-mcmc_amd/csrc/engine_preorder.cpp
@@ -50,7 +50,7 @@
         void *dPairs = nullptr, *dPass = nullptr;
         int rc = uploadTransient(in, pairs.data(), (size_t)2 * n * sizeof(int), &dPairs); if (rc) return rc;
         rc = uploadTransient(in, pass.data(), (size_t)2 * n * sizeof(OpDesc), &dPass); if (rc) return rc;
-        mi355::launchTransposeMatrices(live(in), in->matrices, (const int*)dPairs, n, in->S, in->C);
+        mi355::launchTransposeMatrices(live(in), matricesForWrite(in), (const int*)dPairs, n, in->S, in->C);
         mi355::launchPruneLevelTiled(live(in), (const OpDesc*)dPass, n, in->matrices, in->P, in->S, in->C, false);
         mi355::launchPruneLevelTiled(live(in), (const OpDesc*)dPass + n, n, in->matrices, in->P, in->S, in->C, anyWrite);
     }
diff --git a/beast-mcmc_amd/csrc/engine_stats.cpp b/beast-mcmc_amd/csrc/engine_stats.cpp
--- a/beast-mcmc_amd/csrc/engine_stats.cpp
+++ b/beast-mcmc_amd/csrc/engine_stats.cpp
@@ -177,6 +177,16 @@
     return BEAGLE_SUCCESS;
 }
 
+int beagleMi355StreamScatterStats(int instance, long* out4) {
+    if (mi355::isShardedHandle(instance)) {
+        return mi355::shardedFirst(instance, [&](int h) { return beagleMi355StreamScatterStats(h, out4); });
+    }
+    Instance* in = lookup(instance);
+    if (!in || !out4) return BEAGLE_ERROR_UNINITIALIZED_INSTANCE;
+    out4[0] = in->statGatherSkipped; out4[1] = in->statScatterCalls; out4[2] = in->statScatterRegistered; out4[3] = in->statScatterDropped;
+    return BEAGLE_SUCCESS;
+}
+
 int beagleMi355WalkLaunchInfo(int instance, long* out8) {
     if (mi355::isShardedHandle(instance)) {
         return mi355::shardedFirst(instance, [&](int h) { return beagleMi355WalkLaunchInfo(h, out8); });
diff --git a/beast-mcmc_amd/csrc/engine_tipemission.cpp b/beast-mcmc_amd/csrc/engine_tipemission.cpp
--- a/beast-mcmc_amd/csrc/engine_tipemission.cpp
+++ b/beast-mcmc_amd/csrc/engine_tipemission.cpp
@@ -17,7 +17,7 @@
     if (rc) { delete in->emis; in->emis = nullptr; matrixSlotLayout(in); return rc; }
     HIP_TRY(hipMemsetAsync(grown + oldSlots * per, 0, (slots - oldSlots) * per * sizeof(double), live(in)));
     HIP_TRY(hipMemcpyAsync(grown, in->matrices, oldSlots * per * sizeof(double), hipMemcpyDeviceToDevice, live(in)));
-    in->matrices = grown;
+    in->matrices = grown; in->matrixEpoch++;
     in->resolveEpoch++;
     return 0;
 }
@@ -118,7 +118,7 @@
     }
     void* dJobs = nullptr;
     int rc = uploadTransient(in, E.jobs.data(), E.jobs.size() * sizeof(mi355::TipFoldJob), &dJobs); if (rc) return rc;
-    mi355::launchFoldTipEmission(live(in), in->matrices, (const mi355::TipFoldJob*)dJobs, (int)E.jobs.size(), in->S, in->C);
+    mi355::launchFoldTipEmission(live(in), matricesForWrite(in), (const mi355::TipFoldJob*)dJobs, (int)E.jobs.size(), in->S, in->C);
     HIP_TRY(hipGetLastError());
     E.foldLaunches++;
     *opsInOut = E.ops.data();
diff --git a/beast-mcmc_amd/csrc/engine_walk.cpp b/beast-mcmc_amd/csrc/engine_walk.cpp
--- a/beast-mcmc_amd/csrc/engine_walk.cpp
+++ b/beast-mcmc_amd/csrc/engine_walk.cpp
@@ -509,7 +509,9 @@
     r.epoch = in->resolveEpoch;
 }
 
+static void dropScatter(Instance* in, Instance::Resolved& r);
 static int resolveProgram(Instance* in, const mi355::Plan& plan, long planTag, Instance::Resolved& r) {
+    dropScatter(in, r);
     ProgramResolver pr{in, plan, r, planTag};
     return pr.run();
 }
@@ -598,11 +600,11 @@
     return 0;
 }
 
-static bool uploadsCanRide(const Instance* in, const PackedProgram& pp) {
+static bool uploadsCanRide(const Instance* in, const DevBuf& sb, const PackedProgram& pp) {
     if (in->walkT || !in->fuseLaunches || !pp.staged || in->pendingCopies.empty() || (int)in->pendingCopies.size() > mi355::HOST_COPY_MAX) return false;
     const char* m0 = (const char*)in->matrices;
     const char* m1 = m0 + (size_t)std::max(1, in->planner.matrixSlots()) * in->C * in->S * in->S * sizeof(double);
-    const char* t0 = in->matStream.p; const char* t1 = t0 + in->matStream.bytes;
+    const char* t0 = sb.p; const char* t1 = t0 + sb.bytes;
     const std::vector<Instance::PendingCopy>& pc = in->pendingCopies;
     for (size_t a = 0; a < pc.size(); a++) {
         const char* d0 = (const char*)pc[a].dst; const char* d1 = d0 + pc[a].bytes;
@@ -629,24 +631,89 @@
     return blocks;
 }
 
-static int gatherMatrices(Instance* in, const Instance::Resolved& r, const PackedProgram& pp, bool* rode) {
+static void dropScatter(Instance* in, Instance::Resolved& r) {
+    if (r.scat.registered) in->statScatterDropped++;
+    r.scat.registered = false; r.scat.filled = false; r.scat.stamp = -1; r.scat.triedSerial = -1;
+}
+static bool scatterHolds(const Instance* in, const Instance::Resolved& r) {
+    const Instance::Resolved::Scatter& sc = r.scat;
+    return sc.registered && r.tag != 0 && sc.tag == r.tag && sc.resolveEpoch == in->resolveEpoch && r.epoch == in->resolveEpoch && sc.matBase == in->matrices;
+}
+static inline DevBuf& streamOf(Instance* in, Instance::Resolved& r) { return r.scat.registered ? (DevBuf&)r.scat.stream : (DevBuf&)in->matStream; }
+
+static int registerScatter(Instance* in, Instance::Resolved& r) {
+    Instance::Resolved::Scatter& sc = r.scat;
+    if (sc.triedTag == r.tag && sc.triedSerial == in->listSerial) return 0;
+    sc.triedTag = r.tag; sc.triedSerial = in->listSerial;
+    if (in->lastList.empty() || in->emis) return 0;
+    const size_t n = r.w.size(), matStride = (size_t)in->C * 16;
+    std::vector<int> tableSlot(2 * n * (r.cm.empty() ? 1 : 2), -1);
+    auto slotOf = [&](const double* m) { return m >= in->matrices && (size_t)(m - in->matrices) % matStride == 0 ? (int)((size_t)(m - in->matrices) / matStride) : -2; };
+    for (size_t k = 0; k < n; k++) {
+        const bool nop = ((r.w[k].flags >> 5) & 7) == (unsigned)mi355::WK_TIPS && ((r.w[k].flags >> 8) & 7) == (unsigned)mi355::WK_TIPS &&
+                         r.w[k].src1 == in->dummyTips && r.w[k].src2 == in->dummyTips;
+        if (!nop) { tableSlot[2 * k] = slotOf(r.w[k].m1); tableSlot[2 * k + 1] = slotOf(r.w[k].m2); }
+        if (!r.cm.empty()) for (int m = 0; m < 2; m++) if (r.cm[2 * k + m]) tableSlot[2 * (n + k) + m] = slotOf(r.cm[2 * k + m]);
+    }
+    std::vector<int> dest;
+    const mi355::StreamDestVerdict v = mi355::streamDestinations(in->lastList.data(), (int)in->lastList.size(), tableSlot.data(), (int)tableSlot.size(), in->matrixCount, dest);
+    if (in->hostTrace) fprintf(stderr, "[mi355] stream scatter: program of %zu micro-operations against a list of %zu matrices: verdict %d\n", n, in->lastList.size(), (int)v);
+    if (v != mi355::STREAM_DEST_OK) return 0;
+    for (int& d : dest) if (d >= 0) d = mi355::streamColumnOf(d, in->C);
+    const size_t streamBytes = matStreamBytes(in, r), destBytes = dest.size() * sizeof(int);
+    { int rc = growDevice(in, sc.stream, streamBytes, streamBytes + streamBytes / 4, Grow::SyncIfHeld); if (rc) return rc; }
+    { int rc = growDevice(in, sc.dDest, destBytes, destBytes + destBytes / 4, Grow::SyncIfHeld); if (rc) return rc; }
+    { int rc = upload(in, sc.dDest.p, dest.data(), destBytes); if (rc) return rc; }
+    sc.list = in->lastList;
+    sc.tag = r.tag; sc.resolveEpoch = in->resolveEpoch; sc.matBase = in->matrices;
+    sc.registered = true; sc.filled = false; sc.stamp = -1;
+    in->statScatterRegistered++;
+    return 0;
+}
+
+int prepareScatter(Instance* in, const int* probIdx, int count, mi355::StreamScatter& out, bool* any) {
+    *any = false;
+    out.t[0].dest = out.t[1].dest = nullptr; out.t[0].stream = out.t[1].stream = nullptr;
+    if (!mi355::sameIndexList(in->lastList, probIdx, count)) { in->lastList.assign(probIdx, probIdx + count); in->listSerial++; }
+    Instance::Resolved* pick[2] = {nullptr, nullptr};
+    for (Instance::Resolved& r : in->resolved) {
+        if (!r.scat.registered) continue;
+        if (!scatterHolds(in, r)) { dropScatter(in, r); continue; }
+        if (!r.scat.filled || !mi355::sameIndexList(r.scat.list, probIdx, count)) continue;
+        if (!pick[0] || r.scat.lastRun > pick[0]->scat.lastRun) { pick[1] = pick[0]; pick[0] = &r; }
+        else if (!pick[1] || r.scat.lastRun > pick[1]->scat.lastRun) pick[1] = &r;
+    }
+    if (!pick[0]) return 0;
+    if (in->pendingWalk.valid) { int rc = flushWalk(in); if (rc) return rc; }
+    for (int k = 0; k < 2 && pick[k]; k++) {
+        out.t[k].dest = pick[k]->scat.dDest.as<int>(); out.t[k].stream = pick[k]->scat.stream.as<double>();
+        pick[k]->scat.stamp = in->matrixEpoch;
+    }
+    in->statScatterCalls++;
+    *any = true;
+    return 0;
+}
+
+static int gatherMatrices(Instance* in, Instance::Resolved& r, const PackedProgram& pp, bool* rode) {
     const int elems = in->C * in->S * in->S;
     const bool fusedSnapshot = pp.nPairs && !in->walkT && in->fuseLaunches;
     if (pp.nPairs && !fusedSnapshot) mi355::launchSnapshotMatrices(live(in), in->matrices, pp.pairs(pp.dev), pp.nPairs, elems);
     const size_t streamBytes = matStreamBytes(in, r);
-    { int rc = growDevice(in, in->matStream, streamBytes, std::max(streamBytes + streamBytes / 4, (size_t)1 << 20), Grow::SyncAndFree); if (rc) return rc; }
-    *rode = uploadsCanRide(in, pp);
+    DevBuf& sb = streamOf(in, r);
+    { int rc = growDevice(in, sb, streamBytes, std::max(streamBytes + streamBytes / 4, (size_t)1 << 20), Grow::SyncAndFree); if (rc) return rc; }
+    *rode = uploadsCanRide(in, sb, pp);
     if (*rode) {
         if (in->pendingWalk.valid) { int rc = flushWalk(in); if (rc) return rc; }
         mi355::HostCopyList L;
         const unsigned blocks = takeQueuedCopies(in, L);
-        mi355::launchGatherAndSnapshot(in->stream, pp.ops(pp.staged), pp.nOps, in->C, in->matStream.p, in->matrices, pp.pairs(pp.staged), pp.nPairs, elems,
+        mi355::launchGatherAndSnapshot(in->stream, pp.ops(pp.staged), pp.nOps, in->C, sb.p, in->matrices, pp.pairs(pp.staged), pp.nPairs, elems,
                                        &L, (int)blocks, pp.cherryMats(pp.staged));
     }
-    else if (in->walkT) mi355::launchGatherFragments(live(in), pp.ops(pp.dev), pp.nOps, in->C, in->S, in->matStream.p);
-    else if (fusedSnapshot) mi355::launchGatherAndSnapshot(live(in), pp.ops(pp.dev), pp.nOps, in->C, in->matStream.p, in->matrices, pp.pairs(pp.dev), pp.nPairs, elems,
+    else if (in->walkT) mi355::launchGatherFragments(live(in), pp.ops(pp.dev), pp.nOps, in->C, in->S, sb.p);
+    else if (fusedSnapshot) mi355::launchGatherAndSnapshot(live(in), pp.ops(pp.dev), pp.nOps, in->C, sb.p, in->matrices, pp.pairs(pp.dev), pp.nPairs, elems,
                                                            nullptr, 0, pp.cherryMats(pp.dev));
-    else mi355::launchGatherMatrices(live(in), pp.ops(pp.dev), pp.nOps, in->C, in->matStream.p, pp.cherryMats(pp.dev));
+    else mi355::launchGatherMatrices(live(in), pp.ops(pp.dev), pp.nOps, in->C, sb.p, pp.cherryMats(pp.dev));
+    if (r.scat.registered) r.scat.filled = true;
     return 0;
 }
 
@@ -667,19 +734,19 @@
                     (r.w[i].flags >> 13) & 3, (r.w[i].flags & mi355::WF_STORE) ? 1 : 0);
 }
 
-static void launchClassTables(Instance* in, const Instance::Resolved& r, const PackedProgram& pp) {
+static void launchClassTables(Instance* in, Instance::Resolved& r, const PackedProgram& pp) {
     const size_t lowN = lowerSlices(r);
     in->lowerLaunched = lowN > 0;
     if (!lowN) return;
     const mi355::WalkSeg* dLow = pp.segs(pp.dev) + (r.segs.size() - lowN);
     if (in->fastWalk)
-        mi355::launchWalk4Fast(live(in), pp.ops(pp.dev), dLow, (int)lowN, r.lowerRange, in->matStream.p, in->P, in->C, (long)in->scaleStride,
+        mi355::launchWalk4Fast(live(in), pp.ops(pp.dev), dLow, (int)lowN, r.lowerRange, streamOf(in, r).p, in->P, in->C, (long)in->scaleStride,
                                nullptr, nullptr, 0, 0, nullptr, 0, nullptr, nullptr, 0, false, cherryRegionOff(in, r));
     else
-        mi355::launchWalk4(live(in), pp.ops(pp.dev), dLow, (int)lowN, r.lowerRange, in->matStream.p, in->P, in->C, (long)in->scaleStride);
-}
-
-static int launchWalk(Instance* in, const Instance::Resolved& r, const PackedProgram& pp, bool timed) {
+        mi355::launchWalk4(live(in), pp.ops(pp.dev), dLow, (int)lowN, r.lowerRange, streamOf(in, r).p, in->P, in->C, (long)in->scaleStride);
+}
+
+static int launchWalk(Instance* in, Instance::Resolved& r, const PackedProgram& pp, bool timed) {
     const size_t upN = r.segs.size() - lowerSlices(r);
     const int flagStride = (in->P + 127) / 128 + 1;
     const size_t flagBytes = r.segs.size() * (size_t)flagStride * sizeof(unsigned);
@@ -696,6 +763,7 @@
     pw.nSegs = (int)upN; pw.range = r.maxRange; pw.flagStride = flagStride; pw.epoch = in->walkEpoch;
     pw.leaves = r.leaves;
     pw.cherryOff = cherryRegionOff(in, r);
+    pw.stream = streamOf(in, r).p;
     in->statFastWalks++; in->statWalks++;
     const bool holdParts = in->partitionCount > 1 && r.sinks >= 1 && r.sinks <= mi355::ROOT_MAX_PARTS && in->fuseRootParts;
     const bool hold = in->deferWalk && in->fuseLaunches && !timed && ((in->partitionCount == 1 && pw.range == in->P && r.sinks == 1) || holdParts);
@@ -709,7 +777,8 @@
     return flushWalk(in);
 }
 
-static int launchWaves(Instance* in, const Instance::Resolved& r, const mi355::Plan& UP, const PackedProgram& pp) {
+static int launchWaves(Instance* in, Instance::Resolved& r, const mi355::Plan& UP, const PackedProgram& pp) {
+    const char* const strm = streamOf(in, r).p;
     const size_t lowN = lowerSlices(r), upN = r.segs.size() - lowN;
     for (size_t b = 0; b < upN;) {
         size_t e = b + 1;
@@ -718,15 +787,15 @@
         for (size_t i = b; i < e; i++) range = std::max(range, r.segs[i].pEnd - r.segs[i].pStart);
         if (in->walkT) {
             if (!mi355::launchWalkT32(live(in), pp.ops(pp.dev), pp.segs(pp.dev) + b, (int)(e - b), range,
-                                      in->matStream.p, in->P, in->S, in->C, in->holdSlots, r.traffic.scaleWrites > 0)) return BEAGLE_ERROR_GENERAL;
+                                      strm, in->P, in->S, in->C, in->holdSlots, r.traffic.scaleWrites > 0)) return BEAGLE_ERROR_GENERAL;
         } else if (in->fastWalk) {
             mi355::launchWalk4Fast(live(in), pp.ops(pp.dev), pp.segs(pp.dev) + b, (int)(e - b), range,
-                                   in->matStream.p, in->P, in->C, (long)in->scaleStride, nullptr, nullptr, 0, 0, nullptr, 0, nullptr, nullptr, 0, false,
+                                   strm, in->P, in->C, (long)in->scaleStride, nullptr, nullptr, 0, 0, nullptr, 0, nullptr, nullptr, 0, false,
                                    cherryRegionOff(in, r));
             in->statFastWalks++;
         } else
             mi355::launchWalk4(live(in), pp.ops(pp.dev), pp.segs(pp.dev) + b, (int)(e - b), range,
-                               in->matStream.p, in->P, in->C, (long)in->scaleStride, lowN > 0);
+                               strm, in->P, in->C, (long)in->scaleStride, lowN > 0);
         in->statWalks++;
         b = e;
     }
@@ -739,6 +808,15 @@
     void* dPairs = nullptr;
     int rc = uploadTransient(in, plan.snapPairs.data(), plan.snapPairs.size() * sizeof(int), &dPairs); if (rc) return rc;
     mi355::launchSnapshotMatrices(live(in), in->matrices, (const int*)dPairs, (int)(plan.snapPairs.size() / 2), in->C * in->S * in->S);
+    HIP_TRY(hipGetLastError());
+    return 0;
+}
+
+static int takeDeferredSnapshots(Instance* in) {
+    if (!in->deferredSnap.n) return 0;
+    const int n = in->deferredSnap.n;
+    in->deferredSnap.n = 0;
+    mi355::launchSnapshotMatrices4(in->stream, in->matrices, in->deferredSnap.pairs, n, in->C * 16);
     HIP_TRY(hipGetLastError());
     return 0;
 }
@@ -762,15 +840,24 @@
     }
     accountTraffic(in, r);
     recordSliceSums(in, r);
+    bool scatterOk = false;
+    if (r.kept && in->streamScatter) {
+        if (r.scat.registered && !scatterHolds(in, r)) dropScatter(in, r);
+        if (!r.scat.registered) { int rc = registerScatter(in, r); if (rc) return rc; }
+        r.scat.lastRun = ++in->runSerial;
+        scatterOk = r.scat.registered;
+    }
     const PhaseClock::time_point ph1 = PhaseClock::now();
     PackedProgram pp(r, plan);
     { int rc = stageProgram(in, r, pp); if (rc) return rc; }
     const PhaseClock::time_point ph2 = PhaseClock::now();
     bool rode = false;
-    { int rc = gatherMatrices(in, r, pp, &rode); if (rc) return rc; }
+    const bool current = scatterOk && reuse && pp.dev == r.dProg.p && r.scat.filled && r.scat.stamp == in->matrixEpoch;
+    if (current) { (void)live(in); in->statGatherSkipped++; in->deferredSnap.pairs = pp.pairs(pp.dev); in->deferredSnap.n = pp.nPairs; }
+    else { int rc = gatherMatrices(in, r, pp, &rode); if (rc) return rc; }
     dumpPlan(r, plan);
     const PhaseClock::time_point ph3 = PhaseClock::now();
-    if (in->hostTrace) {
+    if (in->hostTrace && !current) {
         static std::atomic<int> left{6};
         if (left.fetch_sub(1) > 0)
             fprintf(stderr, "[mi355] gather launch: %zu micro-operations x %d categories%s, %zu matrix snapshots, program %s (%zu bytes), %zu queued uploads ride along\n",
@@ -783,8 +870,8 @@
     }
     if (recordBeforeWalk) HIP_TRY(hipEventRecord(recordBeforeWalk, live(in)));
     launchClassTables(in, r, pp);
-    if (r.oneLaunch) return launchWalk(in, r, pp, recordBeforeWalk != nullptr);
-    return launchWaves(in, r, planInUse(r, plan), pp);
+    { int rc = r.oneLaunch ? launchWalk(in, r, pp, recordBeforeWalk != nullptr) : launchWaves(in, r, planInUse(r, plan), pp); if (rc) return rc; }
+    return in->pendingWalk.valid ? 0 : takeDeferredSnapshots(in);
 }
 
 int flushWalk(Instance* in, const mi355::RootFused* root) {
@@ -803,7 +890,7 @@
         mi355::setWalkTrace(dTrace);
     }
 #endif
-    mi355::launchWalk4Fast(in->stream, pw.prog, pw.segs, pw.nSegs, pw.range, in->matStream.p, in->P, in->C, (long)in->scaleStride,
+    mi355::launchWalk4Fast(in->stream, pw.prog, pw.segs, pw.nSegs, pw.range, pw.stream, in->P, in->C, (long)in->scaleStride,
                            pw.deps, in->walkFlags.as<unsigned>(), pw.epoch, pw.flagStride, root, in->walkSpinLimit, in->walkSelfServed,
                            pw.leaves > 0 ? in->walkTickets : nullptr, pw.leaves, in->xcdAware, pw.cherryOff);
 #ifdef BEAGLE_MI355_LAB
@@ -829,6 +916,7 @@
         }
     }
 #endif
+    { int rc = takeDeferredSnapshots(in); if (rc) return rc; }
     if (root) in->statRootFused++;
     if (pw.leaves > 0) in->statTicketWalks++; else in->statFlagWalks++;
     in->lastLaunchRows = pw.leaves > 0 ? pw.leaves : pw.nSegs; in->lastLaunchSlices = pw.nSegs;
diff --git a/beast-mcmc_amd/csrc/kernels.h b/beast-mcmc_amd/csrc/kernels.h
--- a/beast-mcmc_amd/csrc/kernels.h
+++ b/beast-mcmc_amd/csrc/kernels.h
@@ -145,6 +145,7 @@
                                unsigned long long* flag, unsigned long long seq, unsigned* counter);
 
 void launchSnapshotMatrices(hipStream_t stream, double* matrices, const int* dSrcDst, int n, int elems);
+void launchSnapshotMatrices4(hipStream_t stream, double* matrices, const int* dSrcDst, int nPairs, int elems);
 
 
 constexpr int HOST_COPY_MAX = 12;
@@ -172,12 +173,14 @@
 #endif
 void launchPublish(hipStream_t stream, const double* src, int n, double* dst, unsigned long long* flag, unsigned long long seq);
 
+struct StreamScatter { struct Target { const int* dest; double* stream; } t[2]; };
 void launchTransitionMatrices(hipStream_t stream, double* matrices, const double* eigen, const double* rates,
                               const int* dIdx, const double* dLen, const int* dEig, const int* dRate,
-                              int count, int S, int C, bool complexEigen = false);
+                              int count, int S, int C, bool complexEigen = false, const StreamScatter* scatter = nullptr);
 
 void launchTransitionMatrices4Fused(hipStream_t stream, double* matrices, const double* eigSrc, const double* ratesSrc, const int* idx,
-                                    const double* len, int count, int C, bool complexEigen, const HostCopyList& pending, int copyBlocks);
+                                    const double* len, int count, int C, bool complexEigen, const HostCopyList& pending, int copyBlocks,
+                                    const StreamScatter* scatter = nullptr);
 
 void launchConvolveMatrices(hipStream_t stream, double* matrices, const int* dFirst, const int* dSecond,
                             const int* dResult, int count, int S, int C);
diff --git a/beast-mcmc_amd/csrc/kernels.hip b/beast-mcmc_amd/csrc/kernels.hip
--- a/beast-mcmc_amd/csrc/kernels.hip
+++ b/beast-mcmc_amd/csrc/kernels.hip
@@ -89,26 +89,35 @@
     }
 }
 
+__device__ __forceinline__ void scatterToStream(const double (&m)[16], double* __restrict__ stream, int column, int c) {
+    if (column < 0) return;
+    double2* out = reinterpret_cast<double2*>(stream + ((size_t)column + (size_t)c * 10) * 4);
+    for (int j = 0; j < 4; j++) { out[2 * j] = make_double2(m[j], m[4 + j]); out[2 * j + 1] = make_double2(m[8 + j], m[12 + j]); }
+}
+
 __global__ __launch_bounds__(256) void k_transition4(double* __restrict__ matrices, const double* __restrict__ eigen,
                                                      const double* __restrict__ rates, const int* __restrict__ dIdx,
                                                      const double* __restrict__ dLen, const int* __restrict__ dEig,
-                                                     const int* __restrict__ dRate, int count, int C, int complexEigen) {
+                                                     const int* __restrict__ dRate, int count, int C, int complexEigen, const StreamScatter sc) {
     const int t = blockIdx.x * 256 + threadIdx.x;
     if (t >= count * C) return;
     const int u = t / C, c = t - u * C;
+    const int col0 = sc.t[0].dest ? sc.t[0].dest[u] : -1, col1 = sc.t[1].dest ? sc.t[1].dest[u] : -1;
     const double* U = eigen + (size_t)(complexEigen ? 40 : 36) * dEig[u];
     const double dist = dLen[u] * rates[(size_t)dRate[u] * C + c];
     double m[16];
     transitionMatrixThread<4>(m, U, dist, complexEigen);
     double* M = matrices + ((size_t)dIdx[u] * C + c) * 16;
     for (int e = 0; e < 16; e++) M[e] = m[e];
+    scatterToStream(m, sc.t[0].stream, col0, c);
+    scatterToStream(m, sc.t[1].stream, col1, c);
 }
 
 
 __global__ __launch_bounds__(256) void k_transition4Fused(double* __restrict__ matrices, const double* __restrict__ eigSrc,
                                                           const double* __restrict__ ratesSrc, const int* __restrict__ idx,
                                                           const double* __restrict__ len, int count, int C, int complexEigen,
-                                                          const HostCopyList L, int transitionBlocks) {
+                                                          const HostCopyList L, int transitionBlocks, const StreamScatter sc) {
     if ((int)blockIdx.x >= transitionBlocks) { hostCopyBlock(L, blockIdx.x - (unsigned)transitionBlocks); return; }
     __shared__ double sEig[40], sRate[16];
     const int nEig = complexEigen ? 40 : 36;
@@ -117,6 +126,7 @@
     const int u = live ? t / C : 0, c = live ? t - u * C : 0;
     const double myLen = len[u];
     const int myIdx = idx[u];
+    const int col0 = sc.t[0].dest ? sc.t[0].dest[u] : -1, col1 = sc.t[1].dest ? sc.t[1].dest[u] : -1;
     if ((int)threadIdx.x < nEig) sEig[threadIdx.x] = eigSrc[threadIdx.x];
     else if ((int)threadIdx.x >= 64 && (int)threadIdx.x < 64 + C && C <= 16) sRate[threadIdx.x - 64] = ratesSrc[threadIdx.x - 64];
     __syncthreads();
@@ -127,23 +137,28 @@
     transitionMatrixThread<4>(m, U, dist, complexEigen);
     double* M = matrices + ((size_t)myIdx * C + c) * 16;
     for (int e = 0; e < 16; e++) M[e] = m[e];
-}
+    scatterToStream(m, sc.t[0].stream, col0, c);
+    scatterToStream(m, sc.t[1].stream, col1, c);
+}
+
+static const StreamScatter NO_SCATTER = {{{nullptr, nullptr}, {nullptr, nullptr}}};
 
 void launchTransitionMatrices4Fused(hipStream_t stream, double* matrices, const double* eigSrc, const double* ratesSrc, const int* idx,
-                                    const double* len, int count, int C, bool complexEigen, const HostCopyList& pending, int copyBlocks) {
+                                    const double* len, int count, int C, bool complexEigen, const HostCopyList& pending, int copyBlocks,
+                                    const StreamScatter* scatter) {
     if (count <= 0) return;
     const int tb = (int)(((size_t)count * C + 255) / 256);
     hipLaunchKernelGGL(k_transition4Fused, dim3((unsigned)(tb + copyBlocks)), dim3(256), 0, stream, matrices, eigSrc, ratesSrc, idx, len,
-                       count, C, complexEigen ? 1 : 0, pending, tb);
+                       count, C, complexEigen ? 1 : 0, pending, tb, scatter ? *scatter : NO_SCATTER);
 }
 
 void launchTransitionMatrices(hipStream_t stream, double* matrices, const double* eigen, const double* rates,
                               const int* dIdx, const double* dLen, const int* dEig, const int* dRate,
-                              int count, int S, int C, bool complexEigen) {
+                              int count, int S, int C, bool complexEigen, const StreamScatter* scatter) {
     if (count <= 0) return;
     if (S == 4) {
         hipLaunchKernelGGL(k_transition4, dim3((unsigned)(((size_t)count * C + 255) / 256)), dim3(256), 0, stream,
-                           matrices, eigen, rates, dIdx, dLen, dEig, dRate, count, C, complexEigen ? 1 : 0);
+                           matrices, eigen, rates, dIdx, dLen, dEig, dRate, count, C, complexEigen ? 1 : 0, scatter ? *scatter : NO_SCATTER);
         return;
     }
     const int threads = S * S >= 256 ? 256 : 64;
diff --git a/beast-mcmc_amd/csrc/kernels_walk4.hip b/beast-mcmc_amd/csrc/kernels_walk4.hip
--- a/beast-mcmc_amd/csrc/kernels_walk4.hip
+++ b/beast-mcmc_amd/csrc/kernels_walk4.hip
@@ -348,6 +348,20 @@
                        gatherBlocks, matrices, dSrcDst, elems, nPairs, *copies, cherryMats);
 }
 
+__global__ __launch_bounds__(256) void k_snapshot4(double* __restrict__ matrices, const int* __restrict__ srcDst, int elems, int nPairs) {
+    const unsigned unitsPerPair = (unsigned)elems >> 1;
+    const unsigned u = (unsigned)blockIdx.x * 256u + threadIdx.x, k = u / unitsPerPair, e = u - k * unitsPerPair;
+    if ((int)k >= nPairs) return;
+    const double2* s = reinterpret_cast<const double2*>(matrices + (size_t)srcDst[2 * k] * elems);
+    double2* d = reinterpret_cast<double2*>(matrices + (size_t)srcDst[2 * k + 1] * elems);
+    d[e] = s[e];
+}
+void launchSnapshotMatrices4(hipStream_t stream, double* matrices, const int* dSrcDst, int nPairs, int elems) {
+    if (nPairs <= 0) return;
+    const size_t units = (size_t)nPairs * (size_t)(elems >> 1);
+    hipLaunchKernelGGL(k_snapshot4, dim3((unsigned)((units + 255) / 256)), dim3(256), 0, stream, matrices, dSrcDst, elems, nPairs);
+}
+
 void launchGatherMatrices(hipStream_t stream, const WalkOp* dProg, int nOps, int C, void* dStream, const double* const* cherryMats) {
     if (nOps <= 0) return;
     const size_t total = (size_t)nOps * C * (cherryMats ? 20 : 10);
diff --git a/beast-mcmc_amd/csrc/stream_dest.h b/beast-mcmc_amd/csrc/stream_dest.h
--- /dev/null
+++ b/beast-mcmc_amd/csrc/stream_dest.h
@@ -0,0 +1,49 @@
+#ifndef MI355_STREAM_DEST_H
+#define MI355_STREAM_DEST_H
+
+#include <cstring>
+#include <vector>
+
+namespace mi355 {
+
+enum StreamDestVerdict {
+    STREAM_DEST_OK = 0,
+    STREAM_DEST_EMPTY,
+    STREAM_DEST_BAD_INDEX,
+    STREAM_DEST_DUPLICATE,
+    STREAM_DEST_MISSING,
+    STREAM_DEST_SHARED
+};
+
+inline StreamDestVerdict streamDestinations(const int* probIdx, int count, const int* tableSlot, int nTables, int matrixCount, std::vector<int>& dest) {
+    dest.assign(count > 0 ? (size_t)count : 0, -1);
+    if (count <= 0 || nTables <= 0 || matrixCount <= 0) return STREAM_DEST_EMPTY;
+    std::vector<int> posOf((size_t)matrixCount, -1);
+    for (int u = 0; u < count; u++) {
+        const int s = probIdx[u];
+        if (s < 0 || s >= matrixCount) return STREAM_DEST_BAD_INDEX;
+        if (posOf[(size_t)s] >= 0) return STREAM_DEST_DUPLICATE;
+        posOf[(size_t)s] = u;
+    }
+    int used = 0;
+    for (int q = 0; q < nTables; q++) {
+        const int s = tableSlot[q];
+        if (s == -1) continue;
+        if (s < 0 || s >= matrixCount) return STREAM_DEST_BAD_INDEX;
+        const int u = posOf[(size_t)s];
+        if (u < 0) return STREAM_DEST_MISSING;
+        if (dest[(size_t)u] >= 0) return STREAM_DEST_SHARED;
+        dest[(size_t)u] = q;
+        used++;
+    }
+    return used ? STREAM_DEST_OK : STREAM_DEST_EMPTY;
+}
+
+inline bool sameIndexList(const std::vector<int>& kept, const int* probIdx, int count) {
+    return count > 0 && kept.size() == (size_t)count && memcmp(kept.data(), probIdx, (size_t)count * sizeof(int)) == 0;
+}
+
+inline int streamColumnOf(int q, int C) { return (q >> 1) * C * 10 + (q & 1) * 5; }
+
+}
+#endif
diff --git a/include/beagle_mi355.h b/include/beagle_mi355.h
--- a/include/beagle_mi355.h
+++ b/include/beagle_mi355.h
@@ -273,6 +273,7 @@
 int beagleMi355RepeatStats(int instance, long* out10);
 int beagleMi355RepeatSubRunStats(int instance, long* out2);
 int beagleMi355TableOperandStats(int instance, long* out4);
+int beagleMi355StreamScatterStats(int instance, long* out4);
 int beagleMi355WalkLaunchInfo(int instance, long* out8);
 int beagleMi355GradientStats(int instance, long* out4);
 int beagleMi355GetDimensions(int instance, int* out8);
```

Result: no change. 3603 (-0.3%).
